# bolcom/serenade

Hardware: AMD Instinct MI355X
Metric: predict_next queries/sec (higher is better)
Workload: dtype u32 ids / i32 accumulators / f64 scores; 1 GPU; BASELINE configs[2]: synthetic 60000000 interactions / 1760000 items, k=1500 m=2500 idf_weighting=2 last_items=4 how_many=21; batch_per_gpu=1048576, query_pool_batches=2, parallelism=query-sharded replicas x1 (no data-path collective), index=csr (built by this library)

## Files before the change

### include/serenade_hip_internal.h

```cpp
#ifndef SERENADE_HIP_INTERNAL_H
#define SERENADE_HIP_INTERNAL_H

#include "serenade_hip.h"

#ifdef __cplusplus
extern "C" {
#endif

int srn_debug_phase_cycles(const srn_index_t* idx, int enable, uint64_t* out16);

int srn_debug_shard_group_times(const srn_shard_group_t* g, double* out_ms3);

int srn_debug_last_mid_count(const srn_index_t* idx, uint32_t* out_listed);
int srn_debug_last_dedup_count(const srn_index_t* idx, uint32_t* out_merged);
int srn_debug_serve_stamps(const srn_index_t* idx, uint32_t* out4);
uint32_t srn_debug_shard_nb_positions_stride(size_t k, size_t m);
int srn_debug_last_big_count(const srn_index_t* idx, uint32_t* out_listed);

int srn_debug_sback_launches(const srn_index_t* idx, uint64_t* out_launches);

int srn_debug_eval_terms(srn_eval_set_t* set, const srn_eval_trial_t* trial, double* out_terms, size_t cap, size_t* out_n, srn_eval_result_t* out);

int srn_debug_device_sessions_last_batch(srn_device_sessions_t* s, const void** d_items, const void** d_q_off, size_t* out_n, size_t* out_max_len,
                                         uint64_t* h_items, size_t cap, uint32_t* h_q_off);

int srn_debug_exclude_filter(const srn_index_t* idx, size_t nq, const uint64_t* d_wide_ids, const double* d_wide_scores, const uint32_t* d_wide_counts, size_t wide, const uint64_t* d_excl_flat,
                             const uint32_t* d_excl_off, size_t max_excl, const uint64_t* d_items_flat, const uint32_t* d_q_off, size_t how_many, uint64_t* d_out_ids, double* d_out_scores,
                             uint32_t* d_out_counts, void* stream);

int srn_debug_fill(const srn_index_t* idx, size_t nq, uint64_t* d_ids, double* d_scores, uint32_t* d_counts, size_t how_many, const uint64_t* d_excl_flat, const uint32_t* d_excl_off,
                   const uint64_t* d_items_flat, const uint32_t* d_q_off, unsigned flags, void* stream);

int srn_debug_class_counts(const uint64_t* acc, size_t n_waves, uint32_t* out16, int device);

#define SRN_DEBUG_MERGE_ROOM 12032
int srn_debug_merge_pair(uint32_t* room, const uint32_t* pairs, size_t n_pairs, int device);

void srn_debug_reload_knobs(void);

#ifdef __cplusplus
}
#endif
#endif
```

### serenade_amd/capi.py

```python
import ctypes as C
import os

import numpy as np

from . import build as _build

SRN_OK, SRN_EINVAL, SRN_ENOMEM, SRN_EHIP, SRN_ERANGE, SRN_EIO, SRN_ENODEV, SRN_ESTATE, SRN_ETIMEOUT = 0, -1, -2, -3, -4, -5, -6, -7, -8
ATTR_ADULT, ATTR_FOR_SALE, ATTR_NONE = 1, 2, 0xFF
FLAG_BUSINESS_LOGIC = 1
MAX_HOW_MANY, MAX_SESSION_LEN, MAX_K = 512, 255, 8192

_CODES = {SRN_EINVAL: "SRN_EINVAL", SRN_ENOMEM: "SRN_ENOMEM", SRN_EHIP: "SRN_EHIP", SRN_ERANGE: "SRN_ERANGE",
          SRN_EIO: "SRN_EIO", SRN_ENODEV: "SRN_ENODEV", SRN_ESTATE: "SRN_ESTATE", SRN_ETIMEOUT: "SRN_ETIMEOUT"}


class SerenadeError(RuntimeError):
    def __init__(self, code, msg):
        super().__init__("%s: %s" % (_CODES.get(code, code), msg))
        self.code = code


class SessionsView(C.Structure):
    _fields_ = [("sess_off", C.c_void_p), ("items", C.c_void_p), ("max_ts", C.c_void_p), ("n_sessions", C.c_size_t)]

# ... 143 lines not shown
    "srn_find_neighbors": (_i, [_vp, _vp, _sz, _sz, _sz, _vp, _vp, C.POINTER(_sz)]),
    "srn_index_free": (None, [_vp]),
    "srn_predict": (_i, [_vp, _vp, _sz, _sz, _sz, _sz, _i, _vp, _vp, C.POINTER(_sz)]),
    "srn_predict_stats": (_i, [_vp, C.POINTER(_u64), C.POINTER(_u64), C.POINTER(_u64)]),
    "srn_predict_batch": (_i, [_vp, _vp, _vp, _sz, _sz, _sz, _sz, C.c_uint, _vp, _vp, _vp]),
    "srn_batcher_create": (_i, [_vp, _sz, C.c_uint, _sz, _sz, _sz, _i, C.POINTER(_vp)]),
    "srn_batcher_predict": (_i, [_vp, _vp, _sz, _vp, _vp, C.POINTER(_sz)]),
    "srn_batcher_stats": (_i, [_vp, C.POINTER(_u64), C.POINTER(_u64), C.POINTER(_u64)]),
    "srn_batcher_free": (None, [_vp]),
    "srn_batcher_how_many": (_i, [_vp, C.POINTER(_sz)]),
    "srn_session_key": (_i, [C.c_char_p, _sz, C.POINTER(_u64), C.POINTER(_u64)]),
    "srn_session_store_create": (_i, [_u64, _u64, C.POINTER(_vp)]),
    "srn_session_store_free": (None, [_vp]),
    "srn_session_store_get": (_i, [_vp, _u64, _u64, _u64, _vp, _sz, C.POINTER(_sz)]),
    "srn_session_store_update": (_i, [_vp, _u64, _u64, _u64, _vp, _sz]),
    "srn_session_store_sweep": (_i, [_vp, _u64, C.POINTER(_u64)]),
    "srn_recommend": (_i, [_vp, _vp, C.c_char_p, _sz, _u64, _i, _sz, _u64, _vp, _vp, C.POINTER(_sz)]),
    "srn_predict_batch_device": (_i, [_vp, _vp, _vp, _sz, _sz, _sz, _sz, _sz, C.c_uint, _vp, _vp, _vp, _vp]),
    "srn_predict_batch_device_excl": (_i, [_vp, _vp, _vp, _sz, _sz, _vp, _vp, _sz, _sz, _sz, _sz, C.c_uint, _vp, _vp, _vp, _vp]),
    "srn_predict_batch_excl": (_i, [_vp, _vp, _vp, _sz, _vp, _vp, _sz, _sz, _sz, _sz, C.c_uint, _vp, _vp, _vp]),
    "srn_debug_exclude_filter": (_i, [_vp, _sz, _vp, _vp, _vp, _sz, _vp, _vp, _sz, _vp, _vp, _sz, _vp, _vp, _vp, _vp]),
    "srn_debug_fill": (_i, [_vp, _sz, _vp, _vp, _vp, _sz, _vp, _vp, _vp, _vp, C.c_uint, _vp]),
    "srn_debug_class_counts": (_i, [_vp, _sz, _vp, _i]),
    "srn_debug_merge_pair": (_i, [_vp, _vp, _sz, _i]),
    "srn_predict_batch_debug": (_i, [_vp, _vp, _vp, _sz, _sz, _sz, _sz, C.c_uint, _vp, _vp, _vp, _vp, _vp, _vp, _vp]),
    "srn_index_reserve": (_i, [_vp, _sz, _sz, _sz, _sz, _sz, C.c_uint, _vp]),
    "srn_last_kernel_ms": (_i, [_vp, C.POINTER(C.c_double), C.POINTER(C.c_double), C.POINTER(C.c_uint32)]),
    "srn_index_build_shard": (_i, [C.POINTER(SessionsView), _sz, _sz, C.c_double, C.c_uint32, C.c_uint32, _i, C.POINTER(_vp)]),
    "srn_index_shard": (_i, [_vp, C.c_uint32, C.c_uint32, _i, C.POINTER(_vp)]),
    "srn_index_build_shard_gpu": (_i, [C.POINTER(SessionsView), _sz, _sz, C.c_double, C.c_uint32, C.c_uint32, _i, C.POINTER(_vp)]),
    "srn_index_load_shard": (_i, [C.c_char_p, C.c_uint32, C.c_uint32, _i, C.POINTER(_vp)]),
    "srn_shard_group_unique_id": (_i, [_vp, _sz]),
    "srn_shard_group_create": (_i, [_vp, _vp, _i, _i, C.POINTER(_vp)]),
    "srn_shard_group_create_with_comm": (_i, [_vp, _i, _i, _vp, C.POINTER(_vp)]),
    "srn_shard_group_create_local": (_i, [C.POINTER(_vp), _i, C.POINTER(_vp)]),
    "srn_shard_group_predict_batch": (_i, [_vp, _vp, _vp, _sz, _sz, _sz, _sz, _sz, C.c_uint, _vp, _vp, _vp, _vp]),
    "srn_shard_group_stats": (_i, [_vp, _vp]),
    "srn_shard_group_set_overlap": (_i, [_vp, _i]),
    "srn_shard_group_wait": (_i, [_vp, _u64]),
    "srn_shard_group_set_postings": (_i, [_vp, _vp]),
    "srn_debug_shard_group_times": (_i, [_vp, _vp]),
    "srn_index_postings_view": (_i, [_vp, _i, C.POINTER(_vp)]),
    "srn_shard_group_free": (None, [_vp]),
    "srn_kernel_timing": (_i, [_vp, C.c_int]),
    "srn_kernel_times": (_i, [_vp, C.c_uint32, _vp, _vp, C.POINTER(C.c_uint32)]),
    "srn_kernel_times_detail": (_i, [_vp, C.c_uint32, _vp, _vp, _vp, _vp, C.POINTER(C.c_uint32)]),
    "srn_debug_phase_cycles": (_i, [_vp, _i, _vp]),
    "srn_debug_reload_knobs": (None, []),
    "srn_debug_last_mid_count": (_i, [_vp, C.POINTER(C.c_uint32)]),
    "srn_debug_last_dedup_count": (_i, [_vp, C.POINTER(C.c_uint32)]),
    "srn_debug_serve_stamps": (_i, [_vp, _vp]),
    "srn_debug_shard_nb_positions_stride": (C.c_uint32, [_sz, _sz]),
    "srn_debug_last_big_count": (_i, [_vp, C.POINTER(C.c_uint32)]),
    "srn_debug_sback_launches": (_i, [_vp, C.POINTER(_u64)]),
    "srn_last_path_counts": (_i, [_vp, C.POINTER(C.c_uint32), C.POINTER(C.c_uint32), C.POINTER(C.c_uint32)]),
    "srn_eval_set_create": (_i, [_vp, _vp, _vp, _sz, _vp, _vp, _sz, C.POINTER(_vp)]),
    "srn_eval_set_from_tsv": (_i, [_vp, C.c_char_p, C.c_char_p, C.POINTER(_vp)]),
    "srn_eval_set_from_events": (_i, [_vp, _vp, _vp, _vp, _sz, _vp, _sz, C.c_uint, _vp, C.POINTER(_vp)]),
    "srn_evaluate": (_i, [_vp, C.POINTER(EvalTrial), _sz, C.POINTER(EvalResult), _vp]),
    "srn_eval_set_free": (None, [_vp]),
    "srn_evaluate_bootstrap": (_i, [_vp, C.POINTER(EvalTrial), _sz, C.POINTER(Bootstrap), C.POINTER(EvalResult), _vp, _vp]),
    "srn_bootstrap_weights": (_i, [_u64, C.c_uint32, _u64, _sz, _vp]),
    "srn_debug_eval_terms": (_i, [_vp, C.POINTER(EvalTrial), _vp, _sz, C.POINTER(_sz), C.POINTER(EvalResult)]),
    "srn_device_sessions_create": (_i, [_i, _sz, _sz, _u64, _u64, C.POINTER(_vp)]),
    "srn_device_sessions_free": (None, [_vp]),
    "srn_device_sessions_get": (_i, [_vp, _u64, _u64, _u64, _vp, _sz, C.POINTER(_sz)]),
    "srn_device_sessions_update": (_i, [_vp, _u64, _u64, _u64, _vp, _sz]),
    "srn_device_sessions_sweep": (_i, [_vp, _u64, C.POINTER(_u64)]),
    "srn_device_sessions_stats": (_i, [_vp, C.POINTER(DeviceSessionsStats)]),
    "srn_device_sessions_timing": (_i, [_vp, _i]),
    "srn_device_sessions_last_ms": (_i, [_vp, C.POINTER(C.c_double), C.POINTER(C.c_double)]),
    "srn_device_sessions_count": (_i, [_vp, _u64, C.POINTER(_u64), C.POINTER(_u64)]),
    "srn_device_sessions_export_device": (_i, [_vp, _u64, _sz, _vp, _vp, _vp, _vp, _vp, _sz, _vp, _vp]),
    "srn_device_sessions_export": (_i, [_vp, _u64, _sz, _vp, _vp, _vp, _vp, _vp, _sz, C.POINTER(_sz)]),
    "srn_device_sessions_import_device": (_i, [_vp, _vp, _vp, _vp, _vp, _vp, _sz, _sz, _vp]),
    "srn_device_sessions_import": (_i, [_vp, _vp, _vp, _vp, _vp, _vp, _sz, _sz]),
    "srn_device_sessions_resize": (_i, [_vp, _sz, _sz, _u64]),
    "srn_device_sessions_set_max_capacity": (_i, [_vp, _sz]),
    "srn_device_sessions_growth": (_i, [_vp, C.POINTER(_u64), C.POINTER(_u64), C.POINTER(_u64)]),
    "srn_device_sessions_save": (_i, [_vp, C.c_char_p, _u64]),
    "srn_device_sessions_load": (_i, [C.c_char_p, _i, _sz, _sz, _u64, _u64, C.POINTER(_vp)]),
    "srn_device_sessions_file_info": (_i, [C.c_char_p, C.POINTER(DeviceSessionsFileInfo)]),
    "srn_device_sessions_top_items": (_i, [_vp, _u64, _u64, C.c_uint32, _sz, _vp, _vp, C.POINTER(_sz)]),
    "srn_index_set_fallback_trending": (_i, [_vp, _vp, _u64, _u64, C.c_uint32, _sz, C.c_uint, C.POINTER(_sz)]),
    "srn_session_keys": (_i, [_vp, _vp, _sz, _vp, _vp]),
    "srn_device_sessions_set_history": (_i, [_vp, _sz]),
    "srn_device_sessions_history": (_i, [_vp, C.POINTER(_sz)]),
    "srn_recommend_batch_device": (_i, [_vp, _vp, _vp, _vp, _vp, _vp, _sz, _u64, _sz, _sz, _sz, _sz, C.c_uint, _vp, _vp, _vp, _vp]),
    "srn_recommend_batch": (_i, [_vp, _vp, _vp, _vp, _vp, _vp, _sz, _u64, _sz, _sz, _sz, _sz, C.c_uint, _vp, _vp, _vp]),
    "srn_recommend_batch_device_at": (_i, [_vp, _vp, _vp, _vp, _vp, _vp, _vp, _sz, _u64, _sz, _sz, _sz, _sz, C.c_uint, _vp, _vp, _vp, _vp]),
    "srn_recommend_batch_at": (_i, [_vp, _vp, _vp, _vp, _vp, _vp, _vp, _sz, _u64, _sz, _sz, _sz, _sz, C.c_uint, _vp, _vp, _vp]),
    "srn_feedback_observe_device_at": (_i, [_vp, _vp, _vp, _vp, _vp, _vp, _sz, _u64, _vp, _vp, _vp, _sz, _vp, _vp]),
    "srn_feedback_observe_at": (_i, [_vp, _vp, _vp, _vp, _vp, _vp, _sz, _u64, _vp, _vp, _vp, _sz, _vp]),
    "srn_debug_device_sessions_last_batch": (_i, [_vp, C.POINTER(_vp), C.POINTER(_vp), C.POINTER(_sz), C.POINTER(_sz), _vp, _sz, _vp]),
    "srn_feedback_create": (_i, [_i, _sz, _sz, _u64, _u64, C.POINTER(_vp)]),
    "srn_feedback_free": (None, [_vp]),
    "srn_feedback_observe_device": (_i, [_vp, _vp, _vp, _vp, _vp, _sz, _u64, _vp, _vp, _vp, _sz, _vp, _vp]),
    "srn_feedback_observe": (_i, [_vp, _vp, _vp, _vp, _vp, _sz, _u64, _vp, _vp, _vp, _sz, _vp]),
    "srn_feedback_stats": (_i, [_vp, C.POINTER(FeedbackStats)]),
    "srn_feedback_histogram": (_i, [_vp, _vp, _vp, _sz]),
    "srn_feedback_reset_counters": (_i, [_vp]),
    "srn_feedback_sweep": (_i, [_vp, _u64, C.POINTER(_u64)]),
    "srn_feedback_get": (_i, [_vp, _u64, _u64, _u64, _vp, _sz, C.POINTER(C.c_uint32), C.POINTER(C.c_uint32), C.POINTER(_u64)]),
    "srn_feedback_bootstrap_enable": (_i, [_vp, C.c_uint32, _u64]),
    "srn_feedback_bootstrap_disable": (_i, [_vp]),
    "srn_feedback_bootstrap_info": (_i, [_vp, C.POINTER(C.c_uint32), C.POINTER(_u64)]),
# ... 82 lines not shown
```

### serenade_amd/csrc/srn_capi.cpp

```cpp
#include <algorithm>
#include <cstring>
#include <new>
#include <vector>

#include "srn_internal.h"

namespace srn { const char* last_error_cstr(); int device_count(); }
using namespace srn;

namespace {
template <typename F> int guarded(F f) {
    try { return f(); }
    catch (const std::bad_alloc&) { return fail(SRN_ENOMEM, "out of host memory"); }
    catch (const std::exception& e) { return fail(SRN_EINVAL, std::string("internal error: ") + e.what()); }
    catch (...) { return fail(SRN_EINVAL, "internal error"); }
}

int check_predict_args(const srn_index_t* idx, size_t k, size_t m, size_t how_many) {
    if (!idx) return fail(SRN_EINVAL, "null index");
    if (!idx->dev) return fail(SRN_ENODEV, "index has no device attached; there is no CPU fallback behind this ABI");
    if (idx->flat.postings_only) return fail(SRN_EINVAL, "a postings-only view holds no rows: it serves a shard group (srn_shard_group_set_postings), not predict calls");
    if (k == 0 || m == 0 || how_many == 0) return fail(SRN_EINVAL, "k, m and how_many must be > 0");
    if (how_many > SRN_MAX_HOW_MANY) return fail(SRN_ERANGE, "how_many above SRN_MAX_HOW_MANY");
    if (k > SRN_MAX_K) return fail(SRN_ERANGE, "k above SRN_MAX_K");
// ... 585 lines not shown
        if (rc) return rc;
        srn_index* ix = new srn_index();
        return finish_index(ix, shard_flat_index(full, shard, n_shards, ix->flat), device, out); });
}
int srn_index_load_shard(const char* path, uint32_t shard, uint32_t n_shards, int device, srn_index_t** out) {
    return guarded([&]() -> int {
        if (!path || !out) return fail(SRN_EINVAL, "null argument");
        *out = nullptr;
        FlatIndex full;
        int rc = load_flat_index(path, full);
        if (rc) return rc;
        srn_index* ix = new srn_index();
        rc = full.n_shards == 1 ? shard_flat_index(full, shard, n_shards, ix->flat)
                                : (full.shard == shard && full.n_shards == n_shards ? (ix->flat = std::move(full), SRN_OK) : fail(SRN_EINVAL, "the file holds another shard"));
        return finish_index(ix, rc, device, out); });
}
int srn_kernel_times(const srn_index_t* idx, uint32_t max_n, double* out_ms_main, double* out_ms_retry, uint32_t* out_n) {
    if (!idx || !idx->dev) return fail(SRN_ENODEV, "index has no device attached");
    if (!out_n) return fail(SRN_EINVAL, "null argument");
    return guarded([&]() -> int { return device_kernel_times(idx->dev, max_n, out_ms_main, out_ms_retry, out_n); });
}

int srn_kernel_times_detail(const srn_index_t* idx, uint32_t max_n, double* out_ms_prep, double* out_ms_fast, double* out_ms_predict,
                            double* out_ms_retry, uint32_t* out_n) {
    if (!idx || !idx->dev) return fail(SRN_ENODEV, "index has no device attached");
    if (!out_n) return fail(SRN_EINVAL, "null argument");
    return guarded([&]() -> int { return device_kernel_times(idx->dev, max_n, out_ms_predict, out_ms_retry, out_n, out_ms_prep, out_ms_fast); });
}

int srn_kernel_timing(srn_index_t* idx, int enable) {
    if (!idx || !idx->dev) return fail(SRN_ENODEV, "index has no device attached");
    return device_kernel_timing(idx->dev, enable);
}

int srn_debug_phase_cycles(const srn_index_t* idx, int enable, uint64_t* out16) {
    if (!idx || !idx->dev) return fail(SRN_ENODEV, "index has no device attached");
    return guarded([&]() -> int { return device_phase_cycles(idx->dev, enable, (unsigned long long*)out16); });
}

int srn_last_path_counts(const srn_index_t* idx, uint32_t* out_nq, uint32_t* out_general, uint32_t* out_global_pass) {
    if (!idx || !idx->dev) return fail(SRN_ENODEV, "index has no device attached");
    return guarded([&]() -> int { return device_last_path_counts(idx->dev, out_nq, out_general, out_global_pass); });
}
uint32_t srn_debug_shard_nb_positions_stride(size_t k, size_t m) {
    return device_shard_nb_positions_stride(launch_params(1, k, m, 21, 0, 4));
}
int srn_debug_serve_stamps(const srn_index_t* idx, uint32_t* out4) {
    if (!idx || !idx->dev || !out4) return fail(SRN_EINVAL, "null argument");
    return device_serve_last_stamps(idx->dev, out4);
}
int srn_debug_last_mid_count(const srn_index_t* idx, uint32_t* out_listed) {
    if (!idx || !idx->dev) return fail(SRN_ENODEV, "index has no device attached");
    return guarded([&]() -> int { return device_last_mid_count(idx->dev, out_listed); });
}
int srn_debug_last_dedup_count(const srn_index_t* idx, uint32_t* out_merged) {
    if (!idx || !idx->dev || !out_merged) return fail(SRN_EINVAL, "null argument");
    return guarded([&]() -> int { return device_last_dedup_count(idx->dev, out_merged); });
}
int srn_debug_last_big_count(const srn_index_t* idx, uint32_t* out_listed) {
    if (!idx || !idx->dev) return fail(SRN_ENODEV, "index has no device attached");
    return guarded([&]() -> int { return device_last_mid_count(idx->dev, nullptr, out_listed); });
}

int srn_debug_sback_launches(const srn_index_t* idx, uint64_t* out_launches) {
    if (!idx || !idx->dev || !out_launches) return fail(SRN_EINVAL, "null argument / no device");
    *out_launches = device_sback_launches(idx->dev); return SRN_OK;
}

void srn_debug_reload_knobs(void) { reload_knobs(); }

static int check_eval_index(const srn_index_t* idx) {
    if (!idx) return fail(SRN_EINVAL, "null index");
    if (!idx->dev) return fail(SRN_ENODEV, "index has no device attached; evaluation runs on the GPU only");
    if (idx->flat.postings_only) return fail(SRN_EINVAL, "a postings-only view holds no rows");
    return check_not_a_shard(idx);
}

static int check_trials(const srn_eval_set_t* set, const srn_eval_trial_t* trials, size_t n_trials, const srn_eval_result_t* out) {
    if (n_trials && (!trials || !out)) return fail(SRN_EINVAL, "null argument");
    for (size_t t = 0; t < n_trials; ++t) {
        const srn_eval_trial_t& tr = trials[t];
        if (tr.max_items_in_session == 0) return fail(SRN_EINVAL, "max_items_in_session must be > 0");
        if (tr.max_items_in_session > SRN_MAX_SESSION_LEN) return fail(SRN_ERANGE, "max_items_in_session above SRN_MAX_SESSION_LEN: a prefix could exceed the kernels' session limit");
        if (tr.length == 0) return fail(SRN_EINVAL, "length must be > 0");
        if (tr.length > SRN_MAX_HOW_MANY) return fail(SRN_ERANGE, "length above SRN_MAX_HOW_MANY");
        if (tr.k == 0 || tr.m == 0 || tr.how_many == 0) return fail(SRN_EINVAL, "k, m and how_many must be > 0");
        if (tr.how_many > SRN_MAX_HOW_MANY) return fail(SRN_ERANGE, "how_many above SRN_MAX_HOW_MANY");
        if (tr.k > SRN_MAX_K) return fail(SRN_ERANGE, "k above SRN_MAX_K");
        if (tr.m > 0x7FFFFFFFu) return fail(SRN_ERANGE, "m too large");
        if (tr.history != 0 && (tr.history < tr.max_items_in_session || tr.history > SRN_MAX_SESSION_LEN))
            return fail(SRN_ERANGE, "history must be 0 or in max_items_in_session..SRN_MAX_SESSION_LEN");
        if (tr.how_many + eval_excl_capacity(tr) > SRN_MAX_HOW_MANY)
            return fail(SRN_ERANGE, "how_many + the exclusion lists' capacity (history, or max_items_in_session) above SRN_MAX_HOW_MANY");
    }
    if (!set) return fail(SRN_EINVAL, "null evaluation set");
    for (size_t t = 0; t < n_trials; ++t) { int rc = check_predict_args(set->idx, trials[t].k, trials[t].m, trials[t].how_many); if (rc) return rc;
                                            if (trials[t].flags & SRN_FLAG_FILL) { rc = check_has_fallback(set->idx); if (rc) return rc; } }
    return SRN_OK;
}

int srn_eval_set_create(const srn_index_t* idx, const uint64_t* items_flat, const uint64_t* sess_off, size_t n_sessions,
                        const uint64_t* train_item_ids, const uint64_t* train_item_counts, size_t n_train_items, srn_eval_set_t** out) {
    return guarded([&]() -> int {
        if (!out) return fail(SRN_EINVAL, "null argument");
        *out = nullptr;
        int rc = check_eval_index(idx); if (rc) return rc;
// ... 280 lines not shown
```

### serenade_amd/csrc/srn_fast.hip

```cpp
#include <hip/hip_runtime.h>

#include <cstdio>
#include <cstdlib>

#include "srn_device.h"
#include "srn_prep.h"
#include "srn_kernels.h"

namespace srn {

#ifndef SRN_FAST_NT
#define SRN_FAST_NT 1
#endif
typedef uint32_t fin_v4u __attribute__((ext_vector_type(4)));
__device__ __forceinline__ void fin_store(uint4* p, const uint4& v) {
#if SRN_FAST_NT
    __builtin_nontemporal_store((fin_v4u{v.x, v.y, v.z, v.w}), reinterpret_cast<fin_v4u*>(p));
#else
    *p = v;
#endif
}
__device__ __forceinline__ uint4 fin_load(const uint4* p) {
#if SRN_FAST_NT
    const fin_v4u v = __builtin_nontemporal_load(reinterpret_cast<const fin_v4u*>(p)); return make_uint4(v.x, v.y, v.z, v.w);
// ... 232 lines not shown
            inm |= in ? 1u << x : 0u;
            nmp |= in ? (unsigned long long)nmv[x] << (4 * x) : 0ull;
            acc += in ? 1ull << (4u * nmv[x]) : 0ull;
        }
    }
    uint32_t* cls = misc + FS_CLS;
    {
        const uint32_t wc = wave_class_counts(acc, lane);
        const uint32_t mycnt = lane < 16u ? wc : 0u;
        if (mycnt) atomicAdd(&cls[lane], mycnt);
    }
    __syncthreads();
    uint32_t nstar, rstar;
    {
        const uint32_t cv = lane < 16u ? cls[lane] : 0u; const uint32_t pre = wave_incl_scan(cv);
        const uint32_t suf = (uint32_t)__builtin_amdgcn_readlane((int)pre, 63) - pre + cv;
        const unsigned long long reach = __ballot(suf >= k);
        nstar = 63u - (uint32_t)__clzll((long long)reach);
        rstar = k - ((uint32_t)__builtin_amdgcn_readlane((int)suf, (int)nstar) - (uint32_t)__builtin_amdgcn_readlane((int)cv, (int)nstar));
    }
    uint32_t mine = 0;
#pragma unroll
    for (int x = 0; x < G; ++x) mine += ((inm >> x) & 1u) && (uint32_t)((nmp >> (4 * x)) & 15ull) == nstar;
    uint32_t tot_star;
    uint32_t before = block_excl_scan<BLOCK>(mine, misc + FS_SCAN_B, tot_star);
    uint32_t sel = 0, tmask = 0;
#pragma unroll
    for (int x = 0; x < G; ++x) {
        const bool in = (inm >> x) & 1u; const uint32_t c = (uint32_t)((nmp >> (4 * x)) & 15ull);
        const bool eq = in && c == nstar, take = in && (c > nstar || (eq && before < rstar));
        tmask |= take ? 1u << x : 0u; sel += take; before += eq;
    }
    const uint32_t inc = wave_incl_scan(sel);
    uint32_t base = 0; if (lane == 63u && inc) base = atomicAdd(&misc[FS_NB], inc);
    uint32_t at = (uint32_t)__builtin_amdgcn_readlane((int)base, 63) + inc - sel;
#pragma unroll
    for (int x = 0; x < G; ++x) if ((tmask >> x) & 1u) nbl[at++] = fv[x];
    return 0xFFFFFFFFu;
}

enum { FM_FUSED = 0, FM_FRONT = 1, FM_BACK = 2 };
template <int WG_PER_CU, bool FRAG, bool WIDE, int MODE = FM_FUSED, bool MID = false, bool BIG = false, bool LONG = false, bool TINY = false>
#ifndef SRN_FAST_WAVES
#define SRN_FAST_WAVES (WG_PER_CU * 2)
#endif
#ifndef SRN_TINY_WAVES
#define SRN_TINY_WAVES 2
#endif
__global__ __launch_bounds__(512, TINY ? SRN_TINY_WAVES : BIG ? 4 : SRN_FAST_WAVES) void vmis_fast_kernel(DeviceIndex ix_arg, LaunchParams p_arg, FastParams f_arg) {
#if SRN_FAST_SMALL
    static_assert(!BIG || MID, "BIG is a form of MID"); static_assert(!LONG || BIG, "LONG is a form of BIG");
    constexpr uint32_t SIDF = BIG ? F_BIG_TOTAL - (F_TOTAL - F_SIDF) : F_SIDF, SATTR = SIDF + 512 * 8;
    constexpr uint32_t MW = (SIDF - F_WORK) / 4;
    __shared__ __attribute__((aligned(16))) char smem[BIG ? F_BIG_TOTAL : F_TOTAL];
#else
    extern __shared__ __attribute__((aligned(16))) char smem[];
#endif
    typedef const __attribute__((address_space(4))) char* KArg;
    const KArg ka = (KArg)__builtin_amdgcn_kernarg_segment_ptr();
    constexpr size_t OFF_P = (sizeof(DeviceIndex) + alignof(LaunchParams) - 1) / alignof(LaunchParams) * alignof(LaunchParams);
    constexpr size_t OFF_F = (OFF_P + sizeof(LaunchParams) + alignof(FastParams) - 1) / alignof(FastParams) * alignof(FastParams);
    const __attribute__((address_space(4))) DeviceIndex& ix = *(const __attribute__((address_space(4))) DeviceIndex*)ka;
    const __attribute__((address_space(4))) LaunchParams& p = *(const __attribute__((address_space(4))) LaunchParams*)(ka + OFF_P);
    const __attribute__((address_space(4))) FastParams& f = *(const __attribute__((address_space(4))) FastParams*)(ka + OFF_F);
    constexpr int BLOCK = 512, NW = 8;
    constexpr int NL = LONG ? (int)F_LONG_LISTS : MID ? (int)F_MID_LISTS : 4;
    constexpr uint32_t SINV = F_SINV;
    static_assert(!MID || MODE == FM_FUSED, "MID: fused form only");
    const uint32_t tid = threadIdx.x, lane = tid & 63u, wave = tid >> 6;
    const unsigned long long lt = (1ull << lane) - 1ull;
    static_assert(!TINY || (MODE == FM_FUSED && !BIG && !FRAG), "TINY: the lean or the MID fused form over an unsharded index");
    if constexpr (TINY) {
        unsigned long long* const a_items = reinterpret_cast<unsigned long long*>(smem + F_W10 + 64); uint32_t* const a_off = reinterpret_cast<uint32_t*>(smem + F_W10 + 64 + 64);
        const uint32_t alen = f.tiny_len;
        if (f.serve == nullptr) {
        if (alen) { if (tid < 8u) a_items[tid] = f.tiny_items[tid]; if (tid == 0u) { a_off[0] = 0u; a_off[1] = alen; } __syncthreads(); }
        if (tid < PREP_LANES) prep_group(ix_arg, alen ? (const uint64_t*)a_items : p.items_flat, alen ? (const uint32_t*)a_off : p.q_off, alen ? 0u : blockIdx.x, tid, p.m, p.max_len,
                                         const_cast<char*>(p.prep) + (size_t)blockIdx.x * p.prep_stride, nullptr, 0u, nullptr);
        __syncthreads();
        }
    }

    uint32_t* misc = (uint32_t*)(smem + F_MISC);
    uint8_t* wlut = (uint8_t*)(smem + F_WLUT);
    uint16_t* w10t = (uint16_t*)(smem + F_W10);
    uint32_t* nbl = (uint32_t*)(smem + F_NBL);
    unsigned long long* ckey = (unsigned long long*)(smem + F_CAND);
    uint32_t* cidx = (uint32_t*)(smem + F_CAND + F_CAND_CAP * 8);
    char* const acc_base = smem + F_HOT;
    uint32_t* hot = (uint32_t*)(smem + F_HOT);
    uint32_t* ikeys = (uint32_t*)(smem + F_TABLE);
    int* iacc = (int*)(smem + F_TABLE + F_TABLE_WORDS * 4);
    uint2* hits = (uint2*)(smem + F_HITS);
    uint32_t* surv = (uint32_t*)(smem + F_SURV);
    constexpr uint32_t SURV_CAP = F_SURV_WORDS - 256u;
    uint32_t* const cls_area = BIG ? (uint32_t*)(smem + SIDF) - 256 : surv + SURV_CAP;
    uint32_t* const dn_area = cls_area - F_M_MAX / 4u;
    uint2* const nb2 = reinterpret_cast<uint2*>(dn_area - F_K_MAX * 2u);
    uint32_t* thist = surv + SURV_CAP;
    auto num_of = [&](uint32_t set) -> uint32_t {
        if constexpr (MID) return (uint32_t)wlut[set & 31u] + (uint32_t)wlut[32u + (set >> 5)];
        else return (uint32_t)wlut[set]; };
    auto w10_of = [&](uint32_t set) -> uint32_t {
        if constexpr (MID) { const uint32_t lo = set & 31u, hi = set >> 5; const uint32_t mp = lo ? (uint32_t)wlut[64u + lo] : (uint32_t)wlut[96u + hi]; return (9u - mp) * ((uint32_t)wlut[lo] + (uint32_t)wlut[32u + hi]); }
        else return (uint32_t)w10t[set]; };

    unsigned long long* tacc = (unsigned long long*)(smem + F_MISC + FS_TACC * 4);
    if (tid < 16u) tacc[tid] = 0ull;
    const bool ticking = p.phase_cycles != nullptr;
    const bool business = (p.flags & SRN_FLAG_BUSINESS_LOGIC) != 0u;
    const uint32_t n_kept = ix.n_kept;
    auto qpos = [&](uint32_t pq) -> uint32_t { return ((wave + NW * (pq >> 6)) << 6) + (pq & 63u); };

    uint32_t* const pre = (uint32_t*)(smem + F_W10 + 64);
    bool have_pre = false;
    { const ItemMeta m0 = f.meta_sample[tid];
      ((double*)(smem + SIDF))[tid] = m0.idf > 0.0 ? m0.idf : 1.0; ((uint8_t*)(smem + SATTR))[tid] = (uint8_t)m0.attr;
      if (tid < 16u) ((double*)(smem + SINV))[tid] = tid < 8u ? f.inv_idf_hot[tid] : f.inv_idf_hi; }
    const bool listed = !MID && MODE == FM_BACK && f.mid_list != nullptr;
    const uint32_t q_end = TINY ? p.nq : LONG ? *f.long_cnt : BIG ? *f.bigq_cnt : MID || listed ? *f.mid_cnt : p.nq;
    const bool ordered = !MID && MODE != FM_FRONT && f.order != nullptr && !listed;
    const uint32_t ox = blockIdx.x & 7u;
    const bool serving = TINY && f.serve != nullptr;
    const uint32_t qi_step = serving ? 0u : ordered ? gridDim.x >> 3 : gridDim.x;
    uint32_t serve_seq = 0u; bool serve_have = false; unsigned long long serve_t0 = 0ull, serve_c0 = 0ull;
    if constexpr (TINY) { if (serving) serve_seq = __atomic_load_n(&(f.serve + blockIdx.x)->done_seq, __ATOMIC_RELAXED); }
    const uint32_t qi_end = ordered ? ord_count(f.order_dups != nullptr ? p.nq - *f.order_dups : p.nq, ox) : q_end;
    for (uint32_t qi = ordered ? blockIdx.x >> 3 : (MODE == FM_FRONT ? f.q_base : 0u) + blockIdx.x; qi < qi_end; qi += qi_step) {
        if constexpr (TINY) {
            if (serving) {
                uint32_t* const sv_flag = reinterpret_cast<uint32_t*>(smem + F_W10 + 64 + 192);
                unsigned long long* const sv_items = reinterpret_cast<unsigned long long*>(smem + F_W10 + 64); uint32_t* const sv_off = reinterpret_cast<uint32_t*>(smem + F_W10 + 64 + 128);
                ServeCtl* const c = f.serve + blockIdx.x;
                __syncthreads();
                if (wave == 0u) {
                    __threadfence_system();
                    uint32_t leave = 0u;
                    if (serve_have && lane == 0u) {
                        const uint32_t cnt = __atomic_load_n(&p.out_counts[blockIdx.x], __ATOMIC_RELAXED);
                        if (cnt & 0x80000000u) { (void)atomicExch(&f.slow_cnt[SC_GENERAL], 0u); (void)atomicExch(&f.slow_cnt[SC_MID], 0u); (void)atomicExch(&f.slow_cnt[SC_BIG_TICKET_LO], 0u); (void)atomicExch(&f.slow_cnt[SC_BIG_TICKET_HI], 0u); }
                        const unsigned long long t_end = wall_clock64();
                        c->stamp[2] = (uint32_t)(t_end - serve_t0); c->stamp[3] = (uint32_t)((unsigned long long)clock64() - serve_c0);
                        __atomic_store_n(&c->count, cnt, __ATOMIC_RELAXED);
                        __atomic_store_n(&c->status, (cnt & 0x80000000u) ? 1u : 0u, __ATOMIC_RELAXED);
                        __threadfence_system();
                        __atomic_store_n(&c->done_seq, serve_seq, __ATOMIC_RELAXED);
                    }
                    const unsigned long long t0 = wall_clock64(), idle = __builtin_nontemporal_load(&c->idle_ticks);
                    uint32_t w = 0u, s_new = 0u, n = 0u;
                    for (;;) {
                        if (lane < 16u) w = __atomic_load_n(reinterpret_cast<const uint32_t*>(c) + lane, __ATOMIC_RELAXED);
                        s_new = (uint32_t)__builtin_amdgcn_readlane((int)w, 0); n = min((uint32_t)__builtin_amdgcn_readlane((int)w, 1), 16u);
                        if (s_new != serve_seq) {
                            uint32_t x = lane >= 4u && lane < 4u + 2u * min(n, 5u) ? w : 0u;
#pragma unroll
                            for (int d = 1; d < 16; d <<= 1) x ^= __shfl_xor(x, d, 16);
                            if ((uint32_t)__builtin_amdgcn_readlane((int)x, 0) == ((uint32_t)__builtin_amdgcn_readlane((int)w, 2) ^ s_new ^ n)) break;
                        }
                        if ((uint32_t)__builtin_amdgcn_readlane((int)w, 3) != 0u || wall_clock64() - t0 > idle) { leave = 1u; break; }
                    }
                    if (!leave) {
                        serve_seq = s_new; serve_have = true; serve_t0 = wall_clock64(); serve_c0 = (unsigned long long)clock64();
                        if (lane >= 4u && lane < 14u) reinterpret_cast<uint32_t*>(sv_items)[lane - 4u] = w;
                        if (n > 5u && lane < 2u * (n - 5u)) reinterpret_cast<uint32_t*>(sv_items)[10u + lane] = __atomic_load_n(reinterpret_cast<const uint32_t*>(c->more) + lane, __ATOMIC_RELAXED);
                        if (lane == 0u) { sv_off[0] = 0u; sv_off[1] = n; p.out_counts[blockIdx.x] = 0x80000002u; c->stamp[0] = (uint32_t)(serve_t0 - t0); }
                    }
                    if (lane == 0u) sv_flag[0] = leave;
                }
                __syncthreads();
                if (sv_flag[0] != 0u) break;
                if (tid < PREP_LANES) prep_group(ix_arg, (const uint64_t*)sv_items, (const uint32_t*)sv_off, 0u, tid, p.m, p.max_len, const_cast<char*>(p.prep) + (size_t)blockIdx.x * p.prep_stride, nullptr, 0u, nullptr);
                __syncthreads();
                if (tid == 0u) c->stamp[1] = (uint32_t)(wall_clock64() - serve_t0);
            }
        }
        const uint32_t q = TINY ? qi : LONG ? f.long_list[qi] : BIG ? f.bigq_list[qi] : MID || listed ? f.mid_list[qi] : ordered ? (uint32_t)f.order[ord_pos(ox, qi)] : qi;
        const uint32_t q_ord_next = ordered && qi + qi_step < qi_end ? (uint32_t)f.order[ord_pos(ox, qi + qi_step)]
                                  : listed && qi + qi_step < qi_end ? f.mid_list[qi + qi_step] : 0xFFFFFFFFu;
#ifndef SRN_MID_PREFETCH
#define SRN_MID_PREFETCH 0
#endif
        const uint32_t q_after = !(MID && SRN_MID_PREFETCH) ? 0xFFFFFFFFu : qi + gridDim.x < q_end ? (BIG ? f.bigq_list : f.mid_list)[qi + gridDim.x] : 0xFFFFFFFFu;
        long long t_prev = ticking ? clock64() : 0;
        FAST_PRIO(FP_REC);
        const char* const rec = p.prep + (size_t)q * p.prep_stride;
        struct { uint32_t U, rmax, xlo, sumw, L, n_staged, cur_attr, unsafe; } hd;
        constexpr uint32_t HW = (uint32_t)sizeof(PrepHead) / 4u;
        struct { uint32_t idx, kept; unsigned long long base; } x0{kNone, 0u, 0ull};
        if (have_pre) {
            auto uni = [&](uint32_t w) -> uint32_t { return (uint32_t)__builtin_amdgcn_readfirstlane((int)pre[w]); };
            hd.U = uni(0); hd.rmax = uni(1); hd.xlo = uni(2); hd.sumw = uni(3); hd.L = uni(6); hd.n_staged = uni(7); hd.cur_attr = uni(16); hd.unsafe = uni(17);
            if (lane < (LONG ? 32u : MID ? 16u : 8u) && lane < hd.L) { const uint32_t* it = pre + HW + 6u * lane; x0.idx = it[0]; x0.kept = it[3]; x0.base = ((unsigned long long)it[5] << 32) | it[4]; }
        } else {
            const PrepHead h0 = *(const PrepHead*)rec;
            hd.U = h0.U; hd.rmax = h0.rmax; hd.xlo = h0.xlo; hd.sumw = h0.sumw; hd.L = h0.L; hd.n_staged = h0.n_staged; hd.cur_attr = h0.cur_attr; hd.unsafe = h0.unsafe;
            if ((MID ? lane < (LONG ? 32u : 16u) && lane < p.max_len : lane < 8u) && lane < hd.L) { const PrepItem pi = ((const PrepItem*)(rec + sizeof(PrepHead)))[lane]; x0.idx = pi.idx; x0.kept = pi.kept; x0.base = pi.base; }
        }
        have_pre = false;
        const uint32_t L = hd.L, n = hd.n_staged, U = hd.U;
        unsigned long long rm = __ballot(x0.kept > 0u);
#ifdef SRN_FAST_EXP_ONELIST
        rm &= 0ull - rm;
#endif
        const uint32_t nr = (uint32_t)__popcll(rm);
        const bool rel = MID || (WIDE && nr > 3u);
        const uint32_t NB = LONG ? F_LONG_NB : MID ? max(nr, 4u) : WIDE && !rel ? 3u : 4u, NBM = (1u << NB) - 1u, base = rel ? hd.xlo : 0u;
        const bool fits = hd.unsafe != 0u ? false : LONG ? L >= 1u && L <= F_LONG_LMAX && L <= p.max_len && hd.sumw <= F_LONG_CLASSES && nr <= F_LONG_LISTS && 2u * n + 8u + F_LONG_RES_WORDS <= MW && hd.rmax - hd.xlo < (1u << (32u - F_LONG_NB))
                        : MID ? L >= 1u && L <= F_MID_LMAX && L <= p.max_len && hd.sumw <= F_MID_CLASSES && nr <= F_MID_LISTS && 2u * n + 8u + 256u <= MW && hd.rmax - hd.xlo < (1u << (32u - NB))
                              : L >= 1u && L <= 8u && L <= p.max_len && hd.sumw <= 15u && nr <= 4u && 2u * n + 8u <= MW && (!rel || hd.rmax - hd.xlo < (1u << 28));
        uint32_t* const xq = MODE == FM_FUSED ? nullptr : f.xchg + (size_t)q * f.xchg_stride;
        if (!fits) {
            if constexpr (MODE == FM_FRONT) { if (tid == 0) xq[0] = 0xFFFFFFFFu; }
            else if (tid == 0) {
                if (hd.unsafe != 0u) f.slow_list[atomicAdd(&f.slow_cnt[SC_GENERAL], 1u)] = q;
                else if (!MID && MODE == FM_FUSED && f.bigq_list != nullptr && L >= 1u && L <= 8u && L <= p.max_len && hd.sumw <= 15u && nr <= 4u && hd.rmax - hd.xlo < (1u << 28) &&
                    2u * n + 8u + 256u <= (F_BIG_TOTAL - (F_TOTAL - F_SIDF) - F_WORK) / 4u) f.bigq_list[atomicAdd(f.bigq_cnt, 1u)] = q;
                else if (!MID && MODE == FM_FUSED && f.mid_list != nullptr && L >= 1u && L <= F_MID_LMAX && L <= p.max_len) f.mid_list[atomicAdd(f.mid_cnt, 1u)] = q;
                else if (!MID && MODE == FM_FUSED && f.long_list != nullptr && L > F_MID_LMAX && L <= F_LONG_LMAX && L <= p.max_len) f.long_list[atomicAdd(f.long_cnt, 1u)] = q;
                else if (MID && !BIG && f.bigq_list != nullptr && L >= 1u && L <= F_MID_LMAX && L <= p.max_len && hd.sumw <= F_MID_CLASSES && nr <= F_MID_LISTS && hd.rmax - hd.xlo < (1u << (32u - NB)) &&
                         2u * n + 8u + 256u <= (F_BIG_TOTAL - (F_TOTAL - F_SIDF) - F_WORK) / 4u) f.bigq_list[atomicAdd(f.bigq_cnt, 1u)] = q;
                else f.slow_list[atomicAdd(&f.slow_cnt[SC_GENERAL], 1u)] = q;
            }
            continue;
        }
        if (n == 0u) { if (tid == 0) { if constexpr (MODE == FM_FRONT) xq[0] = 0u; else p.out_counts[q] = 0u; } continue; }
        uint32_t kp[NL], ps[NL]; const uint32_t* src[NL];
#pragma unroll
        for (int r = 0; r < NL; ++r) {
            const int l = rm ? __ffsll((long long)rm) - 1 : 0;
            kp[r] = rm ? (uint32_t)__builtin_amdgcn_readlane((int)x0.kept, l) : 0u;
            const uint32_t blo = (uint32_t)__builtin_amdgcn_readlane((int)(uint32_t)x0.base, l), bhi = (uint32_t)__builtin_amdgcn_readlane((int)(uint32_t)(x0.base >> 32), l);
            src[r] = ix.post_rank + (((unsigned long long)bhi << 32) | blo);
            ps[r] = (uint32_t)l;
            rm &= rm - 1ull;
        }
        const uint32_t cur_idx = (uint32_t)__builtin_amdgcn_readlane((int)x0.idx, 0);
        const uint32_t cur_attr = hd.cur_attr;
        const uint32_t s1 = kp[0], s2 = s1 + kp[1], s3 = s2 + kp[2];

        uint32_t v[4][5];
        uint32_t K = 0;
        uint32_t pfv[4] = {0u, 0u, 0u, 0u};
        uint32_t xsv[3] = {0u, 0u, 0u};
        if constexpr (MODE == FM_BACK) {
            const uint32_t kv = xq[0];
#pragma unroll
            for (int t = 0; t < 3; ++t) xsv[t] = xq[1u + min(wave * 64u + lane + (uint32_t)t * BLOCK, f.xchg_stride - 2u)];
            K = (uint32_t)__builtin_amdgcn_readfirstlane((int)kv);
        } else {
#pragma unroll
        for (int r = 0; r < 4; ++r)
#pragma unroll
            for (int j = 0; j < 5; ++j) { v[r][j] = 0u; if ((uint32_t)j * BLOCK < kp[r]) v[r][j] = src[r][min(tid + j * BLOCK, kp[r] - 1u)]; }
        }
        __syncthreads();
        FAST_PRIO(FP_FRONT);
        if constexpr (MODE != FM_BACK) {
#pragma unroll
        for (int r = 0; r < 4; ++r)
#pragma unroll
            for (int j = 0; j < 5; ++j) asm volatile("" : "+v"(v[r][j]));
        }
        FAST_TICK(0);
        if (tid < (uint32_t)FS_TACC) misc[tid] = 0;
#ifndef SRN_FAST_EARLY_CLEAR
#define SRN_FAST_EARLY_CLEAR 0
#endif
        const uint32_t clr_lo = (!SRN_FAST_EARLY_CLEAR || MODE == FM_FRONT) ? F_TABLE : (MODE == FM_BACK || nr <= 1u) ? F_HOT : min(F_TABLE, max(F_HOT, (F_WORK + (2u * n + 16u) * 4u + 15u) & ~15u));
        if (SRN_FAST_EARLY_CLEAR && MODE != FM_FRONT) {
            uint4* z = reinterpret_cast<uint4*>(smem);
            for (uint32_t i = clr_lo / 16u + tid; i < F_TABLE / 16u; i += BLOCK) z[i] = make_uint4(0u, 0u, 0u, 0u);
        }
        if constexpr (LONG) {
            if (tid < 32u) {
                uint32_t pr = 0u;
#pragma unroll
                for (int r = 0; r < NL; ++r) pr = tid == (uint32_t)(31 - r) ? ps[r] : pr;
                wlut[tid] = (uint8_t)(L - pr); wlut[32u + tid] = (uint8_t)pr;
            }
        } else
        if constexpr (MID) {
            if (tid < 64u) {
                const uint32_t half = tid >> 5, hs = tid & 31u;
                uint32_t num = 0u, mp = 0u;
                const uint32_t lo = hs ? (uint32_t)__ffs((int)hs) - 1u : 0u;
#pragma unroll
                for (int r = 0; r < 5; ++r) { const uint32_t pr = half ? ps[5 + r] : ps[r]; num += ((hs >> r) & 1u) ? L - pr : 0u; mp = lo == (uint32_t)r ? pr : mp; }
                wlut[tid] = (uint8_t)num; wlut[64u + tid] = (uint8_t)mp;
            }
        } else
        if (tid < (1u << nr)) {
            const uint32_t num = ((tid & 1u) ? L - ps[0] : 0u) + ((tid & 2u) ? L - ps[1] : 0u) + ((tid & 4u) ? L - ps[2] : 0u) + ((tid & 8u) ? L - ps[3] : 0u);
            const uint32_t lo = tid ? (uint32_t)__ffs((int)tid) - 1u : 0u;
            const uint32_t mp = lo == 0u ? ps[0] : lo == 1u ? ps[1] : lo == 2u ? ps[2] : ps[3];
            wlut[tid] = (uint8_t)num; w10t[tid] = (uint16_t)((9u - mp) * num);
        }
        if constexpr (MODE == FM_BACK) {
            if (K == 0xFFFFFFFFu) { if (tid == 0) f.slow_list[atomicAdd(&f.slow_cnt[SC_GENERAL], 1u)] = q; continue; }
            if (K == 0u) { if (tid == 0) p.out_counts[q] = 0u; continue; }
        } else
        if (nr == 1u) {
            K = min(kp[0], p.k);
#pragma unroll
            for (int j = 0; j < 3; ++j) { const uint32_t e = tid + j * BLOCK; if ((uint32_t)j * BLOCK < K && e < K) {
                if constexpr (LONG) nb2[e] = make_uint2(((v[0][j] - base) << NB) | 31u, (uint32_t)((9 - (int)ps[0]) * (int)(L - ps[0])));
                else nbl[e] = ((v[0][j] - base) << NB) | 1u; } }
            __syncthreads();
// ... 241 lines not shown
        __syncthreads();
        FAST_PRIO(FP_WALK);
        FAST_TICK(8);
        auto add2 = [&](uint32_t wd, uint32_t w) {
            if constexpr (LONG) {
                const bool neg = (int)w < 0; const uint32_t a = wd & 0xFFFFu, b = wd >> 16;
                if (!neg || a < F_SKETCH - F_HOT) atomicAdd((uint32_t*)(acc_base + a), w);
                if (!neg || b < F_SKETCH - F_HOT) atomicAdd((uint32_t*)(acc_base + b), w);
            } else {
            atomicAdd((uint32_t*)(acc_base + (wd & 0xFFFFu)), w); atomicAdd((uint32_t*)(acc_base + (wd >> 16)), w); } };
        constexpr uint32_t INL1 = FRAG ? 6u : 14u, INL2 = FRAG ? 20u : 28u;
        uint32_t cnt3 = 0;
#pragma unroll
        for (int t = 0; t < 3; ++t) {
            const bool m3 = wave * 64u + lane + (uint32_t)t * BLOCK < K && (rq[t].x & 0xFFFFu) > INL1;
            const unsigned long long b3 = __ballot(m3);
            if (m3) nbl[qpos(cnt3 + (uint32_t)__popcll(b3 & lt))] = LONG ? wave * 64u + lane + (uint32_t)t * BLOCK : svr[t];
            cnt3 += (uint32_t)__popcll(b3);
        }
#ifdef SRN_FAST_SUBTICKS
        FAST_TICK(5);
#endif
        uint32_t wr[3];
#pragma unroll
        for (int t = 0; t < 3; ++t) wr[t] = LONG ? wvr[t] : w10_of(svr[t] & NBM);
        if constexpr (!FRAG) {
#pragma unroll
            for (int t = 0; t < 3; ++t) {
                const bool more6 = wave * 64u + lane + (uint32_t)t * BLOCK < K && (rq[t].x & 0xFFFFu) > 6u;
                const size_t r1 = more6 ? (size_t)(base + (svr[t] >> NB)) : (size_t)n_kept;
                rq1[t] = *reinterpret_cast<const uint4*>(&f.row_packed[r1 * 4 + 1]);
            }
        }
        auto tok_slot = [&](uint32_t tok) -> uint32_t { if constexpr (LONG) return nb2[tok].x; else return tok; };
        auto tok_w = [&](uint32_t tok, uint32_t slot) -> uint32_t { if constexpr (LONG) return nb2[tok].y; else return w10_of(slot & NBM); };
        auto q3_load = [&](uint32_t p0, uint32_t& tok, uint32_t& sv, uint32_t& hdr, uint4& c4, uint4& d4, uint32_t& blk) {
            tok = nbl[qpos(min(p0 + lane, cnt3 - 1u))];
            sv = tok_slot(tok);
            if constexpr (FRAG) {
                const uint4 s4 = *reinterpret_cast<const uint4*>(f.row_packed + (size_t)(base + (sv >> NB)));
                hdr = s4.x;
                const uint4* eb = reinterpret_cast<const uint4*>(f.row_ext16) + ((hdr & 0xFFFFu) > 6u ? (size_t)s4.w : (size_t)0);
                c4 = eb[0]; d4 = eb[1]; blk = s4.w + 2u;
            } else {
                const RowQuad* rowp = f.row_packed + (size_t)(base + (sv >> NB)) * 4;
                hdr = *reinterpret_cast<const uint32_t*>(rowp); c4 = *reinterpret_cast<const uint4*>(rowp + 2); d4 = *reinterpret_cast<const uint4*>(rowp + 3); blk = 0u;
            } };
        uint32_t tk3 = 0, sv3 = 0, hdr3 = 0, blk3 = 0; uint4 c43 = make_uint4(0u, 0u, 0u, 0u), d43 = c43;
        if (cnt3) q3_load(0u, tk3, sv3, hdr3, c43, d43, blk3);
        const uint32_t w3 = cnt3 ? tok_w(tk3, sv3) : 0u;
        const uint32_t qn = MID ? q_after : ordered || listed ? q_ord_next : q + gridDim.x;
        const bool park = MID ? q_after != 0xFFFFFFFFu : ordered || listed ? q_ord_next != 0xFFFFFFFFu : qn < p.nq;
        if (wave == 1u && park) {
            const char* const rn = p.prep + (size_t)qn * p.prep_stride + lane * 4u;
            const uint32_t dst = (uint32_t)__builtin_amdgcn_readfirstlane((int)lds_addr(pre));
            if (lane * 4u < p.prep_stride) glds_dword_uncounted(rn, dst);
            if (256u + lane * 4u < min(p.prep_stride, 320u)) glds_dword_uncounted(rn + 256, dst + 256u);
        }
#pragma unroll
        for (int t = 0; t < 3; ++t) {
            if (wave * 64u + (uint32_t)t * BLOCK < K) {
                const bool act = wave * 64u + lane + (uint32_t)t * BLOCK < K;
                const uint32_t w = wr[t], len = rq[t].x & 0xFFFFu;
                if constexpr (FRAG) { if (act) { add2(rq[t].y, w); add2(rq[t].z, w); if (len <= 6u) add2(rq[t].w, w); } }
                else if (act) { add2(rq[t].y, w); add2(rq[t].z, w); add2(rq[t].w, w); }
            }
        }
        if constexpr (!FRAG) {
#pragma unroll
        for (int t = 0; t < 3; ++t) {
            if (wave * 64u + (uint32_t)t * BLOCK < K) {
                const bool act = wave * 64u + lane + (uint32_t)t * BLOCK < K;
                const uint32_t w = wr[t], len = rq[t].x & 0xFFFFu;
                if (act && len > 6u) { add2(rq1[t].x, w); add2(rq1[t].y, w); add2(rq1[t].z, w); add2(rq1[t].w, w); }
            }
        }
        }
        auto add_tail = [&](uint32_t p0, uint32_t w, uint32_t hdr, const uint4& c4, const uint4& d4, uint32_t blk) {
            const bool act = p0 + lane < cnt3;
            const uint32_t len = hdr & 0xFFFFu;
            const bool more = FRAG ? true : len > 30u;
            if constexpr (FRAG) {
                if (act) { add2(c4.x, w); add2(c4.y, w); add2(c4.z, w); add2(c4.w, w); }
                if (act && len > 12u) { add2(d4.x, w); add2(d4.y, w); add2(d4.z, w); add2(d4.w, w); }
            } else if (act) {
                add2(c4.x, w); add2(c4.y, w); add2(c4.z, w); add2(c4.w, w);
                add2(d4.x, w); add2(d4.y, w); add2(d4.z, w);
                if (len <= 30u) add2(d4.w, w);
            }
            for (uint32_t t8 = INL2; __ballot(act && more && t8 < len) != 0ull; t8 += 8u) {
                if (act && more && t8 < len) {
                    const uint4 e4 = reinterpret_cast<const uint4*>(f.row_ext16)[(size_t)blk + ((t8 - INL2) >> 3)];
                    add2(e4.x, w); add2(e4.y, w); add2(e4.z, w); add2(e4.w, w);
                }
            } };
#ifdef SRN_FAST_SUBTICKS
        FAST_TICK(6);
#endif
        FAST_PRIO_X(1);
        { fin_v4u dv = {d43.x, d43.y, d43.z, d43.w};
          asm volatile("" : "+v"(hdr3), "+v"(dv));
          d43 = make_uint4(dv.x, dv.y, dv.z, dv.w); }
        if constexpr (!FRAG) blk3 = d43.w;
        if (cnt3) add_tail(0u, w3, hdr3, c43, d43, blk3);
        for (uint32_t p0 = 64u; p0 < cnt3; p0 += 64u) { uint32_t tk, sv, hdr, blk; uint4 c4, d4; q3_load(p0, tk, sv, hdr, c4, d4, blk); if constexpr (!FRAG) blk = d4.w; add_tail(p0, tok_w(tk, sv), hdr, c4, d4, blk); }
#ifdef SRN_FAST_SUBTICKS
        FAST_TICK(7);
#endif
        __syncthreads();
        FAST_PRIO(FP_HARV);
// ... 605 lines not shown
```

### serenade_amd/csrc/srn_internal.h

```cpp
#pragma once
#include <cstddef>
#include <cstdint>
#include <mutex>
#include <string>
#include <vector>

#include "../../include/serenade_hip.h"

namespace srn {

void set_error(const std::string& msg);
int fail(int code, const std::string& msg);
std::string last_error_string();

struct IdSlot {
    uint64_t key;
    uint32_t idx;
    uint32_t pad;
};
static constexpr uint32_t kNone = 0xFFFFFFFFu;

static inline uint64_t mix64(uint64_t x) {
    x ^= x >> 33; x *= 0xff51afd7ed558ccdULL;
    x ^= x >> 33; x *= 0xc4ceb9fe1a85ec53ULL;
// ... 118 lines not shown
    for (size_t q = 0; q < nq; ++q) if (counts[q] == 0xFFFFFFFFu) return fail(SRN_ERANGE, "a query exceeded the kernel's table limits");
    return SRN_OK;
}
int device_exclude_filter(DeviceState* d, uint32_t nq, const uint64_t* w_ids, const double* w_scores, const uint32_t* w_counts, uint32_t wide, const uint64_t* x_flat, const uint32_t* x_off,
                          uint32_t max_excl, const uint64_t* items_flat, const uint32_t* q_off, uint64_t* out_ids, double* out_scores, uint32_t* out_counts, uint32_t how_many, void* stream);
bool device_has_fallback(const DeviceState* d);
int device_set_fallback(DeviceState* d, const FlatIndex& ix, const uint64_t* item_ids, uint32_t n);
void device_clear_fallback(DeviceState* d);
int device_fill(DeviceState* d, uint32_t nq, uint64_t* ids, double* scores, uint32_t* counts, uint32_t how_many, const uint64_t* x_flat, const uint32_t* x_off,
                const uint64_t* items_flat, const uint32_t* q_off, bool whole_session, bool business, void* stream);
int device_debug_class_counts(const uint64_t* acc, size_t n_waves, uint32_t* out16, int device);
int device_debug_merge_pair(uint32_t* room, const uint32_t* pairs, size_t n_pairs, int device);
struct ShardIO {
    void* cand; uint32_t* cand_cnt;
    const void* gathered; const uint32_t* gathered_cnt; uint32_t n_shards;
    uint32_t gathered_stride;
    void* nb; uint32_t* nb_cnt; int* minpos;
};

bool device_shard_lists_supported(DeviceState* d, const FlatIndex& ix, const LaunchParams& p);
bool device_fast_eligible(DeviceState* d, const FlatIndex& ix, const LaunchParams& p, uint64_t max_row_len_all = 0);
bool device_has_packed_rows(const DeviceState* d);
int device_sback_attach_postings(DeviceState* d, DeviceState* post, uint64_t n_postings);
bool device_sback_streams(const DeviceState* d);
bool device_sback_wanted(const DeviceState* d);
uint64_t device_sback_launches(const DeviceState* d);
int device_shard_nb_prep(DeviceState* d, DeviceState* post, const LaunchParams& p, char* records, void* stream, char** order_buf = nullptr, size_t* order_bytes = nullptr,
                         const unsigned long long** order_out = nullptr);
int device_shard_nb_front(DeviceState* d, const FlatIndex& ix, DeviceState* post, const LaunchParams& p, const char* records, uint32_t* xchg, uint32_t xchg_stride, uint32_t q_lo, uint32_t q_hi, void* stream);
int device_shard_nb_back(DeviceState* d, const FlatIndex& ix, DeviceState* post, const LaunchParams& p, const char* records, uint32_t* xchg, uint32_t xchg_stride, void* stream,
                         const unsigned long long* order = nullptr, bool positions = false);
int device_shard_nb_positions(DeviceState* d, const FlatIndex& ix, DeviceState* post, const LaunchParams& p, const char* records, const uint32_t* xin, uint32_t in_stride, uint32_t* xout, uint32_t out_stride,
                              uint32_t q_lo, uint32_t q_hi, void* stream);
uint32_t device_shard_nb_positions_stride(const LaunchParams& p);
uint32_t device_prep_stride(uint32_t max_len);
int device_shard_lists_head(DeviceState* d, const LaunchParams& p, void* pos, int* head, void* stream);
int device_shard_lists_count(DeviceState* d, const LaunchParams& p, const void* pos, const int* head, uint32_t* kept, int* tot, void* stream);
int device_shard_lists_copy(DeviceState* d, const LaunchParams& p, const void* pos, const uint32_t* kept, const long long* off, uint32_t* out, void* stream);
int device_shard_lists_predict(DeviceState* d, const FlatIndex& ix, const LaunchParams& p, uint32_t n_shards, const uint32_t* kept_g, const long long* off_g,
                               unsigned long long shard_stride, const uint32_t* lists_g, const int* head, const void* pos_local, char* records, void* stream,
                               const unsigned long long* shard_base = nullptr, bool direct = false);
int device_shard_stage(DeviceState* d, const FlatIndex& ix, int stage, const LaunchParams& p, const ShardIO& sh, void* stream);
int device_slot_bytes(DeviceState* d, const FlatIndex& ix, uint32_t max_len, uint32_t* num_bits = nullptr);
int device_serve_start(DeviceState* d, const FlatIndex& ix, uint32_t k, uint32_t m, uint32_t how_many, uint32_t flags, uint32_t lanes, uint32_t max_items, uint32_t idle_ms);
int device_serve_stop(DeviceState* d);
int device_serve_predict(DeviceState* d, const uint64_t* items, uint32_t len, uint32_t k, uint32_t m, uint32_t how_many, uint32_t flags, uint64_t* out_ids, double* out_scores, size_t* out_n);
int device_serve_last_stamps(DeviceState* d, uint32_t* out4);
int device_serve_stats(DeviceState* d, uint64_t* served, uint64_t* not_served, uint64_t* launches, uint32_t* lanes);
int device_last_kernel_ms(DeviceState* d, double* ms_main, double* ms_retry, uint32_t* retried);
int device_phase_cycles(DeviceState* d, int enable, unsigned long long* out16);
int device_kernel_timing(DeviceState* d, int enable);
int device_reserve(DeviceState* d, const FlatIndex& ix, const LaunchParams& p, void* stream);
int device_last_path_counts(DeviceState* d, uint32_t* nq, uint32_t* general, uint32_t* global_pass);
int device_last_mid_count(DeviceState* d, uint32_t* listed, uint32_t* big_listed = nullptr);
int device_last_dedup_count(DeviceState* d, uint32_t* merged);
static constexpr unsigned kFlagNoResultCache = 0x80000000u;
int device_result_cache_enable(DeviceState* d, uint64_t rows, uint32_t max_len, uint32_t k, uint32_t m, uint32_t how_many, uint32_t flags);
int device_result_cache_disable(DeviceState* d);
int device_result_cache_clear(DeviceState* d);
int device_result_cache_clear_if_enabled(DeviceState* d);
int device_result_cache_stats(DeviceState* d, srn_result_cache_stats_t* out);
void device_result_cache_bypassed(DeviceState* d);
int device_kernel_times(DeviceState* d, uint32_t max_n, double* ms_main, double* ms_retry, uint32_t* out_n, double* ms_prep = nullptr, double* ms_fast = nullptr);

}

namespace srn {
struct Combiner;
Combiner* combiner_create();
void combiner_free(Combiner* c);
void combiner_stats(const Combiner* c, uint64_t* rounds, uint64_t* requests, uint64_t* max_round);
int combiner_predict(Combiner* c, const srn_index* idx, const uint64_t* evolving, size_t len, size_t k, size_t m, size_t how_many, unsigned flags,
                     uint64_t* out_ids, double* out_scores, size_t* out_n, int lanes, size_t round_cap);
int knob_predict_lanes();
size_t knob_tiny_max();
}

struct srn_index {
    srn::FlatIndex flat;
    srn::DeviceState* dev = nullptr;
    int device = -1;
    srn::Combiner* comb = nullptr;
    std::vector<uint64_t> fallback;
    mutable std::vector<uint32_t> session_to_rank; mutable std::once_flag s2r_once;
};
struct srn_sessions {
    srn::Sessions s;
    srn_load_info_t info{};
};
struct srn_events {
    uint64_t* s = nullptr; uint64_t* i = nullptr; uint64_t* t = nullptr;
    size_t n = 0;
    int device = -1;
};

namespace srn { struct EvalDevice; }
struct srn_eval_set {
    const srn_index* idx = nullptr;
    std::vector<uint64_t> sess_off;
    uint64_t max_session_len = 0;
    double max_freq = 1.0;
    uint64_t unique_training_items = 0;
    srn::EvalDevice* dev = nullptr;
};
namespace srn {
int eval_set_create(const srn_index* idx, const uint64_t* items_flat, const uint64_t* sess_off, size_t n_sessions,
// ... 80 lines not shown
```

### serenade_amd/csrc/srn_kernels.h

```cpp
#pragma once
#include <hip/hip_runtime.h>

#include "srn_internal.h"

namespace srn {

static constexpr uint32_t EMPTY32 = 0xFFFFFFFFu;
static constexpr int CAND_CAP = 1024;
static constexpr int MISC_WORDS = 64;
static constexpr int kBlock = 512;
static constexpr int SEL_BITS = 11, SEL_BINS = 1 << SEL_BITS;
static constexpr int SEL_WORDS = SEL_BINS + SEL_BINS / 32;

struct KernelCfg {
    uint32_t sess_slots, item_slots;
    uint32_t item_buckets;
    uint32_t hot_slots;
    uint32_t sketch_slots, sketch_shift;
    uint32_t sum_bits;
    uint32_t num_bits;
    uint32_t q_cap;
    uint32_t off_q, off_wave, off_b, off_a;
    uint32_t region_a_bytes;
    uint32_t no_merge;
};

struct LaunchAux { const uint32_t* qlist; const uint32_t* qlist_n; uint32_t* retry_list; uint32_t* retry_cnt; char* gscratch; unsigned long long gscratch_stride; char* nb_spill; };

struct PrepHead { uint32_t U, rmax, xlo, sumw, P, nruns, L, n_staged, run_start[8], cur_attr, unsafe; };
struct PrepItem { uint32_t idx, len, pre, kept; unsigned long long base; };

struct ShardPos { uint32_t idx, len; unsigned long long base; };

#ifndef SRN_FAST_SMALL
#define SRN_FAST_SMALL 1
#endif
#if defined(SRN_FAST_EXP_LDS40)
static constexpr uint32_t F_HOT_WORDS = 3840, F_SK_WORDS = 1024, F_DUMP_WORDS = 256, F_TABLE_BUCKETS = 127, F_TABLE_WORDS = 512, F_SURV_WORDS = 512, F_WG_PER_CU = 4;
#elif SRN_FAST_SMALL
static constexpr uint32_t F_HOT_WORDS = 4096, F_SK_WORDS = 4096, F_DUMP_WORDS = 256, F_TABLE_BUCKETS = 127, F_TABLE_WORDS = 512, F_SURV_WORDS = 512, F_WG_PER_CU = 3;
#else
static constexpr uint32_t F_HOT_WORDS = 4096, F_SK_WORDS = 8192, F_DUMP_WORDS = 1024, F_TABLE_BUCKETS = 127, F_TABLE_WORDS = 512, F_SURV_WORDS = 768, F_WG_PER_CU = 2;
#endif
static constexpr uint32_t F_MISC = 0, F_WLUT = 256, F_W10 = 512, F_NBL = 1024, F_K_MAX = 1536, F_CAND = F_NBL + F_K_MAX * 4, F_CAND_CAP = 160;
static constexpr uint32_t F_HOT = 9216, F_SKETCH = F_HOT + F_HOT_WORDS * 4, F_DUMP = F_SKETCH + F_SK_WORDS * 4, F_TABLE = F_DUMP + F_DUMP_WORDS * 4;
static constexpr uint32_t F_HITS = F_HOT, F_HIT_CAP = F_HOT_WORDS / 2 - 1, F_ZERO_OFF = (F_HOT_WORDS - 1) * 4;
#ifndef SRN_FAST_REPLICAS
#define SRN_FAST_REPLICAS 1
#endif
#ifndef SRN_FAST_REP_ITEMS
#define SRN_FAST_REP_ITEMS 16
#endif
static constexpr uint32_t F_REP_ITEMS = SRN_FAST_REPLICAS ? SRN_FAST_REP_ITEMS : 0, F_REP = 8, F_DIRECT = F_HOT_WORDS - F_REP_ITEMS * F_REP;
static constexpr uint32_t F_SURV = F_TABLE + F_TABLE_WORDS * 8;
static constexpr uint32_t F_LDS_BYTES = F_SURV + F_SURV_WORDS * 4;
static constexpr uint32_t F_WORK = F_NBL, F_WORK_WORDS = (F_LDS_BYTES - F_WORK) / 4;
static constexpr uint32_t F_M_MAX = 2560;
static constexpr uint32_t F_FIN_BYTES = 1024, F_FIN_ENTRIES = F_FIN_BYTES / 16 - 1;
static_assert(F_CAND + F_CAND_CAP * 12 <= F_HOT, "candidate buffer overlaps the accumulators");
static constexpr uint32_t F_BIG_TOTAL = 80 * 1024;
static constexpr uint32_t F_MID_LISTS = 10, F_MID_LMAX = 10, F_MID_CLASSES = 63;
static constexpr uint32_t F_LONG_LISTS = 20, F_LONG_LMAX = 20, F_LONG_CLASSES = 255, F_LONG_NB = 5;
static constexpr uint32_t F_LONG_RES_WORDS = F_K_MAX * 2 + F_M_MAX / 4 + 256;
static_assert(F_LDS_BYTES * F_WG_PER_CU <= 160 * 1024, "LDS budget");
static_assert(F_DUMP + F_DUMP_WORDS * 4 - F_HOT <= 65536, "16-bit row offsets");
struct ServeCtl {
    uint32_t seq, len, check, stop;
    unsigned long long items[5]; unsigned long long pad1;
    unsigned long long more[8];
    uint32_t pad2[2]; unsigned long long idle_ticks; uint32_t pad3[12];
    uint32_t done_seq, status, count, alive; uint32_t stamp[4]; uint32_t pad4[8];
};
static_assert(sizeof(ServeCtl) == 256, "ServeCtl layout");
enum SlowCnt : uint32_t { SC_GENERAL = 0, SC_MID = 1, SC_BIG_TICKET_LO = 2, SC_BIG_TICKET_HI = 3, SC_BIGQ = 4, SC_LONG = 5, SC_TINY_TICKET = 6, SC_SPARE = 7, SC_WORDS = 8 };
using SlowCntBlock = uint32_t[SC_WORDS];
enum HostWord : uint32_t { HW_GLOBAL = 0, HW_GENERAL = 1, HW_MID = 2, HW_BIGQ = 3, HW_OVER63 = 4, HW_SEQ = 5, HW_MERGED = 6, HW_WORDS = 8 };
using HostWordBlock = uint32_t[HW_WORDS];
enum SlowPart : uint32_t { SL_GENERAL = 0, SL_MID = 1, SL_BIGQ = 2, SL_LONG = 3 };
inline uint32_t* slow_part(uint32_t* slow_list, size_t slow_cap, SlowPart part) { return slow_list + (size_t)part * (slow_cap + 16); }
struct FastParams {
    const RowQuad* row_packed; const uint32_t* row_ext16;
    const ItemMeta* meta_sample;
    double inv_idf_hot[8];
    double inv_idf_hi;
    uint32_t* slow_list; uint32_t* slow_cnt;
    uint32_t* bigq_list; uint32_t* bigq_cnt;
    uint32_t* long_list; uint32_t* long_cnt;
    uint32_t* mid_list; uint32_t* mid_cnt;
    char* fin;
    char* big_arena; uint32_t* big_list; unsigned long long* big_ticket; uint32_t big_cap_entries;
    uint32_t nb;
    uint32_t max_runs;
    uint32_t* xchg; uint32_t xchg_stride; uint32_t q_base;
    const unsigned long long* order;
    uint64_t tiny_items[8]; uint32_t tiny_len, host_seq;
    ServeCtl* serve;
    uint32_t* host_words;
    const uint32_t* order_dups;
};
hipError_t sort_order_keys(hipStream_t st, const unsigned long long* in, unsigned long long* out, size_t n, void* temp, size_t* temp_bytes);
uint32_t dedup_slots(uint32_t nq);
hipError_t launch_dedup_group(hipStream_t st, const uint64_t* items_flat, const uint32_t* q_off, uint32_t nq, uint32_t* slots, uint32_t* slot_min, uint32_t n_slots, uint32_t hash_bits,
                              uint32_t* rep, unsigned long long* okeys, uint32_t* out_counts, uint32_t* n_dup);
hipError_t launch_dedup_mark(hipStream_t st, uint32_t nq, const uint32_t* rep, uint32_t* out_counts);
hipError_t launch_dedup_fill(hipStream_t st, uint32_t nq, const uint32_t* rep, uint64_t* out_ids, double* out_scores, uint32_t* out_counts, uint32_t how_many, const uint32_t* n_dup, uint32_t* host_word);

static constexpr uint32_t RC_WAYS = 8, RC_MAX_LEN = 8;
enum ResultCacheCounter : uint32_t { RC_LOOKUPS = 0, RC_HITS = 1, RC_INSERTS = 2, RC_EVICTIONS = 3, RC_COUNTERS = 4 };
struct ResultCacheView {
    uint32_t* stamp; uint32_t* len; uint32_t* count;
    uint64_t* keys; uint64_t* ids; double* scores;
    unsigned long long* counters;
    uint32_t n_buckets, max_len, how_many, hash_mask;
};

static constexpr uint32_t SB_H = 1024, SB_S = 1024, SB_DUMP = 64, SB_REP_ITEMS = 16, SB_REP = 8, SB_DIRECT = SB_H - SB_REP_ITEMS * SB_REP;
struct SBackParams {
    const uint2* frag8;
    const uint4* ext8;
    const ItemMeta* sample;
    double inv_idf_chunk[SB_H / 256];
    double inv_idf_all;
    const uint2* frag_post;
    const uint32_t* post_rank;
    uint32_t finish_here;
    uint32_t* scr;
};
hipError_t launch_rows_to_frag8(hipStream_t st, const uint64_t* row_off, const uint32_t* row_items, uint64_t n_rows, const uint32_t* block_base, uint2* frag8, uint4* ext8);
hipError_t launch_frag_post(hipStream_t st, const uint32_t* post_rank, const uint2* frag8, uint2* out, uint64_t n);
uint32_t shard_back_scratch_words();
hipError_t launch_shard_nb_positions(dim3 grid, hipStream_t st, const char* prep, uint32_t prep_stride, uint32_t max_len, const uint32_t* xin, uint32_t in_stride, uint32_t* xout, uint32_t out_stride,
                                     const uint32_t* post_rank, uint32_t q_lo, uint32_t q_hi, uint32_t m, bool wide);
uint32_t shard_nb_positions_stride(uint32_t k, uint32_t m);
hipError_t launch_shard_back(dim3 grid, hipStream_t st, const DeviceIndex& di, const LaunchParams& p, const FastParams& f, const SBackParams& sb, bool debug = false);

struct PredictLaunch {
    bool masks = false, slot64 = false, global_tables = false; int stage = 0;
    const uint32_t* qlist = nullptr; const uint32_t* qn = nullptr;
    uint32_t* retry_list = nullptr; uint32_t* retry_cnt = nullptr;
    char* gscratch = nullptr; unsigned long long gstride = 0; char* spill = nullptr; ShardIO sh{};
};
hipError_t launch_predict(const PredictLaunch& a, dim3 grid, size_t lds, hipStream_t st, const DeviceIndex& di, const LaunchParams& p, const KernelCfg& c);
hipError_t launch_prep(hipStream_t st, const DeviceIndex& di, const uint64_t* items_flat, const uint32_t* q_off, uint32_t nq, uint32_t m,
                       uint32_t max_len, char* out, uint32_t stride, uint32_t* zero_a = nullptr, uint32_t* zero_b = nullptr,
                       const IdSlot* loc_table = nullptr, uint32_t loc_mask = 0, unsigned long long* okeys = nullptr);
hipError_t launch_finish_big(hipStream_t st, const DeviceIndex& di, const FastParams& f, uint64_t* out_ids, double* out_scores, uint32_t* out_counts, uint32_t how_many, uint32_t grid, const uint32_t* cnt_retry = nullptr, const uint32_t* cnt_slow = nullptr, uint32_t* host_words = nullptr);
hipError_t launch_finish(hipStream_t st, const DeviceIndex& di, const FastParams& f, uint64_t* out_ids, double* out_scores, uint32_t* out_counts, uint32_t nq, uint32_t how_many);
hipError_t launch_shard_lists_head(hipStream_t st, const DeviceIndex& di, const uint64_t* items_flat, const uint32_t* q_off, uint32_t nq, uint32_t m, uint32_t max_len,
                                   ShardPos* pos_out, int* head);
hipError_t launch_shard_lists_count(hipStream_t st, const DeviceIndex& di, const uint32_t* q_off, uint32_t nq, uint32_t max_len, const ShardPos* pos_in, const int* head,
                                    uint32_t* kept, int* tot);
hipError_t launch_shard_lists_copy(hipStream_t st, const DeviceIndex& di, uint32_t nq, uint32_t max_len, const ShardPos* pos_in, const uint32_t* kept, const long long* off,
                                   uint32_t* out);
hipError_t launch_shard_prep(hipStream_t st, const uint64_t* items_flat, const uint32_t* q_off, uint32_t nq, uint32_t max_len, uint32_t n_shards, const uint32_t* kept_g,
                             const long long* off_g, unsigned long long shard_stride, const int* head, const ShardPos* pos_local, char* out, uint32_t stride,
                             const unsigned long long* shard_base = nullptr, bool direct = false);
hipError_t launch_shard_max(hipStream_t st, int* dst, const int* src, size_t n);
hipError_t launch_shard_offsets(hipStream_t st, const uint32_t* kept_g, uint32_t nq, uint32_t max_len, uint32_t n_shards, long long* off_g, unsigned long long* tot_dev,
                                unsigned long long* tot_host, unsigned long long* chunk_scratch);
hipError_t launch_shard_min(hipStream_t st, int* dst, const int* src, size_t n);
hipError_t launch_shard_scrub_counts(hipStream_t st, uint32_t* cnt_g, uint32_t n_shards, uint32_t nq, uint32_t* flag);
hipError_t launch_shard_mark(hipStream_t st, const uint32_t* flag, uint32_t nq, uint32_t* out_counts);
hipError_t launch_shard_fill_i32(hipStream_t st, int* dst, int v, size_t n);
hipError_t launch_shard_merge_topn(hipStream_t st, const char* part, size_t block_bytes, uint32_t n_shards, uint32_t nq, uint32_t how_many, uint64_t* out_ids, double* out_scores,
                                   uint32_t* out_counts);
enum class FastForm { Lean, Mid, Big, Long, Tiny, TinyMid, Front, Back };
hipError_t launch_fast(FastForm form, dim3 grid, hipStream_t st, const DeviceIndex& di, const LaunchParams& p, const FastParams& f, bool debug = false);
hipError_t launch_rows_to_packed(hipStream_t st, const uint64_t* row_off, const uint32_t* row_items, uint64_t n_rows, const uint32_t* block_base,
                                 uint32_t* packed, uint32_t* ext16, bool frag = false);
hipError_t launch_rows_to_frags(hipStream_t st, const uint64_t* row_off, const uint32_t* row_items, uint64_t n_rows, const uint32_t* block_base,
                                uint32_t* slots, uint32_t* ext);
hipError_t launch_rows_to_slots(hipStream_t st, const uint64_t* row_off, const uint32_t* row_items, uint64_t n_rows, const uint32_t* block_base,
                                uint32_t* slots, uint32_t* ext);

}
```

### serenade_amd/csrc/srn_kernels.hip

```cpp
#include <hip/hip_runtime.h>

#include <algorithm>
#include <cstdio>
#include <cstdlib>
#include <mutex>
#include <string>
#include <vector>

#include "srn_kernels.h"
#include "srn_device.h"
#include "srn_prep.h"

namespace srn {

#define HIP_TRY(expr)                                                                                   \
    do {                                                                                                \
        hipError_t e_ = (expr);                                                                         \
        if (e_ != hipSuccess) return fail(SRN_EHIP, std::string(#expr) + ": " + hipGetErrorString(e_)); \
    } while (0)


static constexpr int MAX_ITEM_PASSES = 64;


// ... 206 lines not shown
                                                             const uint32_t* __restrict__ block_base, uint32_t* __restrict__ slots, uint32_t* __restrict__ ext) {
    __shared__ uint32_t wave_tot[16];
    const uint64_t r = (uint64_t)blockIdx.x * 1024 + threadIdx.x;
    const int lane = threadIdx.x & 63, wave = threadIdx.x >> 6;
    uint64_t o = 0, len = 0;
    if (r < n) { o = row_off[r]; len = row_off[r + 1] - o; }
    const uint32_t e = len > 15 ? (uint32_t)(len - 14) : 0u;
    uint32_t inc = e;
#pragma unroll
    for (int d = 1; d < 64; d <<= 1) { const uint32_t t = __shfl_up(inc, d, 64); if (lane >= d) inc += t; }
    if (lane == 63) wave_tot[wave] = inc;
    __syncthreads();
    uint32_t base = block_base[blockIdx.x];
    for (int w = 0; w < wave; ++w) base += wave_tot[w];
    const uint32_t eoff = base + inc - e;
    if (r > n) return;
    uint32_t sl[16];
#pragma unroll
    for (int i = 0; i < 16; ++i) sl[i] = EMPTY32;
    sl[0] = (uint32_t)len;
    if (len <= 15) { for (uint32_t i = 0; i < (uint32_t)len; ++i) sl[1 + i] = row_items[o + i]; }
    else { sl[1] = eoff;
#pragma unroll
           for (int i = 0; i < 14; ++i) sl[2 + i] = row_items[o + i];
           for (uint64_t i = 14; i < len; ++i) ext[eoff + (i - 14)] = row_items[o + i]; }
    uint4* dst = reinterpret_cast<uint4*>(slots + r * 16);
#pragma unroll
    for (int qd = 0; qd < 4; ++qd) dst[qd] = make_uint4(sl[4 * qd], sl[4 * qd + 1], sl[4 * qd + 2], sl[4 * qd + 3]);
}

__global__ __launch_bounds__(1024) void rows_to_frags_kernel(const uint64_t* __restrict__ row_off, const uint32_t* __restrict__ row_items, uint64_t n,
                                                             const uint32_t* __restrict__ block_base, uint32_t* __restrict__ slots, uint32_t* __restrict__ ext) {
    __shared__ uint32_t wave_tot[16];
    const uint64_t r = (uint64_t)blockIdx.x * 1024 + threadIdx.x;
    const int lane = threadIdx.x & 63, wave = threadIdx.x >> 6;
    uint64_t o = 0, len = 0;
    if (r < n) { o = row_off[r]; len = row_off[r + 1] - o; }
    const uint32_t e = len > 3 ? (uint32_t)(len - 2) : 0u;
    const uint32_t inc = wave_incl_scan(e);
    if (lane == 63) wave_tot[wave] = inc;
    __syncthreads();
    uint32_t base = block_base[blockIdx.x];
    for (int w = 0; w < wave; ++w) base += wave_tot[w];
    const uint32_t eoff = base + inc - e;
    if (r > n) return;
    uint32_t sl[4] = {(uint32_t)len, EMPTY32, EMPTY32, EMPTY32};
    if (len <= 3) { for (uint32_t i = 0; i < (uint32_t)len; ++i) sl[1 + i] = row_items[o + i]; }
    else { sl[1] = eoff; sl[2] = row_items[o]; sl[3] = row_items[o + 1];
           for (uint64_t i = 2; i < len; ++i) ext[eoff + (i - 2)] = row_items[o + i]; }
    reinterpret_cast<uint4*>(slots)[r] = make_uint4(sl[0], sl[1], sl[2], sl[3]);
}

__global__ __launch_bounds__(256) void vmis_prep_kernel(DeviceIndex ix, const uint64_t* __restrict__ items_flat, const uint32_t* __restrict__ q_off,
                                                        uint32_t nq, uint32_t m, uint32_t max_len, char* out, uint32_t stride, uint32_t* zero_a, uint32_t* zero_b,
                                                        const IdSlot* __restrict__ loc_table, uint32_t loc_mask, unsigned long long* __restrict__ okeys) {
    const uint32_t t = blockIdx.x * blockDim.x + threadIdx.x;
    if (t < 8 && zero_a) zero_a[t] = 0u;
    if (t == 8 && zero_b) *zero_b = 0u;
    const uint32_t q = t / PREP_LANES, sub = t % PREP_LANES;
    if (q >= nq) return;
    prep_group(ix, items_flat, q_off, q, sub, m, max_len, out + (size_t)q * stride, loc_table, loc_mask, okeys);
}

#ifndef SRN_GEN_PRIO_LEVELS
#define SRN_GEN_PRIO_LEVELS 2013
#endif
#define GEN_PRIO(ph) do { if (SRN_GEN_PRIO_LEVELS) __builtin_amdgcn_s_setprio((short)(((SRN_GEN_PRIO_LEVELS) / (ph)) % 10)); } while (0)
#ifndef SRN_STOP_AT
#define SRN_STOP_AT (-1)
#endif
#define SRN_TICK(ph)                                                                                         \
    do { if (ticking && tid == 0) { const long long t_ = clock64(); atomicAdd(&p.phase_cycles[ph], (unsigned long long)(t_ - t_prev)); t_prev = t_; } } while (0); \
    if (SRN_STOP_AT == (ph)) continue

template <int BLOCK, typename SlotT, bool GLOBAL_TABLES, int STAGE = 0, bool MASKS = false>
__global__ __launch_bounds__(BLOCK, 2 * BLOCK / 256) void vmis_predict_kernel(DeviceIndex ix_arg, LaunchParams p_arg, KernelCfg c_arg, LaunchAux aux_arg, ShardIO sh_arg) {
    extern __shared__ __attribute__((aligned(16))) char smem[];
    typedef const __attribute__((address_space(4))) char* KArg;
    const KArg ka = (KArg)__builtin_amdgcn_kernarg_segment_ptr();
    constexpr size_t OFF_P = (sizeof(DeviceIndex) + alignof(LaunchParams) - 1) / alignof(LaunchParams) * alignof(LaunchParams);
    constexpr size_t OFF_C = (OFF_P + sizeof(LaunchParams) + alignof(KernelCfg) - 1) / alignof(KernelCfg) * alignof(KernelCfg);
    const __attribute__((address_space(4))) DeviceIndex& ix = *(const __attribute__((address_space(4))) DeviceIndex*)ka;
    const __attribute__((address_space(4))) LaunchParams& p = *(const __attribute__((address_space(4))) LaunchParams*)(ka + OFF_P);
    const __attribute__((address_space(4))) KernelCfg& c = *(const __attribute__((address_space(4))) KernelCfg*)(ka + OFF_C);
    constexpr size_t OFF_X = (OFF_C + sizeof(KernelCfg) + alignof(LaunchAux) - 1) / alignof(LaunchAux) * alignof(LaunchAux);
    constexpr size_t OFF_S = (OFF_X + sizeof(LaunchAux) + alignof(ShardIO) - 1) / alignof(ShardIO) * alignof(ShardIO);
    const __attribute__((address_space(4))) LaunchAux& aux = *(const __attribute__((address_space(4))) LaunchAux*)(ka + OFF_X);
    const __attribute__((address_space(4))) ShardIO& sh = *(const __attribute__((address_space(4))) ShardIO*)(ka + OFF_S);
    const int tid = threadIdx.x, lane = tid & 63, wave = tid >> 6;
    constexpr int NWAVES = BLOCK / 64;
    constexpr SlotT SEMPTY = SlotTraits<SlotT>::EMPTY;

    uint32_t* misc = (uint32_t*)smem;
    uint64_t* q_raw = (uint64_t*)(smem + c.off_q);
    unsigned long long* l_base = (unsigned long long*)(q_raw + c.q_cap);
    uint32_t* q_idx = (uint32_t*)(l_base + c.q_cap);
    uint32_t* l_len = q_idx + c.q_cap;
    uint32_t* l_pre = l_len + c.q_cap;
    char* region_b = smem + c.off_b;
    uint32_t* hist = (uint32_t*)region_b;
    char* region_a = GLOBAL_TABLES ? (aux.gscratch + (size_t)blockIdx.x * aux.gscratch_stride) : (smem + c.off_a);

    SlotT* stab = (SlotT*)region_a;
    uint32_t* hot = (uint32_t*)region_a;
    uint32_t* sketch = hot + c.hot_slots;
    uint32_t* ikeys = sketch + c.sketch_slots;
    int* iacc = (int*)(ikeys + c.item_slots);
    SlotT* nbl = (SlotT*)region_b;
    SlotT* nb_spill = aux.nb_spill ? (SlotT*)aux.nb_spill + (size_t)blockIdx.x * p.k : nullptr;
    uint64_t* ckey = (uint64_t*)region_b;
    uint32_t* cidx = (uint32_t*)(region_b + CAND_CAP * 8);

    const uint32_t NB = c.num_bits;
    const SlotT num_mask = ((SlotT)1 << NB) - 1;
// ... 914 lines not shown
            if (GLOBAL_TABLES || (STAGE == 3 && aux.retry_list == nullptr)) { if (tid == 0) { p.out_counts[q] = 0xFFFFFFFFu; if (p.stats) p.stats[(size_t)q * 8 + 7] = 3; } }
            else if (tid == 0) aux.retry_list[atomicAdd(aux.retry_cnt, 1u)] = q;
            continue;
        }
        const uint32_t n_res = min(misc[S_CCNT], n_out);
        if (tid < n_res) {
            p.out_ids[(size_t)q * n_out + tid] = ix.id_sorted[cidx[tid]];
            p.out_scores[(size_t)q * n_out + tid] = key_score(ckey[tid]);
        }
        if (tid == 0) {
            p.out_counts[q] = n_res;
            if (p.nb_cnt) p.nb_cnt[q] = K;
            if (p.stats) { uint32_t* st = p.stats + (size_t)q * 8;
                st[0] = P; st[1] = Cm; st[2] = K; st[3] = misc[S_I]; st[4] = d_total; st[5] = n_res; st[6] = L;
                st[7] = misc[S_ERR] ? 4u : (GLOBAL_TABLES ? 1u : (parts > 1 ? 0x100u * parts : 0u)); }
        }
    }
}


template <int BLOCK, bool GLOBAL_TABLES, int STAGE = 0, bool MASKS = false>
static hipError_t launch_variant(const PredictLaunch& a, dim3 grid, size_t lds, hipStream_t st, const DeviceIndex& di, const LaunchParams& p, const KernelCfg& c) {
#define SRN_LAUNCH(SLOT)                                                                                             \
    do {                                                                                                                  \
        auto kern = vmis_predict_kernel<BLOCK, SLOT, GLOBAL_TABLES, STAGE, MASKS>;                                           \
        hipError_t e = hipFuncSetAttribute((const void*)kern, hipFuncAttributeMaxDynamicSharedMemorySize, (int)lds);     \
        if (e != hipSuccess) return e;                                                                                    \
        hipLaunchKernelGGL(kern, grid, dim3(BLOCK), lds, st, di, p, c, LaunchAux{a.qlist, a.qn, a.retry_list, a.retry_cnt, a.gscratch, a.gstride, a.spill}, a.sh); \
        return hipGetLastError();                                                                                         \
    } while (0)
    if (!a.slot64) SRN_LAUNCH(uint32_t);
    SRN_LAUNCH(unsigned long long);
#undef SRN_LAUNCH
}

hipError_t launch_predict(const PredictLaunch& a, dim3 grid, size_t lds, hipStream_t st, const DeviceIndex& di, const LaunchParams& p, const KernelCfg& c) {
    const bool masks = a.masks; const int stage = a.stage;
#define SRN_V(G, S, M) launch_variant<kBlock, G, S, M>(a, grid, lds, st, di, p, c)
    if (a.global_tables) {
        if (stage != 0) return masks ? hipErrorInvalidValue : stage == 1 ? SRN_V(true, 1, false) : stage == 2 ? SRN_V(true, 2, false) : stage == 3 ? SRN_V(true, 3, false) : hipErrorInvalidValue;
        return masks ? SRN_V(true, 0, true) : SRN_V(true, 0, false);
    }
    switch (stage) {
        case 0: return masks ? SRN_V(false, 0, true) : SRN_V(false, 0, false);
        case 1: return masks ? SRN_V(false, 1, true) : SRN_V(false, 1, false);
        case 2: return masks ? SRN_V(false, 2, true) : SRN_V(false, 2, false);
        case 3: return masks ? SRN_V(false, 3, true) : SRN_V(false, 3, false);
        default: return hipErrorInvalidValue;
    }
#undef SRN_V
}

hipError_t launch_prep(hipStream_t st, const DeviceIndex& di, const uint64_t* items_flat, const uint32_t* q_off, uint32_t nq, uint32_t m,
                       uint32_t max_len, char* out, uint32_t stride, uint32_t* zero_a, uint32_t* zero_b, const IdSlot* loc_table, uint32_t loc_mask, unsigned long long* okeys) {
    static_assert(sizeof(PrepHead) == 72 && sizeof(PrepItem) == 24, "vmis_prep_kernel writes the record word by word");
    const uint32_t per_block = 256 / PREP_LANES;
    hipLaunchKernelGGL(vmis_prep_kernel, dim3((nq + per_block - 1) / per_block), dim3(256), 0, st, di, items_flat, q_off, nq, m, max_len, out, stride, zero_a, zero_b, loc_table, loc_mask, okeys);
    return hipGetLastError();
}

hipError_t launch_rows_to_frags(hipStream_t st, const uint64_t* row_off, const uint32_t* row_items, uint64_t n_rows, const uint32_t* block_base,
                                uint32_t* slots, uint32_t* ext) {
    hipLaunchKernelGGL(rows_to_frags_kernel, dim3((unsigned)((n_rows + 1 + 1023) / 1024)), dim3(1024), 0, st, row_off, row_items, n_rows, block_base, slots, ext);
    return hipGetLastError();
}

hipError_t launch_rows_to_slots(hipStream_t st, const uint64_t* row_off, const uint32_t* row_items, uint64_t n_rows, const uint32_t* block_base,
                                uint32_t* slots, uint32_t* ext) {
    hipLaunchKernelGGL(rows_to_slots_kernel, dim3((unsigned)((n_rows + 1 + 1023) / 1024)), dim3(1024), 0, st, row_off, row_items, n_rows, block_base, slots, ext);
    return hipGetLastError();
}

__global__ __launch_bounds__(512) void class_counts_debug_kernel(const unsigned long long* __restrict__ acc, uint32_t n_waves, uint32_t* __restrict__ out16) {
    const uint32_t gt = blockIdx.x * 512u + threadIdx.x, w = gt >> 6, lane = threadIdx.x & 63u;
    const unsigned long long a = w < n_waves ? acc[gt] : 0ull;
    const uint32_t c = wave_class_counts(a, lane);
    if (w < n_waves && lane < 16u) out16[(size_t)w * 16u + lane] = c;
}

int device_debug_class_counts(const uint64_t* acc, size_t n_waves, uint32_t* out16, int device) {
    if (!acc || !out16) return fail(SRN_EINVAL, "null buffer");
    if (n_waves == 0) return SRN_OK;
    if (n_waves > (1u << 20)) return fail(SRN_ERANGE, "srn_debug_class_counts: at most 2^20 waves");
    int prev_device = 0;
    HIP_TRY(hipGetDevice(&prev_device));
    HIP_TRY(hipSetDevice(device));
    struct Restore { int d; ~Restore() { (void)hipSetDevice(d); } } restore{prev_device};
    void* mem = nullptr;
    const size_t in_bytes = n_waves * 64 * 8, out_bytes = n_waves * 16 * 4;
    if (hipMalloc(&mem, in_bytes + out_bytes) != hipSuccess) { (void)hipGetLastError(); return fail(SRN_ENOMEM, "srn_debug_class_counts: hipMalloc failed"); }
    unsigned long long* d_acc = (unsigned long long*)mem; uint32_t* d_out = (uint32_t*)((char*)mem + in_bytes);
    hipError_t e = hipMemcpy(d_acc, acc, in_bytes, hipMemcpyHostToDevice);
    if (e == hipSuccess) {
        hipLaunchKernelGGL(class_counts_debug_kernel, dim3((unsigned)((n_waves + 7) / 8)), dim3(512), 0, 0, d_acc, (uint32_t)n_waves, d_out);
        e = hipGetLastError();
    }
    if (e == hipSuccess) e = hipMemcpy(out16, d_out, out_bytes, hipMemcpyDeviceToHost);
    (void)hipFree(mem);
    if (e != hipSuccess) return fail(SRN_EHIP, std::string("srn_debug_class_counts: ") + hipGetErrorString(e));
    return SRN_OK;
}

}
```

### serenade_amd/csrc/srn_latency.hip

```cpp
#include <hip/hip_runtime.h>

#include <algorithm>
#include <atomic>
#include <chrono>
#include <cstdio>
#include <cstring>
#include <memory>
#include <mutex>
#include <string>
#include <vector>

#include "srn_runtime.h"
#include "srn_hipsync.h"

namespace srn {


struct TinyPin { Bump::Region<uint64_t> items{}, ids{}; Bump::Region<double> sc{}; Bump::Region<uint32_t> qoff{}, cnt{}, rc{}, rl{}; char* dp = nullptr; };
static int tiny_stage(Workspace* w, LaunchParams& p, const uint64_t* h_items, const uint32_t* h_qoff, TinyPin& t) {
    const size_t nitems = h_qoff[p.nq], n_out = (size_t)p.nq * p.how_many;
    Bump b(64);
    t.items = b.take<uint64_t>(nitems * 8); t.qoff = b.take<uint32_t>(((size_t)p.nq + 1) * 4); t.ids = b.take<uint64_t>(n_out * 8); t.sc = b.take<double>(n_out * 8); t.cnt = b.take<uint32_t>((size_t)p.nq * 4);
    t.rc = b.take<uint32_t>(4); t.rl = b.take<uint32_t>((size_t)p.nq * 4 + 4);
    const size_t off = b.bytes;
// ... 64 lines not shown
                               (unsigned long long)c, (unsigned long long)second.load(), (unsigned long long)why[0].load(), (unsigned long long)why[1].load(), (unsigned long long)why[2].load());
}
static int tiny_fused(TinyCall& c, const uint64_t* h_items, const uint32_t* h_qoff) {
    Workspace* w = c.w; const LaunchParams& p = c.p; FastParams& fp = c.fp;
    uint32_t L1 = 0; for (uint32_t q = 0; q < p.nq; ++q) L1 = std::max(L1, h_qoff[q + 1] - h_qoff[q]);
    if (w->cnt_dirty) HIP_TRY(hipMemsetAsync(w->slow_cnt, 0, sizeof(SlowCntBlock), c.st));
    w->cnt_dirty = true;
    fp.tiny_len = p.nq == 1 && L1 >= 1u && L1 <= 8u ? L1 : 0u;
    for (uint32_t i = 0; i < fp.tiny_len; ++i) fp.tiny_items[i] = h_items[h_qoff[0] + i];
    uint32_t seq = ++w->tiny_seq; if (seq == 0u) seq = ++w->tiny_seq;
    fp.host_seq = seq; fp.host_words = w->h_retry_dev;
    HIP_TRY(launch_fast(c.plan.mid_tier && L1 > 4u ? FastForm::TinyMid : FastForm::Tiny, dim3(p.nq), c.st, c.d->di, p, fp, c.kn.debug));
    fp.host_words = nullptr; fp.tiny_len = 0;
    const volatile uint32_t* hw = w->h_retry;
    bool seen = false;
    if (!c.blocking_wait && !c.kn.no_tiny_spin) {
        const auto t0 = std::chrono::steady_clock::now();
        for (uint32_t spin = 0; !seen; ++spin) {
            seen = hw[HW_SEQ] == seq;
            if (!seen) {
                __builtin_ia32_pause();
                if ((spin & 1023u) == 1023u && std::chrono::steady_clock::now() - t0 > std::chrono::milliseconds(5)) break;
            }
        }
        std::atomic_thread_fence(std::memory_order_acquire);
    }
    if (!seen) { int rc = latency_wait(w, c.st, c.blocking_wait); if (rc) return rc; }
    if (hw[HW_SEQ] != seq) { int rc = tiny_rest(c); return rc ? rc : latency_wait(w, c.st, c.blocking_wait); }
    const uint32_t n_slow = hw[HW_GENERAL], n_mid = hw[HW_MID], n_big = hw[HW_OVER63];
    if (c.kn.debug) tiny_fused_stats(n_slow, n_mid, n_big);
    if ((n_slow | n_mid | n_big) == 0u) { w->cnt_dirty = false; return SRN_OK; }
    int rc = SRN_OK;
    if (n_mid == 0u) {
        if (n_slow) rc = tiny_general(c, true, std::min<uint32_t>(p.nq, n_slow));
        if (!rc && n_big) rc = tiny_finish_big(c);
    }
    else rc = tiny_rest(c);
    return rc ? rc : latency_wait(w, c.st, c.blocking_wait);
}

int device_predict_tiny(DeviceState* d, const FlatIndex& ix, Workspace* w, const Geometry& geo, LaunchParams p, const uint64_t* h_items, const uint32_t* h_qoff,
                        uint64_t* h_ids, double* h_scores, uint32_t* h_counts, bool blocking_wait) {
    TinyPin pin; { int rc = tiny_stage(w, p, h_items, h_qoff, pin); if (rc) return rc; }
    hipStream_t st = w->stream;
    const size_t cap_q = std::max<size_t>(p.nq, (size_t)std::max(1, knobs().tiny_max));
    { int rc = ensure(&w->spill, &w->spill_bytes, cap_q * p.k * geo.slot_bytes); if (rc) return rc; }
    const uint32_t prep_stride = prep_stride_of(p.max_len);
    { int rc = ensure(&w->prep, &w->prep_bytes, cap_q * prep_stride); if (rc) return rc; }
    const Knobs kn = knobs();
    const FastPlan plan = fast_plan(d, ix, p, geo, kn, false);
    const bool tiny_fast = plan.fast && (kn.tiny_fast == 3 || (kn.tiny_fast >= 1 && p.max_len > 8) || (kn.tiny_fast == 2 && p.nq <= (kn.no_tiny_fused ? 32u : (uint32_t)kn.tiny_fused_max)));
    if (tiny_fast) { int rc = reserve_fast(w, cap_q); if (rc) return rc; }
    const bool fused = tiny_fast && p.nq <= (uint32_t)kn.tiny_fused_max && !kn.no_tiny_fused;
    if (!fused) { w->cnt_dirty = true; HIP_TRY(launch_prep(st, d->di, p.items_flat, p.q_off, p.nq, p.m, p.max_len, w->prep, prep_stride, tiny_fast ? w->slow_cnt : nullptr)); }
    p.prep = w->prep; p.prep_stride = prep_stride;
    TinyCall c{d, w, geo, p, plan, kn, pin, st, blocking_wait};
    int rc = SRN_OK;
    if (fused) { c.fp = fast_params(d, w, plan, cap_q, plan.mid_tier ? TIER_MID : 0u); rc = tiny_fused(c, h_items, h_qoff); }
    else if (tiny_fast) {
        c.fp = fast_params(d, w, plan, cap_q, plan.mid_tier ? TIER_MID : 0u);
        HIP_TRY(launch_fast(FastForm::Lean, dim3(p.nq), st, d->di, p, c.fp, kn.debug));
        rc = tiny_rest(c);
        if (!rc) rc = latency_wait(w, st, blocking_wait);
    } else {
        rc = tiny_general(c, false, p.nq);
        if (!rc) rc = latency_wait(w, st, blocking_wait);
    }
    if (rc) return rc;
    if (*(volatile uint32_t*)pin.rc.at(w->pin) != 0) return 1;
    ++w->untimed_calls; w->last_nq = p.nq; w->last_retry = 0; w->last_fast = tiny_fast; w->last_mid = tiny_fast && plan.mid_tier; w->last_dedup = false; w->last_untimed = true;
    tiny_unstage(w, p, pin, h_ids, h_scores, h_counts);
    return SRN_OK;
}


struct ServeForm {
    DeviceState* d = nullptr; bool mid = false; std::atomic<bool> dead{false}; uint32_t n = 0;
    hipStream_t st = nullptr;
    ServeCtl* ctl = nullptr; ServeCtl* ctl_dev = nullptr;
    char* rows = nullptr; char* rows_dev = nullptr; size_t row_bytes = 0;
    char *prep = nullptr, *fin = nullptr, *big = nullptr; uint32_t *slow_list = nullptr, *slow_cnt = nullptr, *counts = nullptr;
    LaunchParams p{}; FastParams fp{};
    std::unique_ptr<std::atomic<int>[]> busy; std::vector<uint32_t> seq;
    std::mutex mu; bool running = false;
};
struct ServeState {
    std::vector<ServeForm*> forms; uint32_t k = 0, m = 0, how_many = 0, flags = 0, max_items = 0; unsigned long long idle_ticks = 0;
    std::atomic<uint64_t> served{0}, not_served{0}, launches{0};
};
static std::mutex g_serve_mu; static std::vector<ServeForm*> g_serve_forms; static std::atomic<int> g_serve_running{0};

static void lane_lock(ServeForm* f, uint32_t i) { int e = 0; while (!f->busy[i].compare_exchange_weak(e, 1, std::memory_order_acquire)) { e = 0; __builtin_ia32_pause(); } }
static void lane_unlock(ServeForm* f, uint32_t i) { f->busy[i].store(0, std::memory_order_release); }
static void form_park(ServeForm* f) {
    if (!f->running) return;
    for (uint32_t i = 0; i < f->n; ++i) lane_lock(f, i);
    int cur = 0; (void)hipGetDevice(&cur);
    if (cur != f->d->device) (void)hipSetDevice(f->d->device);
    for (uint32_t i = 0; i < f->n; ++i) __atomic_store_n(&f->ctl[i].stop, 1u, __ATOMIC_RELEASE);
    (void)hipStreamSynchronize(f->st);
    if (cur != f->d->device) (void)hipSetDevice(cur);
    f->running = false; g_serve_running.fetch_sub(1);
    for (uint32_t i = 0; i < f->n; ++i) lane_unlock(f, i);
}
static std::atomic<int> g_serve_hold{0};
void serve_hold_begin() { g_serve_hold.fetch_add(1, std::memory_order_acq_rel); serve_quiesce_all(); }
void serve_hold_end() { g_serve_hold.fetch_sub(1, std::memory_order_acq_rel); }
// ... 150 lines not shown
```

### serenade_amd/csrc/srn_prep.h

```cpp
#pragma once
#include <hip/hip_runtime.h>

#include "srn_device.h"
#include "srn_kernels.h"

namespace srn {

static constexpr uint32_t PREP_LANES = 8;
__device__ __forceinline__ void prep_group(const DeviceIndex& ix, const uint64_t* __restrict__ items_flat, const uint32_t* __restrict__ q_off, uint32_t q, uint32_t sub, uint32_t m, uint32_t max_len,
                                           char* rec, const IdSlot* __restrict__ loc_table, uint32_t loc_mask, unsigned long long* __restrict__ okeys) {
    const uint32_t qb = q_off[q], L = q_off[q + 1] - qb;
    PrepItem* items = (PrepItem*)(rec + sizeof(PrepHead));
    uint32_t U = 0, rmax = 0, xlo = 0, sumw = 0, P = 0, nruns = 0, n_staged = 0, cur_attr = SRN_ATTR_NONE, my_run_start = 0;
    const bool ok = L != 0 && L <= max_len;
    const uint32_t rounds = ok ? (L + PREP_LANES - 1) / PREP_LANES : 0;
    uint32_t vmax = 0;
    uint32_t hot_key2 = kNone;
    uint32_t hot_key = kNone;
    uint32_t idx = kNone, len = 0, pre = 0; unsigned long long base = 0;
    for (uint32_t r = 0; r < rounds; ++r) {
        const uint32_t pos = r * PREP_LANES + sub;
        const bool have = pos < L;
        idx = kNone; len = 0; base = 0;
        uint32_t first_i = 0, head_rank = 0, mth_rank = 0;
        if (have) {
            const uint64_t raw = items_flat[qb + (L - 1 - pos)];
            bool first = true;
            for (uint32_t j = 0; j < pos; ++j) first = first && (items_flat[qb + (L - 1 - j)] != raw);
            { uint32_t hh = (uint32_t)dev_mix64(raw) & ix.id_mask;
              for (;;) { const IdSlot s = ix.id_table[hh]; if (s.idx == kNone) break; if (s.key == raw) { idx = s.idx; break; } hh = (hh + 1) & ix.id_mask; } }
            if (idx < hot_key) { hot_key2 = hot_key; hot_key = idx; } else if (idx != hot_key) hot_key2 = min(hot_key2, idx);
            if (ix.viol != nullptr && idx != kNone) vmax = max(vmax, ix.viol[idx]);
            first_i = first ? 1u : 0u;
            if (first && idx != kNone) {
                const unsigned long long o0 = ix.post_off[idx], o1 = ix.post_off[idx + 1];
                len = (uint32_t)min((unsigned long long)m, o1 - o0); base = o0;
                if (len) { head_rank = ix.post_rank[o0]; if (len >= m) mth_rank = ix.post_rank[o0 + m - 1]; }
            }
            if (pos == 0 && idx != kNone) cur_attr = ix.meta[idx].attr;
            if (loc_table) {
                idx = kNone;
                uint32_t hh = (uint32_t)dev_mix64(raw) & loc_mask;
                for (;;) { const IdSlot s2 = loc_table[hh]; if (s2.idx == kNone) break; if (s2.key == raw) { idx = s2.idx; break; } hh = (hh + 1) & loc_mask; }
            }
        }
        uint32_t sc_len = len, sc_run = len ? 1u : 0u;
        #pragma unroll
        for (uint32_t d = 1; d < PREP_LANES; d <<= 1) {
            const uint32_t a = __shfl_up(sc_len, d, PREP_LANES), b2 = __shfl_up(sc_run, d, PREP_LANES);
            if (sub >= d) { sc_len += a; sc_run += b2; }
        }
        uint32_t u = first_i, rm = head_rank, xl = mth_rank, sw = len ? L - pos : 0u;
        #pragma unroll
        for (uint32_t d = 1; d < PREP_LANES; d <<= 1) {
            u += __shfl_xor(u, d, PREP_LANES); sw += __shfl_xor(sw, d, PREP_LANES);
            rm = max(rm, __shfl_xor(rm, d, PREP_LANES)); xl = max(xl, __shfl_xor(xl, d, PREP_LANES));
        }
        pre = P + sc_len - len;
        const uint32_t run_idx = nruns + sc_run - (len ? 1u : 0u);
        #pragma unroll
        for (uint32_t s = 0; s < PREP_LANES; ++s) {
            const uint32_t rp = __shfl(pre, s, PREP_LANES), ri = __shfl(run_idx, s, PREP_LANES), rl = __shfl(len, s, PREP_LANES);
            if (rl != 0u && ri == sub) my_run_start = rp;
        }
        U += u; sumw += sw; rmax = max(rmax, rm); xlo = max(xlo, xl);
        P += __shfl(sc_len, PREP_LANES - 1, PREP_LANES); nruns += __shfl(sc_run, PREP_LANES - 1, PREP_LANES);
        if (have && rounds > 1) items[pos] = PrepItem{idx, len, pre, 0u, base};
    }
    for (uint32_t r = 0; r < rounds; ++r) {
        const uint32_t pos = r * PREP_LANES + sub;
        const bool have = pos < L;
        uint32_t kept = 0;
        if (have) {
            if (rounds > 1) { len = items[pos].len; base = items[pos].base; }
            if (len != 0) {
                const uint32_t* __restrict__ lst = ix.post_rank + base;
                uint32_t lo = 0, hi = len;
                if (xlo == 0u || lst[len - 1] >= xlo) lo = len;
                while (hi - lo > 8u) {
                    const uint32_t w = hi - lo;
                    uint32_t b[7], v[7];
#pragma unroll
                    for (uint32_t j = 0; j < 7u; ++j) { b[j] = lo + (uint32_t)(((unsigned long long)w * (j + 1u)) >> 3); v[j] = lst[b[j]]; }
                    uint32_t c = 0;
#pragma unroll
                    for (uint32_t j = 0; j < 7u; ++j) c += v[j] >= xlo ? 1u : 0u;
                    uint32_t nlo = lo, nhi = hi;
#pragma unroll
                    for (uint32_t j = 0; j < 7u; ++j) { if (c == j + 1u) nlo = b[j] + 1u; if (c == j) nhi = b[j]; }
                    lo = nlo; hi = nhi;
                }
                {
                    uint32_t v[8], c = 0;
#pragma unroll
                    for (uint32_t j = 0; j < 8u; ++j) v[j] = lst[min(lo + j, len - 1u)];
#pragma unroll
                    for (uint32_t j = 0; j < 8u; ++j) c += lo + j < hi && v[j] >= xlo ? 1u : 0u;
                    lo += c; hi = lo;
                }
                kept = lo;
            }
            if (rounds > 1) items[pos].kept = kept; else items[pos] = PrepItem{idx, len, pre, kept, base};
        }
        uint32_t ks = kept;
        #pragma unroll
        for (uint32_t d = 1; d < PREP_LANES; d <<= 1) ks += __shfl_xor(ks, d, PREP_LANES);
        n_staged += ks;
    }
    cur_attr = __shfl(cur_attr, 0, PREP_LANES);
    #pragma unroll
    for (uint32_t d = 1; d < PREP_LANES; d <<= 1) {
        const uint32_t o1 = (uint32_t)__shfl_xor((int)hot_key, d, PREP_LANES), o2 = (uint32_t)__shfl_xor((int)hot_key2, d, PREP_LANES);
        hot_key2 = o1 == hot_key ? min(hot_key2, o2) : min(max(hot_key, o1), min(hot_key2, o2));
        hot_key = min(hot_key, o1);
        vmax = max(vmax, (uint32_t)__shfl_xor((int)vmax, d, PREP_LANES));
    }
    const uint32_t unsafe = vmax > xlo ? 1u : 0u;
#ifndef SRN_ORDER_KEY2
#define SRN_ORDER_KEY2 0
#endif
    if (okeys && sub == 0) okeys[q] = SRN_ORDER_KEY2 ? ((unsigned long long)min(hot_key, 0xFFFFu) << 40) | ((unsigned long long)min(hot_key2 >> 4, 0xFFu) << 32) | q :
                                      ((unsigned long long)min(hot_key, 0xFFFFu) << 32) | q;
    uint32_t* hw = (uint32_t*)rec;
    if (sub == 0) {
        *(uint2*)hw = make_uint2(U, rmax); *(uint2*)(hw + 2) = make_uint2(xlo, sumw); *(uint2*)(hw + 4) = make_uint2(P, nruns); *(uint2*)(hw + 6) = make_uint2(L, n_staged);
        *(uint2*)(hw + 16) = make_uint2(cur_attr, unsafe);
    }
    hw[8 + sub] = sub < nruns ? my_run_start : 0u;
}

}
```

### serenade_amd/csrc/srn_runtime.hip

```cpp
#include <hip/hip_runtime.h>

#include <chrono>

#include <algorithm>
#include <climits>
#include <cstdio>
#include <cstdlib>
#include <cstring>
#include <memory>
#include <mutex>
#include <string>
#include <vector>

#include "srn_runtime.h"
#include "srn_hipsync.h"

namespace srn {

static Knobs g_knobs; static std::once_flag g_knobs_once; static std::mutex g_knobs_mu;
static bool env_flag(const char* name) { return getenv(name) != nullptr; }
static int env_int(const char* name, int unset, int lo = INT_MIN, int hi = INT_MAX) { const char* e = getenv(name); return e ? std::min(hi, std::max(lo, atoi(e))) : unset; }
static void knobs_read() {
    Knobs k;
    k.fast_how_many_max = env_int("SRN_FAST_HOW_MANY_MAX", k.fast_how_many_max, 1, 64);
// ... 303 lines not shown
    g.slot_bytes = g.slot64 ? 8 : 4;
    const uint32_t slot_bytes = g.slot_bytes;
    const uint64_t m_eff = std::min<uint64_t>(p.m, ix.m_index);
    g.need_sess = std::max<uint64_t>(1, std::min<uint64_t>(Lmax * m_eff, ix.n_kept));
    g.need_item = std::max<uint64_t>(1, std::min<uint64_t>((uint64_t)p.k * std::max<uint64_t>(1, ix.max_row_len), ix.n_items));
    KernelCfg& c = g.c;
    c.num_bits = (uint32_t)num_bits;
    c.q_cap = round_up((uint32_t)Lmax + 1, 4);
    c.off_q = MISC_WORDS * 4 + 1024;
    c.off_wave = round_up(c.off_q + c.q_cap * 24 + (c.q_cap + 4) * 4, 16);
    c.off_b = c.off_wave;
    const uint32_t region_b = round_up(std::max<uint32_t>(std::max<uint32_t>(p.k * slot_bytes, CAND_CAP * 12), min_region_b), 16);
    c.off_a = c.off_b + region_b;
    const uint32_t lds_max = (uint32_t)std::min(d->lds_per_block_max, 160 * 1024);
    uint32_t budget = 80 * 1024;
    if (kn.lds_budget_kb) budget = (uint32_t)kn.lds_budget_kb * 1024;
    if (c.off_a + 32 * 1024 > budget) budget = lds_max;
    if (c.off_a + 8 * 1024 > budget) return fail(SRN_ERANGE, "k / session length too large for the LDS layout");
    const uint32_t a_max = budget - c.off_a;
    c.sess_slots = std::min<uint32_t>(floor_pow2(a_max / slot_bytes), (uint32_t)std::min<uint64_t>(1u << 30, ceil_pow2(g.need_sess * 2)));
    c.sess_slots = std::max<uint32_t>(c.sess_slots, 256);
    const uint64_t w_abs = g.masks ? 9 : std::max<uint64_t>(9, std::min<uint64_t>(Lmax, 99) > 10 ? std::min<uint64_t>(Lmax, 99) - 10 : 0);
    const uint64_t w_max = (uint64_t)p.k * w_abs * (Lmax * (Lmax + 1) / 2) + 1;
    {
        uint64_t wn_max = 0;
        for (uint64_t q = 1; q <= std::min<uint64_t>(Lmax, 99); ++q) {
            const uint64_t wq = q <= 10 ? 10 - q : q - 10, nq_ = (Lmax - q + 1) * (Lmax - q + 2) / 2;
            wn_max = std::max(wn_max, wq * nq_);
        }
        if ((uint64_t)p.k * wn_max >= (1ull << 31))
            return fail(SRN_ERANGE, "k * |10 * linear_score| * similarity numerator can exceed the 32-bit item accumulators at this k and session length: lower k or max_items_in_session");
        g.sketch_may_wrap = sketch_wraps(p.k, ix.max_row_len, Lmax);
    }
    const int sbits = std::max(2, bits_host(w_max) + 1), cbits = bits_host(p.k);
    uint32_t hot = sbits + cbits <= 32 ? (p.k >= 1024 ? 4096u : 2048u) : 0u;
    if (kn.hot_slots >= 0) hot = sbits + cbits <= 32 ? (uint32_t)kn.hot_slots : 0u;
    hot = std::min<uint32_t>(std::min<uint32_t>(hot, a_max / 8), round_up((uint32_t)std::min<uint64_t>(ix.n_items, 1u << 20), 4)) / 4 * 4;
    c.hot_slots = hot; c.sum_bits = (uint32_t)sbits;
    uint32_t sk = hot && !g.sketch_may_wrap ? 8192u : 0u;
    if (kn.sketch_slots >= 0) sk = hot && !g.sketch_may_wrap && kn.sketch_slots > 0 ? floor_pow2((uint64_t)kn.sketch_slots) : 0u;
    while (sk && (uint64_t)sk * 4 * 8 > (uint64_t)(a_max - hot * 4) * 5) sk >>= 1;
    c.sketch_slots = sk; c.sketch_shift = sk ? 32u - (uint32_t)(bits_host(sk) - 1) : 31u;
    const uint64_t want_buckets = std::max<uint64_t>(61, g.need_item / 2 + 8);
    c.item_buckets = prime_at_most((uint32_t)std::min<uint64_t>((a_max - hot * 4 - sk * 4) / 32, want_buckets));
    c.item_slots = c.item_buckets * 4;
    const uint32_t region_a = std::max<uint32_t>(hot * 4 + sk * 4 + c.item_slots * 8, c.sess_slots * slot_bytes);
    c.region_a_bytes = region_a;
    c.no_merge = kn.no_merge ? 1u : 0u;
    g.lds = (size_t)c.off_a + region_a;
    g.sess_may_overflow = (uint64_t)c.sess_slots < g.need_sess * 2; g.item_may_overflow = (uint64_t)c.item_slots < g.need_item * 2;
    return SRN_OK;
}

static uint32_t fast_nb(const FlatIndex& ix, const Knobs& kn) {
    const int rank_bits_f = std::max(1, bits_host(ix.n_kept ? ix.n_kept - 1 : 0));
    return kn.fast_runs == 3 && rank_bits_f <= 29 ? 3u : rank_bits_f <= 28 ? 4u : rank_bits_f <= 29 ? 3u : 0u;
}
FastPlan fast_plan(const DeviceState* d, const FlatIndex& ix, const LaunchParams& p, const Geometry& geo, const Knobs& kn, bool has_ext) {
    FastPlan f;
    f.nb_fast = fast_nb(ix, kn);
    const bool sets_exact = p.m <= ix.m_index && (ix.lists_complete || (d->di.viol != nullptr && !kn.no_viol)) && !kn.no_masks;
    const bool fast_sketch_ok = (uint64_t)p.k * std::max<uint64_t>(1, ix.max_row_len) * 9ull * (p.max_len > 10 ? 210ull : 55ull) < (1ull << 32);
    f.mid_tier = !kn.no_mid && !has_ext && d->di.row_frag == 0u && p.max_len >= 5;
    f.long_tier = f.mid_tier && !kn.no_long && !kn.no_big && p.max_len > 10;
    f.fast = d->fast.row_packed != nullptr && sets_exact && (p.max_len <= 8 ? (geo.masks || !ix.lists_complete) && !geo.sketch_may_wrap : f.mid_tier && fast_sketch_ok) && f.nb_fast != 0 && kn.geometry_default() &&
             !kn.no_fast && p.k <= F_K_MAX && p.m <= F_M_MAX && p.how_many <= (uint32_t)kn.fast_how_many_max && (p.flags & ~(unsigned)SRN_FLAG_BUSINESS_LOGIC) == 0 && p.stats == nullptr && p.nb_rank == nullptr;
    return f;
}

struct DedupRoom { uint32_t* n_dup = nullptr; uint32_t* rep = nullptr; uint32_t* slots = nullptr; uint32_t* slot_min = nullptr; uint32_t n_slots = 0; };
struct OrderBufs { unsigned long long* keys_in = nullptr; unsigned long long* keys_out = nullptr; void* temp = nullptr; size_t temp_bytes = 0; DedupRoom dd;
                   uint32_t* n_skip = nullptr; };
static int order_room(char** buf, size_t* have, uint32_t nq, OrderBufs* o, bool dedup = false, bool cache = false) {
    DedupRoom* dd = dedup ? &o->dd : nullptr;
    size_t tb = 0;
    if (sort_order_keys(nullptr, nullptr, nullptr, nq, nullptr, &tb) != hipSuccess) return fail(SRN_EHIP, "rocprim::radix_sort_keys (size query) failed");
    const size_t kb = ((size_t)nq * 8 + 255) / 256 * 256, tbr = (tb + 255) / 256 * 256;
    const size_t rb = ((size_t)nq * 4 + 255) / 256 * 256, n_slots = dd ? dedup_slots(nq) : 0;
    const size_t dd_bytes = dd ? 256 + rb + 2 * n_slots * 4 : 0;
    int rc = ensure(buf, have, 2 * kb + tbr + 256 + dd_bytes + (cache ? 256 + 256 : 0)); if (rc) return rc;
    o->keys_in = (unsigned long long*)*buf; o->keys_out = (unsigned long long*)(*buf + kb); o->temp = *buf + 2 * kb; o->temp_bytes = tb;
    if (dd) { char* b = *buf + 2 * kb + tbr + 256; dd->n_dup = (uint32_t*)b; dd->rep = (uint32_t*)(b + 256); dd->slots = (uint32_t*)(b + 256 + rb); dd->slot_min = dd->slots + n_slots; dd->n_slots = (uint32_t)n_slots; }
    if (cache) o->n_skip = (uint32_t*)(*buf + (2 * kb + tbr + 256 + dd_bytes + 255) / 256 * 256);
    return SRN_OK;
}

static int ensure_side(Workspace* w) {
    if (w->side) return SRN_OK;
    int lo = 0, hi = 0; (void)hipDeviceGetStreamPriorityRange(&lo, &hi);
    HIP_TRY(hipStreamCreateWithPriority(&w->side, hipStreamNonBlocking, hi));
    for (int i = 0; i < 2; ++i) { HIP_TRY(hipEventCreateWithFlags(&w->ev_prep[i], hipEventDisableTiming)); HIP_TRY(hipEventCreateWithFlags(&w->ev_done[i], hipEventDisableTiming)); }
    HIP_TRY(hipEventCreateWithFlags(&w->ev_fork, hipEventDisableTiming)); HIP_TRY(hipEventCreateWithFlags(&w->ev_join, hipEventDisableTiming));
    return SRN_OK;
}

static uint64_t fast_big_entries(size_t cap_q) { return std::min<uint64_t>(0x7FFFFFF0ull, (uint64_t)cap_q * 16 + 4096); }
int reserve_fast(Workspace* w, size_t cap_q) {
    { int rc = ensure_list(&w->slow_list, &w->slow_cap, cap_q, (cap_q * 4 + 64) * 4); if (rc) return rc; }
    { int rc = ensure(&w->fin, &w->fin_bytes, cap_q * F_FIN_BYTES + 1024); if (rc) return rc; }
    return ensure(&w->big, &w->big_bytes, fast_big_entries(cap_q) * 16 + cap_q * 4 + 64);
}
FastBuffers fast_buffers(const Workspace* w, size_t cap_q) { return FastBuffers{w->slow_list, w->slow_cap, w->slow_cnt, w->fin, w->big, fast_big_entries(cap_q)}; }
FastParams fast_params(const DeviceState* d, const FastBuffers& b, const FastPlan& plan, unsigned tiers) {
    FastParams fp = d->fast; fp.slow_list = b.slow_list; fp.slow_cnt = b.slow_cnt; fp.nb = plan.nb_fast; fp.max_runs = plan.nb_fast; fp.fin = b.fin;
    fp.big_arena = b.big; fp.big_list = b.big ? (uint32_t*)(b.big + b.big_entries * 16) : nullptr; fp.big_cap_entries = (uint32_t)b.big_entries;
    fp.big_ticket = b.slow_cnt ? (unsigned long long*)(b.slow_cnt + SC_BIG_TICKET_LO) : nullptr;
    fp.xchg = nullptr; fp.xchg_stride = 0; fp.q_base = 0; fp.order = nullptr;
    fp.mid_list = (tiers & TIER_MID) ? slow_part(b.slow_list, b.slow_cap, SL_MID) : nullptr; fp.mid_cnt = fp.mid_list ? b.slow_cnt + SC_MID : nullptr;
    fp.bigq_list = (tiers & TIER_BIGQ) ? slow_part(b.slow_list, b.slow_cap, SL_BIGQ) : nullptr; fp.bigq_cnt = fp.bigq_list ? b.slow_cnt + SC_BIGQ : nullptr;
    fp.long_list = (tiers & TIER_LONG) ? slow_part(b.slow_list, b.slow_cap, SL_LONG) : nullptr; fp.long_cnt = fp.long_list ? b.slow_cnt + SC_LONG : nullptr;
// ... 52 lines not shown
        rc = ensure_side(w); if (rc) return rc;
    }
    if (pl.fast.fast) { int rc = reserve_fast(w, p.nq); if (rc) return rc; }
    if (pl.ordered) return order_room(pl.order_set2 ? &w->order2 : &w->order, pl.order_set2 ? &w->order2_bytes : &w->order_bytes, p.nq, &ob, pl.dedup, pl.cache);
    return SRN_OK;
}

struct BatchCall {
    DeviceState* d; Workspace* w; const LaunchPlan& pl; const ExtLists* ext; hipStream_t st; DeviceIndex di; LaunchParams p; OrderBufs ob;
    hipEvent_t* ev = nullptr; bool timed = false, fork_retry = false;
    bool sback_second = false;
    FastParams fp{};
    ResultCache* rcache = nullptr; uint32_t cache_now = 0;
};

static int stage_host_inputs(Workspace* w, hipStream_t st, LaunchParams& p, const HostRows& h) {
    const bool stats = h.stats != nullptr, nb = h.nb_rank != nullptr;
    const size_t n_out = (size_t)p.nq * p.how_many, nitems = h.q_off[p.nq];
    Bump b;
    const auto r_items = b.take<const uint64_t>(nitems * 8); const auto r_qoff = b.take<const uint32_t>(((size_t)p.nq + 1) * 4);
    const auto r_ids = b.take<uint64_t>(n_out * 8); const auto r_sc = b.take<double>(n_out * 8); const auto r_cnt = b.take<uint32_t>((size_t)p.nq * 4);
    const auto r_st = b.take<uint32_t>(stats ? (size_t)p.nq * 32 : 0);
    const auto r_nr = b.take<uint32_t>(nb ? (size_t)p.nq * p.k * 4 : 0), r_nn = b.take<uint32_t>(nb ? (size_t)p.nq * p.k * 4 : 0), r_nc = b.take<uint32_t>(nb ? (size_t)p.nq * 4 : 0);
    int rc = ensure(&w->stage, &w->stage_bytes, b.bytes); if (rc) return rc;
    char* s = w->stage;
    p.items_flat = r_items.at(s); p.q_off = r_qoff.at(s);
    p.out_ids = r_ids.at(s); p.out_scores = r_sc.at(s); p.out_counts = r_cnt.at(s);
    p.stats = stats ? r_st.at(s) : nullptr;
    p.nb_rank = nb ? r_nr.at(s) : nullptr; p.nb_num = nb ? r_nn.at(s) : nullptr;
    p.nb_cnt = nb ? r_nc.at(s) : nullptr;
    HIP_TRY(hipMemsetAsync(p.out_ids, 0, n_out * 8, st));
    HIP_TRY(hipMemsetAsync(p.out_scores, 0, n_out * 8, st));
    HIP_TRY(hipMemcpyAsync((void*)p.items_flat, h.items, nitems * 8, hipMemcpyHostToDevice, st));
    HIP_TRY(hipMemcpyAsync((void*)p.q_off, h.q_off, ((size_t)p.nq + 1) * 4, hipMemcpyHostToDevice, st));
    return SRN_OK;
}
static int fetch_host_outputs(const BatchCall& c, const HostRows& h) {
    const LaunchParams& p = c.p; hipStream_t st = c.st; const size_t n_out = (size_t)p.nq * p.how_many;
    HIP_TRY(hipMemcpyAsync(h.ids, p.out_ids, n_out * 8, hipMemcpyDeviceToHost, st));
    HIP_TRY(hipMemcpyAsync(h.scores, p.out_scores, n_out * 8, hipMemcpyDeviceToHost, st));
    HIP_TRY(hipMemcpyAsync(h.counts, p.out_counts, (size_t)p.nq * 4, hipMemcpyDeviceToHost, st));
    if (h.stats) HIP_TRY(hipMemcpyAsync(h.stats, p.stats, (size_t)p.nq * 32, hipMemcpyDeviceToHost, st));
    if (h.nb_rank) {
        HIP_TRY(hipMemcpyAsync(h.nb_rank, p.nb_rank, (size_t)p.nq * p.k * 4, hipMemcpyDeviceToHost, st));
        HIP_TRY(hipMemcpyAsync(h.nb_num, p.nb_num, (size_t)p.nq * p.k * 4, hipMemcpyDeviceToHost, st));
        HIP_TRY(hipMemcpyAsync(h.nb_cnt, p.nb_cnt, (size_t)p.nq * 4, hipMemcpyDeviceToHost, st));
    }
    HIP_TRY(hipStreamSynchronize(st));
    return SRN_OK;
}

static int enqueue_front(BatchCall& c, hipStream_t s, char* rec) {
    const LaunchParams& p = c.p; const LaunchPlan& pl = c.pl; OrderBufs& ob = c.ob; Workspace* w = c.w;
    HIP_TRY(launch_prep(s, c.di, p.items_flat, p.q_off, p.nq, p.m, p.max_len, rec, pl.prep_stride, pl.prep_clears && pl.fast.fast ? w->slow_cnt : nullptr,
                        pl.prep_clears && pl.retry ? w->retry_cnt : nullptr, nullptr, 0, ob.keys_in));
    if (pl.dedup) {
        HIP_TRY(hipMemsetAsync(ob.dd.slots, 0xFF, (size_t)ob.dd.n_slots * 8, s));
        HIP_TRY(launch_dedup_group(s, p.items_flat, p.q_off, p.nq, ob.dd.slots, ob.dd.slot_min, ob.dd.n_slots, (uint32_t)pl.kn.dedup_hash_bits, ob.dd.rep, ob.keys_in, pl.prep_clears ? p.out_counts : nullptr, ob.dd.n_dup));
    }
    if (pl.cache) { int rc = rcache_enqueue_lookup(c.rcache, s, p, pl.dedup ? ob.dd.rep : nullptr, ob.keys_in, pl.dedup ? ob.dd.n_dup : nullptr, ob.n_skip, pl.kn.cache_hash_bits, &c.cache_now); if (rc) return rc; }
    if (pl.ordered) HIP_TRY(sort_order_keys(s, ob.keys_in, ob.keys_out, p.nq, ob.temp, &ob.temp_bytes));
    c.p.prep = rec; c.p.prep_stride = pl.prep_stride;
    return SRN_OK;
}
static int enqueue_front_resident(BatchCall& c) {
    Workspace* w = c.w; hipStream_t st = c.st;
    const int par = (int)(w->resident_calls & 1u);
    if (!w->rec_used[par] && w->calls > 0) { HIP_TRY(hipEventRecord(w->ev_done[par], st)); w->rec_used[par] = true; }
    if (w->rec_used[par]) HIP_TRY(hipStreamWaitEvent(w->side, w->ev_done[par], 0));
    { int rc = enqueue_front(c, w->side, par ? w->prep2 : w->prep); if (rc) return rc; }
    HIP_TRY(hipEventRecord(w->ev_prep[par], w->side));
    HIP_TRY(hipStreamWaitEvent(st, w->ev_prep[par], 0));
    if (c.pl.dedup) HIP_TRY(launch_dedup_mark(st, c.p.nq, c.ob.dd.rep, c.p.out_counts));
    return SRN_OK;
}
static int enqueue_shard_front(BatchCall& c) {
    const ExtLists* ext = c.ext; LaunchParams& p = c.p;
    if (ext->q_lo >= p.nq) return SRN_OK;
    p.prep = ext->prep; p.prep_stride = c.pl.prep_stride;
    FastParams fp = fast_params(c.d, FastBuffers{}, c.pl.fast);
    fp.xchg = ext->xchg; fp.xchg_stride = ext->xchg_stride; fp.q_base = ext->q_lo;
    const uint64_t cnt = p.nq - ext->q_lo, res_wg = (uint64_t)c.d->n_cu * F_WG_PER_CU;
    const uint32_t grid_front = (uint32_t)std::min<uint64_t>(cnt, std::min<uint64_t>(res_wg * 64, std::max<uint64_t>(res_wg * 16, cnt / 12)));
    HIP_TRY(launch_fast(FastForm::Front, dim3(grid_front), c.st, c.di, p, fp, c.pl.kn.debug));
    return SRN_OK;
}
static int enqueue_shard_back(BatchCall& c) {
    DeviceState* d = c.d; Workspace* w = c.w; const ExtLists* ext = c.ext; const LaunchParams& p = c.p; const Knobs& kn = c.pl.kn; FastParams& fp = c.fp;
    SBackParams sbp = d->sback;
    const bool stream = ext->positions;
    if (stream && !(d->sb_frag_post && d->sb_post_for == ext->post_rank)) return fail(SRN_ESTATE, "the batch's neighbours came as posting positions, but this shard does not hold its fragments in posting order");
    const uint64_t slots = (uint64_t)d->n_cu * (stream ? 9 : 12);
    uint32_t grid_b = (uint32_t)std::min<uint64_t>(p.nq, slots * (kn.grid_mult_set ? (uint32_t)kn.grid_mult : stream ? 4 : 16));
    if (fp.order) grid_b = std::max<uint32_t>(8u, grid_b / 8u * 8u);
    if (stream) {
        int rc = ensure(&w->sb_scr, &w->sb_scr_bytes, (size_t)grid_b * shard_back_scratch_words() * 4); if (rc) return rc;
        sbp.frag_post = (const uint2*)d->sb_frag_post; sbp.post_rank = ext->post_rank; sbp.scr = (uint32_t*)w->sb_scr;
    }
    const bool second = !kn.no_sback_second && !stream; c.sback_second = second;
    if (second) { fp.mid_list = slow_part(w->slow_list, w->slow_cap, SL_MID); fp.mid_cnt = w->slow_cnt + SC_MID; }
    HIP_TRY(launch_shard_back(dim3(grid_b), c.st, c.di, p, fp, sbp, kn.debug));
    d->sback_launches.fetch_add(1, std::memory_order_relaxed);
    if (second) {
        FastParams fl = fp; fl.order = nullptr;
        HIP_TRY(launch_fast(FastForm::Back, dim3((uint32_t)std::min<uint64_t>(p.nq, (uint64_t)d->n_cu * F_WG_PER_CU * 4)), c.st, c.di, p, fl, kn.debug));
        fp.mid_list = nullptr; fp.mid_cnt = nullptr;
    }
// ... 187 lines not shown
        HIP_TRY(hipMemsetAsync(w->retry_cnt, 0, 4, st));
    }
    PredictLaunch a; a.masks = geo.masks; a.slot64 = geo.slot64; a.stage = stage; a.sh = sh;
    if (w) { a.retry_list = w->retry_list; a.retry_cnt = w->retry_cnt; }
    e = launch_predict(a, dim3(grid), geo.lds, st, d->di, p, geo.c);
    if (e != hipSuccess) return fail(SRN_EHIP, std::string("shard stage launch: ") + hipGetErrorString(e));
    if (retry) {
        PredictLaunch g; g.slot64 = geo.slot64; g.global_tables = true; g.stage = stage; g.sh = sh; g.qlist = w->retry_list; g.qn = w->retry_cnt; g.gscratch = w->gscratch; g.gstride = g_stride;
        e = launch_predict(g, dim3(retry_blocks), geo.c.off_a, st, d->di, p, cg);
        if (e != hipSuccess) return fail(SRN_EHIP, std::string("shard stage launch (global tables): ") + hipGetErrorString(e));
    }
    return SRN_OK;
}
bool device_shard_lists_supported(DeviceState* d, const FlatIndex& ix, const LaunchParams& p) {
    Geometry g;
    return make_geometry(d, ix, p, 0, g) == SRN_OK && g.masks && (p.flags & ~(unsigned)SRN_FLAG_BUSINESS_LOGIC) == 0 && p.stats == nullptr && p.nb_rank == nullptr;
}
bool device_fast_eligible(DeviceState* d, const FlatIndex& ix, const LaunchParams& p, uint64_t max_row_len_all) {
    Geometry geo;
    if (make_geometry(d, ix, p, 0, geo) != SRN_OK) return false;
    const Knobs kn = knobs();
    const int rank_bits_f = std::max(1, bits_host(ix.n_kept ? ix.n_kept - 1 : 0));
    const bool wraps = max_row_len_all ? sketch_wraps(p.k, std::max<uint64_t>(max_row_len_all, ix.max_row_len), p.max_len) : geo.sketch_may_wrap;
    return (max_row_len_all != 0 || d->fast.row_packed != nullptr) && geo.masks && !wraps && rank_bits_f <= 29 && kn.geometry_default() && !kn.no_fast && p.k <= F_K_MAX && p.m <= F_M_MAX &&
           p.how_many <= 24 && (p.flags & ~(unsigned)SRN_FLAG_BUSINESS_LOGIC) == 0 && p.stats == nullptr && p.nb_rank == nullptr && p.max_len <= 8;
}
uint32_t device_prep_stride(uint32_t max_len) { return prep_stride_of(max_len); }
int device_shard_lists_head(DeviceState* d, const LaunchParams& p, void* pos, int* head, void* stream) {
    HIP_TRY(hipSetDevice(d->device));
    if (p.nq == 0) return SRN_OK;
    HIP_TRY(launch_shard_lists_head((hipStream_t)stream, d->di, p.items_flat, p.q_off, p.nq, p.m, p.max_len, (ShardPos*)pos, head));
    return SRN_OK;
}
int device_shard_lists_count(DeviceState* d, const LaunchParams& p, const void* pos, const int* head, uint32_t* kept, int* tot, void* stream) {
    HIP_TRY(hipSetDevice(d->device));
    if (p.nq == 0) return SRN_OK;
    HIP_TRY(launch_shard_lists_count((hipStream_t)stream, d->di, p.q_off, p.nq, p.max_len, (const ShardPos*)pos, head, kept, tot));
    return SRN_OK;
}
int device_shard_lists_copy(DeviceState* d, const LaunchParams& p, const void* pos, const uint32_t* kept, const long long* off, uint32_t* out, void* stream) {
    HIP_TRY(hipSetDevice(d->device));
    if (p.nq == 0) return SRN_OK;
    HIP_TRY(launch_shard_lists_copy((hipStream_t)stream, d->di, p.nq, p.max_len, (const ShardPos*)pos, kept, off, out));
    return SRN_OK;
}
int device_shard_lists_predict(DeviceState* d, const FlatIndex& ix, const LaunchParams& p, uint32_t n_shards, const uint32_t* kept_g, const long long* off_g,
                               unsigned long long shard_stride, const uint32_t* lists_g, const int* head, const void* pos_local, char* records, void* stream,
                               const unsigned long long* shard_base, bool direct) {
    HIP_TRY(hipSetDevice(d->device));
    if (p.nq == 0) return SRN_OK;
    if (n_shards != ix.n_shards) return fail(SRN_EINVAL, "n_shards differs from the number of shards this index was cut into");
    if (!device_shard_lists_supported(d, ix, p)) return fail(SRN_EINVAL, "lists mode needs position-set slots (sessions of <= 8 items, m <= m_index, complete lists): use the three-stage pipeline");
    const uint32_t stride = device_prep_stride(p.max_len);
    HIP_TRY(launch_shard_prep((hipStream_t)stream, p.items_flat, p.q_off, p.nq, p.max_len, n_shards, kept_g, off_g, shard_stride, head, (const ShardPos*)pos_local, records, stride, shard_base, direct));
    ExtLists ext{records, stride, direct ? d->di.post_rank : lists_g};
    return predict_ext(d, ix, p, stream, ext);
}

int device_shard_nb_prep(DeviceState* d, DeviceState* post, const LaunchParams& p, char* records, void* stream, char** order_buf, size_t* order_bytes, const unsigned long long** order_out) {
    HIP_TRY(hipSetDevice(d->device));
    if (order_out) *order_out = nullptr;
    if (p.nq == 0) return SRN_OK;
    const Knobs kn = knobs();
    const bool ordered = order_buf && kn.order_min > 0 && p.nq >= (uint32_t)kn.order_min;
    OrderBufs ob;
    if (ordered) { int rc = order_room(order_buf, order_bytes, p.nq, &ob); if (rc) return rc; }
    HIP_TRY(launch_prep((hipStream_t)stream, post->di, p.items_flat, p.q_off, p.nq, p.m, p.max_len, records, device_prep_stride(p.max_len), nullptr, nullptr, d->di.id_table, d->di.id_mask, ob.keys_in));
    if (ordered) { HIP_TRY(sort_order_keys((hipStream_t)stream, ob.keys_in, ob.keys_out, p.nq, ob.temp, &ob.temp_bytes)); *order_out = ob.keys_out; }
    return SRN_OK;
}
int device_shard_nb_front(DeviceState* d, const FlatIndex& ix, DeviceState* post, const LaunchParams& p_in, const char* records, uint32_t* xchg, uint32_t xchg_stride, uint32_t q_lo, uint32_t q_hi, void* stream) {
    if (q_lo >= q_hi) return SRN_OK;
    LaunchParams p = p_in; p.nq = q_hi;
    ExtLists ext{records, device_prep_stride(p.max_len), post->di.post_rank, 1, xchg, xchg_stride, q_lo};
    return predict_ext(d, ix, p, stream, ext);
}
int device_shard_nb_positions(DeviceState* d, const FlatIndex& ix, DeviceState* post, const LaunchParams& p, const char* records, const uint32_t* xin, uint32_t in_stride, uint32_t* xout, uint32_t out_stride,
                              uint32_t q_lo, uint32_t q_hi, void* stream) {
    if (q_lo >= q_hi) return SRN_OK;
    HIP_TRY(hipSetDevice(d->device));
    const uint32_t grid = (uint32_t)std::min<uint64_t>(q_hi - q_lo, (uint64_t)d->n_cu * 16 * 4);
    HIP_TRY(launch_shard_nb_positions(dim3(grid), (hipStream_t)stream, records, device_prep_stride(p.max_len), p.max_len, xin, in_stride, xout, out_stride, post->di.post_rank, q_lo, q_hi, p.m,
                                      fast_nb(ix, knobs()) == 3u));
    return SRN_OK;
}
uint32_t device_shard_nb_positions_stride(const LaunchParams& p) {
    const Knobs kn = knobs();
    if (kn.no_sback_stream || kn.no_sback || p.max_len > 8) return 0u;
    return shard_nb_positions_stride(p.k, p.m);
}
int device_shard_nb_back(DeviceState* d, const FlatIndex& ix, DeviceState* post, const LaunchParams& p, const char* records, uint32_t* xchg, uint32_t xchg_stride, void* stream, const unsigned long long* order, bool positions) {
    if (p.nq == 0) return SRN_OK;
    ExtLists ext{records, device_prep_stride(p.max_len), post->di.post_rank, 2, xchg, xchg_stride, 0u, order, positions};
    return predict_ext(d, ix, p, stream, ext);
}

int device_slot_bytes(DeviceState* d, const FlatIndex& ix, uint32_t max_len, uint32_t* num_bits) {
    const LaunchParams p = launch_params(0, 1, 1, 0, 0, max_len); Geometry g;
    if (make_geometry(d, ix, p, 0, g) != SRN_OK) return -1;
    if (num_bits) *num_bits = g.c.num_bits;
    return (int)g.slot_bytes;
}

int device_last_kernel_ms(DeviceState* d, double* ms_main, double* ms_retry, uint32_t* retried) {
    HIP_TRY(hipSetDevice(d->device));
    Workspace* w;
    { std::lock_guard<std::mutex> lk(d->mu); w = d->last_ws; }
    if (!w || !(w->calls + w->untimed_calls)) return fail(SRN_EINVAL, "no timed predict call yet");
    if (w->last_untimed) return fail(SRN_EINVAL, "the last call took the latency path (<= 256 sessions on host pointers): it records no events");
    if (!w->ring_timed[(w->calls - 1) % Workspace::RING]) return fail(SRN_EINVAL, "kernel timing is off: srn_kernel_timing(idx, 1) before the calls to be timed");
    hipEvent_t* ev = w->ev[(w->calls - 1) % Workspace::RING];
    HIP_TRY(hipEventSynchronize(ev[2]));
    float a = 0, b = 0;
    HIP_TRY(hipEventElapsedTime(&a, ev[3], ev[1]));
    HIP_TRY(hipEventElapsedTime(&b, ev[1], ev[2]));
    if (ms_main) *ms_main = a;
    if (ms_retry) *ms_retry = b;
    if (retried) *retried = w->last_retry ? w->h_retry[HW_GLOBAL] : 0;
    return SRN_OK;
}

int device_reserve(DeviceState* d, const FlatIndex& ix, const LaunchParams& p, void* stream) {
    CallKind kind; kind.stream = stream; kind.reserve_only = true;
    return predict_core(d, ix, p, kind);
}

int device_last_path_counts(DeviceState* d, uint32_t* nq, uint32_t* general, uint32_t* global_pass) {
    HIP_TRY(hipSetDevice(d->device));
    Workspace* w;
    { std::lock_guard<std::mutex> lk(d->mu); w = d->last_ws; }
    if (!w || !(w->calls + w->untimed_calls)) return fail(SRN_EINVAL, "no predict call yet");
    if (!w->last_untimed) HIP_TRY(hipEventSynchronize(w->ev[(w->calls - 1) % Workspace::RING][2]));
    if (nq) *nq = w->last_nq;
    if (general) *general = w->last_fast ? w->h_retry[HW_GENERAL] : w->last_nq;
    if (global_pass) *global_pass = w->last_retry ? w->h_retry[HW_GLOBAL] : 0;
    return SRN_OK;
}
int device_last_mid_count(DeviceState* d, uint32_t* listed, uint32_t* big_listed) {
    uint32_t nq = 0;
    const int rc = device_last_path_counts(d, &nq, nullptr, nullptr);
    if (rc != SRN_OK) return rc;
    Workspace* w;
    { std::lock_guard<std::mutex> lk(d->mu); w = d->last_ws; }
    if (listed) *listed = w->last_fast && w->last_mid ? w->h_retry[HW_MID] : 0u;
    if (big_listed) *big_listed = w->last_fast ? w->h_retry[HW_BIGQ] : 0u;
    return SRN_OK;
}

int device_last_dedup_count(DeviceState* d, uint32_t* merged) {
    const int rc = device_last_path_counts(d, nullptr, nullptr, nullptr);
    if (rc != SRN_OK) return rc;
    Workspace* w;
    { std::lock_guard<std::mutex> lk(d->mu); w = d->last_ws; }
    if (merged) *merged = w->last_dedup ? w->h_retry[HW_MERGED] : 0u;
    return SRN_OK;
}

int device_kernel_timing(DeviceState* d, int enable) { d->timing.store(enable != 0, std::memory_order_relaxed); return SRN_OK; }

int device_phase_cycles(DeviceState* d, int enable, unsigned long long* out16) {
    HIP_TRY(hipSetDevice(d->device));
    HIP_TRY(hipDeviceSynchronize());
    if (!d->d_phase) { HIP_TRY(hipMalloc((void**)&d->d_phase, 16 * 8)); d->allocs.push_back(d->d_phase); HIP_TRY(hipMemset(d->d_phase, 0, 16 * 8)); }
    if (out16) HIP_TRY(hipMemcpy(out16, d->d_phase, 16 * 8, hipMemcpyDeviceToHost));
    HIP_TRY(hipMemset(d->d_phase, 0, 16 * 8));
    d->phase_on = enable != 0;
    return SRN_OK;
}

int device_kernel_times(DeviceState* d, uint32_t max_n, double* ms_main, double* ms_retry, uint32_t* out_n, double* ms_prep, double* ms_fast) {
    HIP_TRY(hipSetDevice(d->device));
    Workspace* w;
    { std::lock_guard<std::mutex> lk(d->mu); w = d->last_ws; }
    *out_n = 0;
    if (!w || !w->calls) return SRN_OK;
    uint64_t n = std::min<uint64_t>(std::min<uint64_t>(max_n, w->calls), Workspace::RING);
    { uint64_t timed = 0; while (timed < n && w->ring_timed[(w->calls - 1 - timed) % Workspace::RING]) ++timed; n = timed; }
    if (!n) return SRN_OK;
    HIP_TRY(hipEventSynchronize(w->ev[(w->calls - 1) % Workspace::RING][2]));
    for (uint64_t i = 0; i < n; ++i) {
        hipEvent_t* ev = w->ev[(w->calls - n + i) % Workspace::RING];
        float a = 0, b = 0;
        HIP_TRY(hipEventElapsedTime(&a, ev[3], ev[1]));
        HIP_TRY(hipEventElapsedTime(&b, ev[1], ev[2]));
        if (ms_main) ms_main[i] = a;
        if (ms_retry) ms_retry[i] = b;
        if (ms_prep) { float c2 = 0; HIP_TRY(hipEventElapsedTime(&c2, ev[0], ev[3])); ms_prep[i] = c2; }
        if (ms_fast) { float c2 = 0; HIP_TRY(hipEventElapsedTime(&c2, ev[3], ev[4])); ms_fast[i] = c2; }
// ... 7 lines not shown
```

### serenade_amd/csrc/srn_shard.hip

```cpp
#include <hip/hip_runtime.h>

#include <cstdlib>

#include "srn_device.h"
#include "srn_kernels.h"

namespace srn {

__global__ __launch_bounds__(256) void shard_lists_head_kernel(DeviceIndex ix, const uint64_t* __restrict__ items_flat, const uint32_t* __restrict__ q_off,
                                                               uint32_t nq, uint32_t m, uint32_t max_len, ShardPos* __restrict__ pos_out, int* __restrict__ head) {
    const uint32_t q = blockIdx.x * blockDim.x + threadIdx.x;
    if (q >= nq) return;
    const uint32_t qb = q_off[q], L = q_off[q + 1] - qb;
    uint32_t xlo = 0, rmax = 0; int attr = -1;
    ShardPos* const out = pos_out + (size_t)q * max_len;
    if (L != 0 && L <= max_len) {
        for (uint32_t pos = 0; pos < L; ++pos) {
            const uint64_t raw = items_flat[qb + (L - 1 - pos)];
            bool first = true;
            for (uint32_t j = 0; j < pos; ++j) first = first && (items_flat[qb + (L - 1 - j)] != raw);
            uint32_t idx = kNone;
            { uint32_t hh = (uint32_t)dev_mix64(raw) & ix.id_mask;
              for (;;) { const IdSlot s = ix.id_table[hh]; if (s.idx == kNone) break; if (s.key == raw) { idx = s.idx; break; } hh = (hh + 1) & ix.id_mask; } }
            uint32_t len = 0; unsigned long long base = 0;
            if (first && idx != kNone) {
                const unsigned long long o0 = ix.post_off[idx], o1 = ix.post_off[idx + 1];
                len = (uint32_t)min((unsigned long long)m, o1 - o0); base = o0;
                if (len) { rmax = max(rmax, ix.post_rank[o0]); if (len >= m) xlo = max(xlo, ix.post_rank[o0 + m - 1]); }
            }
            if (pos == 0 && idx != kNone) attr = (int)ix.meta[idx].attr;
            out[pos] = ShardPos{idx, len, base};
        }
    }
    head[3 * (size_t)q] = (int)xlo; head[3 * (size_t)q + 1] = (int)rmax; head[3 * (size_t)q + 2] = attr;
}

__global__ __launch_bounds__(256) void shard_lists_count_kernel(DeviceIndex ix, const uint32_t* __restrict__ q_off, uint32_t nq, uint32_t max_len,
                                                                const ShardPos* __restrict__ pos_in, const int* __restrict__ head,
                                                                uint32_t* __restrict__ kept, int* __restrict__ tot) {
    const uint32_t q = blockIdx.x * blockDim.x + threadIdx.x;
    if (q >= nq) return;
    const uint32_t L = q_off[q + 1] - q_off[q], xlo = (uint32_t)head[3 * (size_t)q];
    uint32_t total = 0;
    for (uint32_t pos = 0; pos < max_len; ++pos) {
        uint32_t lo = 0;
        if (L != 0 && L <= max_len && pos < L) {
            const ShardPos sp = pos_in[(size_t)q * max_len + pos];
            if (sp.len) {
                const uint32_t* __restrict__ lst = ix.post_rank + sp.base;
                uint32_t hi = sp.len;
                while (lo < hi) { const uint32_t mid = (lo + hi) >> 1; if (lst[mid] >= xlo) lo = mid + 1; else hi = mid; }
            }
        }
        kept[(size_t)q * max_len + pos] = lo; total += lo;
    }
    tot[q] = (int)total;
}

__global__ __launch_bounds__(256) void shard_lists_copy_kernel(DeviceIndex ix, uint32_t nq, uint32_t max_len, const ShardPos* __restrict__ pos_in,
                                                               const uint32_t* __restrict__ kept, const long long* __restrict__ off, uint32_t* __restrict__ out) {
    const uint32_t q = blockIdx.x * (blockDim.x >> 6) + (threadIdx.x >> 6), lane = threadIdx.x & 63u;
    if (q >= nq) return;
    uint32_t* dst = out + off[q];
    for (uint32_t pos = 0; pos < max_len; ++pos) {
        const uint32_t n = kept[(size_t)q * max_len + pos];
        if (n == 0) continue;
        const uint32_t* __restrict__ src = ix.post_rank + pos_in[(size_t)q * max_len + pos].base;
        for (uint32_t e = lane; e < n; e += 64u) dst[e] = src[e];
        dst += n;
    }
}

__global__ __launch_bounds__(256) void shard_prep_kernel(const uint64_t* __restrict__ items_flat, const uint32_t* __restrict__ q_off, uint32_t nq, uint32_t max_len,
                                                         uint32_t n_shards, const uint32_t* __restrict__ kept_g, const long long* __restrict__ off_g,
                                                         unsigned long long shard_stride, const unsigned long long* __restrict__ shard_base, const int* __restrict__ head,
                                                         const ShardPos* __restrict__ pos_local, char* __restrict__ out, uint32_t stride, bool direct) {
    const uint32_t q = blockIdx.x * blockDim.x + threadIdx.x;
    if (q >= nq) return;
    const uint32_t qb = q_off[q], L = q_off[q + 1] - qb;
    PrepHead h{0u, 0u, 0u, 0u, 0u, 0u, L, 0u, {0u, 0u, 0u, 0u, 0u, 0u, 0u, 0u}, SRN_ATTR_NONE, 0u};
    PrepItem* items = (PrepItem*)(out + (size_t)q * stride + sizeof(PrepHead));
    if (L != 0 && L <= max_len) {
        h.xlo = (uint32_t)head[3 * (size_t)q]; h.rmax = (uint32_t)head[3 * (size_t)q + 1];
        if (head[3 * (size_t)q + 2] >= 0) h.cur_attr = (uint32_t)head[3 * (size_t)q + 2];
        for (uint32_t pos = 0; pos < L; ++pos) {
            const uint64_t raw = items_flat[qb + (L - 1 - pos)];
            bool first = true;
            for (uint32_t j = 0; j < pos; ++j) first = first && (items_flat[qb + (L - 1 - j)] != raw);
            if (first) ++h.U;
            uint32_t kp = 0; unsigned long long base = 0;
            for (uint32_t g = 0; g < n_shards; ++g) {
                const uint32_t* kq = kept_g + ((size_t)g * nq + q) * max_len;
                if (kq[pos] == 0) continue;
                unsigned long long before = 0;
                for (uint32_t j = 0; j < pos; ++j) before += kq[j];
                kp = kq[pos];
                if (direct) base = pos_local[(size_t)q * max_len + pos].base;
                else base = (shard_base ? shard_base[g] : (unsigned long long)g * shard_stride) + (unsigned long long)off_g[(size_t)g * nq + q] + before;
                break;
            }
            if (kp) { h.sumw += L - pos; if (h.nruns < 8) h.run_start[h.nruns] = h.P; ++h.nruns; }
            items[pos] = PrepItem{pos_local[(size_t)q * max_len + pos].idx, kp, h.P, kp, base};
            h.P += kp;
        }
        h.n_staged = h.P;
    }
    *(PrepHead*)(out + (size_t)q * stride) = h;
}

hipError_t launch_shard_lists_head(hipStream_t st, const DeviceIndex& di, const uint64_t* items_flat, const uint32_t* q_off, uint32_t nq, uint32_t m, uint32_t max_len,
                                   ShardPos* pos_out, int* head) {
    hipLaunchKernelGGL(shard_lists_head_kernel, dim3((nq + 255) / 256), dim3(256), 0, st, di, items_flat, q_off, nq, m, max_len, pos_out, head);
    return hipGetLastError();
}
hipError_t launch_shard_lists_count(hipStream_t st, const DeviceIndex& di, const uint32_t* q_off, uint32_t nq, uint32_t max_len, const ShardPos* pos_in, const int* head,
                                    uint32_t* kept, int* tot) {
    hipLaunchKernelGGL(shard_lists_count_kernel, dim3((nq + 255) / 256), dim3(256), 0, st, di, q_off, nq, max_len, pos_in, head, kept, tot);
    return hipGetLastError();
}
hipError_t launch_shard_lists_copy(hipStream_t st, const DeviceIndex& di, uint32_t nq, uint32_t max_len, const ShardPos* pos_in, const uint32_t* kept, const long long* off,
                                   uint32_t* out) {
    hipLaunchKernelGGL(shard_lists_copy_kernel, dim3((nq + 3) / 4), dim3(256), 0, st, di, nq, max_len, pos_in, kept, off, out);
    return hipGetLastError();
}
hipError_t launch_shard_prep(hipStream_t st, const uint64_t* items_flat, const uint32_t* q_off, uint32_t nq, uint32_t max_len, uint32_t n_shards, const uint32_t* kept_g,
                             const long long* off_g, unsigned long long shard_stride, const int* head, const ShardPos* pos_local, char* out, uint32_t stride,
                             const unsigned long long* shard_base, bool direct) {
    hipLaunchKernelGGL(shard_prep_kernel, dim3((nq + 255) / 256), dim3(256), 0, st, items_flat, q_off, nq, max_len, n_shards, kept_g, off_g, shard_stride, shard_base, head, pos_local,
                       out, stride, direct);
    return hipGetLastError();
}


__global__ __launch_bounds__(256) void shard_max_kernel(int* __restrict__ dst, const int* __restrict__ src, size_t n) {
    const size_t i = (size_t)blockIdx.x * blockDim.x + threadIdx.x;
    if (i < n) dst[i] = max(dst[i], src[i]);
}
hipError_t launch_shard_max(hipStream_t st, int* dst, const int* src, size_t n) {
    if (n) hipLaunchKernelGGL(shard_max_kernel, dim3((unsigned)((n + 255) / 256)), dim3(256), 0, st, dst, src, n);
    return hipGetLastError();
}

constexpr uint32_t OFFS_CHUNK = 1024;
__device__ __forceinline__ unsigned long long row_sum(const uint32_t* __restrict__ kq, uint32_t max_len) {
    unsigned long long v = 0; for (uint32_t j = 0; j < max_len; ++j) v += kq[j]; return v;
}
__global__ __launch_bounds__(1024) void shard_offsets_sum_kernel(const uint32_t* __restrict__ kept_g, uint32_t nq, uint32_t max_len, uint32_t nchunks,
                                                                 unsigned long long* __restrict__ chunk_tot) {
    __shared__ unsigned long long wsum[16];
    const uint32_t g = blockIdx.y, c = blockIdx.x, q = c * OFFS_CHUNK + threadIdx.x, lane = threadIdx.x & 63u, wave = threadIdx.x >> 6;
    unsigned long long v = q < nq ? row_sum(kept_g + ((size_t)g * nq + q) * max_len, max_len) : 0ull;
    for (int d = 32; d >= 1; d >>= 1) v += __shfl_xor(v, d);
    if (lane == 0u) wsum[wave] = v;
    __syncthreads();
    if (threadIdx.x == 0) { unsigned long long t = 0; for (int w = 0; w < 16; ++w) t += wsum[w]; chunk_tot[(size_t)g * nchunks + c] = t; }
}
__global__ __launch_bounds__(1024) void shard_offsets_scan_kernel(unsigned long long* __restrict__ chunk_tot, uint32_t nchunks, unsigned long long* __restrict__ tot_dev,
                                                                  unsigned long long* __restrict__ tot_host) {
    __shared__ unsigned long long part[1024];
    const uint32_t g = blockIdx.x, t = threadIdx.x;
    unsigned long long* ct = chunk_tot + (size_t)g * nchunks;
    const uint32_t per = (nchunks + 1023u) / 1024u, c0 = min(t * per, nchunks), c1 = min(c0 + per, nchunks);
    unsigned long long sum = 0; for (uint32_t c = c0; c < c1; ++c) sum += ct[c];
    part[t] = sum;
    __syncthreads();
    for (uint32_t d = 1; d < 1024u; d <<= 1) { const unsigned long long v = t >= d ? part[t - d] : 0ull; __syncthreads(); part[t] += v; __syncthreads(); }
    unsigned long long run = part[t] - sum;
    for (uint32_t c = c0; c < c1; ++c) { const unsigned long long v = ct[c]; ct[c] = run; run += v; }
    if (t == 1023u) { tot_dev[g] = part[1023]; if (tot_host) tot_host[g] = part[1023]; }
}
__global__ __launch_bounds__(1024) void shard_offsets_write_kernel(const uint32_t* __restrict__ kept_g, uint32_t nq, uint32_t max_len, uint32_t nchunks,
                                                                   const unsigned long long* __restrict__ chunk_base, long long* __restrict__ off_g) {
    __shared__ unsigned long long wsum[16];
    const uint32_t g = blockIdx.y, c = blockIdx.x, q = c * OFFS_CHUNK + threadIdx.x, lane = threadIdx.x & 63u, wave = threadIdx.x >> 6;
    const unsigned long long v = q < nq ? row_sum(kept_g + ((size_t)g * nq + q) * max_len, max_len) : 0ull;
    unsigned long long inc = v;
    for (int d = 1; d < 64; d <<= 1) { const unsigned long long o = __shfl_up(inc, d); if ((int)lane >= d) inc += o; }
    if (lane == 63u) wsum[wave] = inc;
    __syncthreads();
    unsigned long long before = chunk_base[(size_t)g * nchunks + c];
    for (uint32_t w = 0; w < wave; ++w) before += wsum[w];
    if (q < nq) off_g[(size_t)g * nq + q] = (long long)(before + inc - v);
// ... 194 lines not shown
```

Baseline: 56.19 million queries/s.

## Precompute per-query ready words in prep records to skip in-kernel list decode

The prep stage now writes a 16-word 'ready' block into each PrepHead. It holds a fits/flags word, a per-run load mask, the current item index, list positions, kept counts and 64-bit bases. In the common non-MID path the fast predict kernel reads these words with one lane-indexed load plus readlane instead of ballot, ffs and the fits checks. The goal is less per-query setup latency in the front phase. The parked prefetch size is tightened to the record length, and a debug entry point dumps prep records. The cost is a larger prep record and more prep-kernel work, and kernel correctness now depends on prep and kernel agreeing on the record layout and the wide/NB flag.

```diff
diff --git a/include/serenade_hip_internal.h b/include/serenade_hip_internal.h
--- a/include/serenade_hip_internal.h
+++ b/include/serenade_hip_internal.h
@@ -36,6 +36,9 @@
 #define SRN_DEBUG_MERGE_ROOM 12032
 int srn_debug_merge_pair(uint32_t* room, const uint32_t* pairs, size_t n_pairs, int device);
 
+int srn_debug_prep_records(const srn_index_t* idx, const uint64_t* items_flat, const uint32_t* q_off, size_t nq, size_t m, size_t max_len, void* out_records, size_t cap_bytes,
+                           size_t* out_stride);
+
 void srn_debug_reload_knobs(void);
 
 #ifdef __cplusplus
diff --git a/serenade_amd/capi.py b/serenade_amd/capi.py
--- a/serenade_amd/capi.py
+++ b/serenade_amd/capi.py
@@ -219,6 +219,7 @@
     "srn_debug_serve_stamps": (_i, [_vp, _vp]),
     "srn_debug_shard_nb_positions_stride": (C.c_uint32, [_sz, _sz]),
     "srn_debug_last_big_count": (_i, [_vp, C.POINTER(C.c_uint32)]),
+    "srn_debug_prep_records": (_i, [_vp, _vp, _vp, _sz, _sz, _sz, _vp, _sz, C.POINTER(_sz)]),
     "srn_debug_sback_launches": (_i, [_vp, C.POINTER(_u64)]),
     "srn_last_path_counts": (_i, [_vp, C.POINTER(C.c_uint32), C.POINTER(C.c_uint32), C.POINTER(C.c_uint32)]),
     "srn_eval_set_create": (_i, [_vp, _vp, _vp, _sz, _vp, _vp, _sz, C.POINTER(_vp)]),
diff --git a/serenade_amd/csrc/srn_capi.cpp b/serenade_amd/csrc/srn_capi.cpp
--- a/serenade_amd/csrc/srn_capi.cpp
+++ b/serenade_amd/csrc/srn_capi.cpp
@@ -661,6 +661,10 @@
 int srn_debug_last_mid_count(const srn_index_t* idx, uint32_t* out_listed) {
     if (!idx || !idx->dev) return fail(SRN_ENODEV, "index has no device attached");
     return guarded([&]() -> int { return device_last_mid_count(idx->dev, out_listed); });
+}
+int srn_debug_prep_records(const srn_index_t* idx, const uint64_t* items_flat, const uint32_t* q_off, size_t nq, size_t m, size_t max_len, void* out_records, size_t cap_bytes, size_t* out_stride) {
+    if (!idx || !idx->dev) return fail(SRN_ENODEV, "index has no device attached");
+    return guarded([&]() -> int { return device_debug_prep_records(idx->dev, idx->flat, items_flat, q_off, nq, m, max_len, out_records, cap_bytes, out_stride); });
 }
 int srn_debug_last_dedup_count(const srn_index_t* idx, uint32_t* out_merged) {
     if (!idx || !idx->dev || !out_merged) return fail(SRN_EINVAL, "null argument");
diff --git a/serenade_amd/csrc/srn_fast.hip b/serenade_amd/csrc/srn_fast.hip
--- a/serenade_amd/csrc/srn_fast.hip
+++ b/serenade_amd/csrc/srn_fast.hip
@@ -308,6 +308,7 @@
     static_assert(!BIG || MID, "BIG is a form of MID"); static_assert(!LONG || BIG, "LONG is a form of BIG");
     constexpr uint32_t SIDF = BIG ? F_BIG_TOTAL - (F_TOTAL - F_SIDF) : F_SIDF, SATTR = SIDF + 512 * 8;
     constexpr uint32_t MW = (SIDF - F_WORK) / 4;
+    static_assert(BIG || MW == F_LEAN_MW, "the prep record's lean_ok (ready_words, srn_prep.h) is evaluated for the 53 KB layout's merge room");
     __shared__ __attribute__((aligned(16))) char smem[BIG ? F_BIG_TOTAL : F_TOTAL];
 #else
     extern __shared__ __attribute__((aligned(16))) char smem[];
@@ -331,8 +332,8 @@
         const uint32_t alen = f.tiny_len;
         if (f.serve == nullptr) {
         if (alen) { if (tid < 8u) a_items[tid] = f.tiny_items[tid]; if (tid == 0u) { a_off[0] = 0u; a_off[1] = alen; } __syncthreads(); }
-        if (tid < PREP_LANES) prep_group(ix_arg, alen ? (const uint64_t*)a_items : p.items_flat, alen ? (const uint32_t*)a_off : p.q_off, alen ? 0u : blockIdx.x, tid, p.m, p.max_len,
-                                         const_cast<char*>(p.prep) + (size_t)blockIdx.x * p.prep_stride, nullptr, 0u, nullptr);
+        if (tid < PREP_LANES) prep_group<false>(ix_arg, alen ? (const uint64_t*)a_items : p.items_flat, alen ? (const uint32_t*)a_off : p.q_off, alen ? 0u : blockIdx.x, tid, p.m, p.max_len,
+                                         const_cast<char*>(p.prep) + (size_t)blockIdx.x * p.prep_stride, nullptr, 0u, nullptr, WIDE);
         __syncthreads();
         }
     }
@@ -368,7 +369,8 @@
     const uint32_t n_kept = ix.n_kept;
     auto qpos = [&](uint32_t pq) -> uint32_t { return ((wave + NW * (pq >> 6)) << 6) + (pq & 63u); };
 
-    uint32_t* const pre = (uint32_t*)(smem + F_W10 + 64);
+    constexpr uint32_t F_PRE = F_W10 + 32u;
+    uint32_t* const pre = (uint32_t*)(smem + F_PRE);
     bool have_pre = false;
     { const ItemMeta m0 = f.meta_sample[tid];
       ((double*)(smem + SIDF))[tid] = m0.idf > 0.0 ? m0.idf : 1.0; ((uint8_t*)(smem + SATTR))[tid] = (uint8_t)m0.attr;
@@ -425,7 +427,7 @@
                 }
                 __syncthreads();
                 if (sv_flag[0] != 0u) break;
-                if (tid < PREP_LANES) prep_group(ix_arg, (const uint64_t*)sv_items, (const uint32_t*)sv_off, 0u, tid, p.m, p.max_len, const_cast<char*>(p.prep) + (size_t)blockIdx.x * p.prep_stride, nullptr, 0u, nullptr);
+                if (tid < PREP_LANES) prep_group<false>(ix_arg, (const uint64_t*)sv_items, (const uint32_t*)sv_off, 0u, tid, p.m, p.max_len, const_cast<char*>(p.prep) + (size_t)blockIdx.x * p.prep_stride, nullptr, 0u, nullptr, WIDE);
                 __syncthreads();
                 if (tid == 0u) c->stamp[1] = (uint32_t)(wall_clock64() - serve_t0);
             }
@@ -442,26 +444,52 @@
         const char* const rec = p.prep + (size_t)q * p.prep_stride;
         struct { uint32_t U, rmax, xlo, sumw, L, n_staged, cur_attr, unsafe; } hd;
         constexpr uint32_t HW = (uint32_t)sizeof(PrepHead) / 4u;
+        constexpr uint32_t RW0 = (uint32_t)offsetof(PrepHead, ready) / 4u;
+        constexpr bool READY = !MID && MODE != FM_BACK && !TINY;
+        static_assert(!READY || sizeof(PrepHead) + 8u * sizeof(PrepItem) <= 128u * 4u, "a lean record lies inside the 128 words wave 1 parks");
         struct { uint32_t idx, kept; unsigned long long base; } x0{kNone, 0u, 0ull};
-        if (have_pre) {
-            auto uni = [&](uint32_t w) -> uint32_t { return (uint32_t)__builtin_amdgcn_readfirstlane((int)pre[w]); };
-            hd.U = uni(0); hd.rmax = uni(1); hd.xlo = uni(2); hd.sumw = uni(3); hd.L = uni(6); hd.n_staged = uni(7); hd.cur_attr = uni(16); hd.unsafe = uni(17);
-            if (lane < (LONG ? 32u : MID ? 16u : 8u) && lane < hd.L) { const uint32_t* it = pre + HW + 6u * lane; x0.idx = it[0]; x0.kept = it[3]; x0.base = ((unsigned long long)it[5] << 32) | it[4]; }
+        const bool from_pre = have_pre;
+        have_pre = false;
+        auto uni = [&](uint32_t w) -> uint32_t { return (uint32_t)__builtin_amdgcn_readfirstlane((int)pre[w]); };
+        auto load_x0 = [&]() {
+            if (from_pre) { if (lane < (LONG ? 32u : MID ? 16u : 8u) && lane < hd.L) { const uint32_t* it = pre + HW + 6u * lane; x0.idx = it[0]; x0.kept = it[3]; x0.base = ((unsigned long long)it[5] << 32) | it[4]; } }
+            else if ((MID ? lane < (LONG ? 32u : 16u) && lane < p.max_len : lane < 8u) && lane < hd.L) { const PrepItem pi = ((const PrepItem*)(rec + sizeof(PrepHead)))[lane]; x0.idx = pi.idx; x0.kept = pi.kept; x0.base = pi.base; } };
+        uint32_t rw = 0u;
+        uint32_t l15 = lane; asm volatile("" : "+v"(l15)); l15 &= 15u;
+        if (from_pre) {
+            hd.U = uni(0); hd.xlo = uni(2); hd.L = uni(6); hd.n_staged = uni(7); hd.cur_attr = uni(16);
+            if constexpr (READY) { rw = pre[RW0 + l15]; asm volatile("" : "+v"(rw)); }
+            else { hd.rmax = uni(1); hd.sumw = uni(3); hd.unsafe = uni(17); }
         } else {
-            const PrepHead h0 = *(const PrepHead*)rec;
-            hd.U = h0.U; hd.rmax = h0.rmax; hd.xlo = h0.xlo; hd.sumw = h0.sumw; hd.L = h0.L; hd.n_staged = h0.n_staged; hd.cur_attr = h0.cur_attr; hd.unsafe = h0.unsafe;
-            if ((MID ? lane < (LONG ? 32u : 16u) && lane < p.max_len : lane < 8u) && lane < hd.L) { const PrepItem pi = ((const PrepItem*)(rec + sizeof(PrepHead)))[lane]; x0.idx = pi.idx; x0.kept = pi.kept; x0.base = pi.base; }
-        }
-        have_pre = false;
+            const PrepHead& h0 = *(const PrepHead*)rec;
+            hd.U = h0.U; hd.xlo = h0.xlo; hd.L = h0.L; hd.n_staged = h0.n_staged; hd.cur_attr = h0.cur_attr;
+            if constexpr (READY) rw = ((const uint32_t*)rec)[RW0 + l15];
+            else { hd.rmax = h0.rmax; hd.sumw = h0.sumw; hd.unsafe = h0.unsafe; }
+        }
+        auto rdy = [&](uint32_t w) -> uint32_t { return (uint32_t)__builtin_amdgcn_readlane((int)rw, (int)w); };
         const uint32_t L = hd.L, n = hd.n_staged, U = hd.U;
-        unsigned long long rm = __ballot(x0.kept > 0u);
+        const uint32_t rflags = READY ? rdy(RW_FLAGS) : 0u;
+        const bool ready_ok = READY && (rflags & 1u) != 0u;
+        unsigned long long rm = 0ull;
+        uint32_t nr = (rflags >> 8) & 7u;
+        if (!ready_ok) {
+            if constexpr (READY) {
+                if (from_pre) { hd.rmax = uni(1); hd.sumw = uni(3); hd.unsafe = uni(17); }
+                else { const PrepHead& h0 = *(const PrepHead*)rec; hd.rmax = h0.rmax; hd.sumw = h0.sumw; hd.unsafe = h0.unsafe; }
+            }
+            load_x0();
+            rm = __ballot(x0.kept > 0u);
 #ifdef SRN_FAST_EXP_ONELIST
-        rm &= 0ull - rm;
-#endif
-        const uint32_t nr = (uint32_t)__popcll(rm);
-        const bool rel = MID || (WIDE && nr > 3u);
+            rm &= 0ull - rm;
+#endif
+            nr = (uint32_t)__popcll(rm);
+        }
+#ifdef SRN_FAST_EXP_ONELIST
+        else nr = min(nr, 1u);
+#endif
+        const bool rel = MID || (WIDE && (ready_ok ? (rflags >> 16) & 1u : nr > 3u));
         const uint32_t NB = LONG ? F_LONG_NB : MID ? max(nr, 4u) : WIDE && !rel ? 3u : 4u, NBM = (1u << NB) - 1u, base = rel ? hd.xlo : 0u;
-        const bool fits = hd.unsafe != 0u ? false : LONG ? L >= 1u && L <= F_LONG_LMAX && L <= p.max_len && hd.sumw <= F_LONG_CLASSES && nr <= F_LONG_LISTS && 2u * n + 8u + F_LONG_RES_WORDS <= MW && hd.rmax - hd.xlo < (1u << (32u - F_LONG_NB))
+        const bool fits = READY ? ready_ok : hd.unsafe != 0u ? false : LONG ? L >= 1u && L <= F_LONG_LMAX && L <= p.max_len && hd.sumw <= F_LONG_CLASSES && nr <= F_LONG_LISTS && 2u * n + 8u + F_LONG_RES_WORDS <= MW && hd.rmax - hd.xlo < (1u << (32u - F_LONG_NB))
                         : MID ? L >= 1u && L <= F_MID_LMAX && L <= p.max_len && hd.sumw <= F_MID_CLASSES && nr <= F_MID_LISTS && 2u * n + 8u + 256u <= MW && hd.rmax - hd.xlo < (1u << (32u - NB))
                               : L >= 1u && L <= 8u && L <= p.max_len && hd.sumw <= 15u && nr <= 4u && 2u * n + 8u <= MW && (!rel || hd.rmax - hd.xlo < (1u << 28));
         uint32_t* const xq = MODE == FM_FUSED ? nullptr : f.xchg + (size_t)q * f.xchg_stride;
@@ -481,6 +509,23 @@
         }
         if (n == 0u) { if (tid == 0) { if constexpr (MODE == FM_FRONT) xq[0] = 0u; else p.out_counts[q] = 0u; } continue; }
         uint32_t kp[NL], ps[NL]; const uint32_t* src[NL];
+        uint32_t lmask = 0u, cur_idx;
+        if constexpr (READY) {
+            lmask = rdy(RW_LMASK);
+#ifdef SRN_FAST_EXP_ONELIST
+            lmask &= 31u;
+#endif
+            const uint32_t psw = rdy(RW_PS);
+#pragma unroll
+            for (int r = 0; r < NL; ++r) {
+                kp[r] = rdy(RW_KEPT + r); ps[r] = (psw >> (8 * r)) & 0xFFu;
+#ifdef SRN_FAST_EXP_ONELIST
+                if (r) kp[r] = 0u;
+#endif
+                src[r] = ix.post_rank + (((unsigned long long)rdy(RW_BASE + 2 * r + 1) << 32) | rdy(RW_BASE + 2 * r));
+            }
+            cur_idx = rdy(RW_CUR);
+        } else {
 #pragma unroll
         for (int r = 0; r < NL; ++r) {
             const int l = rm ? __ffsll((long long)rm) - 1 : 0;
@@ -490,7 +535,8 @@
             ps[r] = (uint32_t)l;
             rm &= rm - 1ull;
         }
-        const uint32_t cur_idx = (uint32_t)__builtin_amdgcn_readlane((int)x0.idx, 0);
+        cur_idx = (uint32_t)__builtin_amdgcn_readlane((int)x0.idx, 0);
+        }
         const uint32_t cur_attr = hd.cur_attr;
         const uint32_t s1 = kp[0], s2 = s1 + kp[1], s3 = s2 + kp[2];
 
@@ -507,8 +553,11 @@
 #pragma unroll
         for (int r = 0; r < 4; ++r)
 #pragma unroll
-            for (int j = 0; j < 5; ++j) { v[r][j] = 0u; if ((uint32_t)j * BLOCK < kp[r]) v[r][j] = src[r][min(tid + j * BLOCK, kp[r] - 1u)]; }
-        }
+            for (int j = 0; j < 5; ++j) { v[r][j] = 0u; if (READY ? (lmask >> (5 * r + j)) & 1u : (uint32_t)j * BLOCK < kp[r]) v[r][j] = src[r][min(tid + j * BLOCK, kp[r] - 1u)]; }
+        }
+#ifdef SRN_FAST_SUBTICKS
+        FAST_TICK(15);
+#endif
         __syncthreads();
         FAST_PRIO(FP_FRONT);
         if constexpr (MODE != FM_BACK) {
@@ -856,10 +905,13 @@
         const uint32_t qn = MID ? q_after : ordered || listed ? q_ord_next : q + gridDim.x;
         const bool park = MID ? q_after != 0xFFFFFFFFu : ordered || listed ? q_ord_next != 0xFFFFFFFFu : qn < p.nq;
         if (wave == 1u && park) {
-            const char* const rn = p.prep + (size_t)qn * p.prep_stride + lane * 4u;
+            uint32_t lo4 = lane * 4u; asm volatile("" : "+v"(lo4));
+            const char* const rn = p.prep + (size_t)qn * p.prep_stride + lo4;
             const uint32_t dst = (uint32_t)__builtin_amdgcn_readfirstlane((int)lds_addr(pre));
             if (lane * 4u < p.prep_stride) glds_dword_uncounted(rn, dst);
-            if (256u + lane * 4u < min(p.prep_stride, 320u)) glds_dword_uncounted(rn + 256, dst + 256u);
+            constexpr uint32_t PARK = (uint32_t)(sizeof(PrepHead) + (MID ? 10u : 8u) * sizeof(PrepItem));
+            static_assert((MID && !SRN_MID_PREFETCH) || F_PRE + PARK <= F_SINV, "the parked record ends in front of F_SINV");
+            if (256u + lane * 4u < min(p.prep_stride, PARK)) glds_dword_uncounted(rn + 256, dst + 256u);
         }
 #pragma unroll
         for (int t = 0; t < 3; ++t) {
diff --git a/serenade_amd/csrc/srn_internal.h b/serenade_amd/csrc/srn_internal.h
--- a/serenade_amd/csrc/srn_internal.h
+++ b/serenade_amd/csrc/srn_internal.h
@@ -194,6 +194,7 @@
 int device_kernel_timing(DeviceState* d, int enable);
 int device_reserve(DeviceState* d, const FlatIndex& ix, const LaunchParams& p, void* stream);
 int device_last_path_counts(DeviceState* d, uint32_t* nq, uint32_t* general, uint32_t* global_pass);
+int device_debug_prep_records(DeviceState* d, const FlatIndex& ix, const uint64_t* items_flat, const uint32_t* q_off, size_t nq, size_t m, size_t max_len, void* out, size_t cap_bytes, size_t* out_stride);
 int device_last_mid_count(DeviceState* d, uint32_t* listed, uint32_t* big_listed = nullptr);
 int device_last_dedup_count(DeviceState* d, uint32_t* merged);
 static constexpr unsigned kFlagNoResultCache = 0x80000000u;
diff --git a/serenade_amd/csrc/srn_kernels.h b/serenade_amd/csrc/srn_kernels.h
--- a/serenade_amd/csrc/srn_kernels.h
+++ b/serenade_amd/csrc/srn_kernels.h
@@ -27,7 +27,8 @@
 
 struct LaunchAux { const uint32_t* qlist; const uint32_t* qlist_n; uint32_t* retry_list; uint32_t* retry_cnt; char* gscratch; unsigned long long gscratch_stride; char* nb_spill; };
 
-struct PrepHead { uint32_t U, rmax, xlo, sumw, P, nruns, L, n_staged, run_start[8], cur_attr, unsafe; };
+enum ReadyWord : uint32_t { RW_FLAGS = 0, RW_LMASK = 1, RW_CUR = 2, RW_PS = 3, RW_KEPT = 4, RW_BASE = 8, RW_WORDS = 16 };
+struct PrepHead { uint32_t U, rmax, xlo, sumw, P, nruns, L, n_staged, run_start[8], cur_attr, unsafe, ready[RW_WORDS]; };
 struct PrepItem { uint32_t idx, len, pre, kept; unsigned long long base; };
 
 struct ShardPos { uint32_t idx, len; unsigned long long base; };
@@ -55,7 +56,9 @@
 static constexpr uint32_t F_SURV = F_TABLE + F_TABLE_WORDS * 8;
 static constexpr uint32_t F_LDS_BYTES = F_SURV + F_SURV_WORDS * 4;
 static constexpr uint32_t F_WORK = F_NBL, F_WORK_WORDS = (F_LDS_BYTES - F_WORK) / 4;
+static constexpr uint32_t F_LEAN_MW = F_WORK_WORDS;
 static constexpr uint32_t F_M_MAX = 2560;
+static_assert(F_M_MAX <= 5 * 512, "a list is staged in <= 5 loads of 512 entries: ReadyWord RW_LMASK has 5 bits per run");
 static constexpr uint32_t F_FIN_BYTES = 1024, F_FIN_ENTRIES = F_FIN_BYTES / 16 - 1;
 static_assert(F_CAND + F_CAND_CAP * 12 <= F_HOT, "candidate buffer overlaps the accumulators");
 static constexpr uint32_t F_BIG_TOTAL = 80 * 1024;
@@ -142,7 +145,7 @@
 };
 hipError_t launch_predict(const PredictLaunch& a, dim3 grid, size_t lds, hipStream_t st, const DeviceIndex& di, const LaunchParams& p, const KernelCfg& c);
 hipError_t launch_prep(hipStream_t st, const DeviceIndex& di, const uint64_t* items_flat, const uint32_t* q_off, uint32_t nq, uint32_t m,
-                       uint32_t max_len, char* out, uint32_t stride, uint32_t* zero_a = nullptr, uint32_t* zero_b = nullptr,
+                       uint32_t max_len, char* out, uint32_t stride, bool wide, uint32_t* zero_a = nullptr, uint32_t* zero_b = nullptr,
                        const IdSlot* loc_table = nullptr, uint32_t loc_mask = 0, unsigned long long* okeys = nullptr);
 hipError_t launch_finish_big(hipStream_t st, const DeviceIndex& di, const FastParams& f, uint64_t* out_ids, double* out_scores, uint32_t* out_counts, uint32_t how_many, uint32_t grid, const uint32_t* cnt_retry = nullptr, const uint32_t* cnt_slow = nullptr, uint32_t* host_words = nullptr);
 hipError_t launch_finish(hipStream_t st, const DeviceIndex& di, const FastParams& f, uint64_t* out_ids, double* out_scores, uint32_t* out_counts, uint32_t nq, uint32_t how_many);
@@ -153,7 +156,7 @@
 hipError_t launch_shard_lists_copy(hipStream_t st, const DeviceIndex& di, uint32_t nq, uint32_t max_len, const ShardPos* pos_in, const uint32_t* kept, const long long* off,
                                    uint32_t* out);
 hipError_t launch_shard_prep(hipStream_t st, const uint64_t* items_flat, const uint32_t* q_off, uint32_t nq, uint32_t max_len, uint32_t n_shards, const uint32_t* kept_g,
-                             const long long* off_g, unsigned long long shard_stride, const int* head, const ShardPos* pos_local, char* out, uint32_t stride,
+                             const long long* off_g, unsigned long long shard_stride, const int* head, const ShardPos* pos_local, char* out, uint32_t stride, bool wide,
                              const unsigned long long* shard_base = nullptr, bool direct = false);
 hipError_t launch_shard_max(hipStream_t st, int* dst, const int* src, size_t n);
 hipError_t launch_shard_offsets(hipStream_t st, const uint32_t* kept_g, uint32_t nq, uint32_t max_len, uint32_t n_shards, long long* off_g, unsigned long long* tot_dev,
diff --git a/serenade_amd/csrc/srn_kernels.hip b/serenade_amd/csrc/srn_kernels.hip
--- a/serenade_amd/csrc/srn_kernels.hip
+++ b/serenade_amd/csrc/srn_kernels.hip
@@ -282,14 +282,14 @@
 }
 
 __global__ __launch_bounds__(256) void vmis_prep_kernel(DeviceIndex ix, const uint64_t* __restrict__ items_flat, const uint32_t* __restrict__ q_off,
-                                                        uint32_t nq, uint32_t m, uint32_t max_len, char* out, uint32_t stride, uint32_t* zero_a, uint32_t* zero_b,
+                                                        uint32_t nq, uint32_t m, uint32_t max_len, char* out, uint32_t stride, bool wide, uint32_t* zero_a, uint32_t* zero_b,
                                                         const IdSlot* __restrict__ loc_table, uint32_t loc_mask, unsigned long long* __restrict__ okeys) {
     const uint32_t t = blockIdx.x * blockDim.x + threadIdx.x;
     if (t < 8 && zero_a) zero_a[t] = 0u;
     if (t == 8 && zero_b) *zero_b = 0u;
     const uint32_t q = t / PREP_LANES, sub = t % PREP_LANES;
     if (q >= nq) return;
-    prep_group(ix, items_flat, q_off, q, sub, m, max_len, out + (size_t)q * stride, loc_table, loc_mask, okeys);
+    prep_group(ix, items_flat, q_off, q, sub, m, max_len, out + (size_t)q * stride, loc_table, loc_mask, okeys, wide);
 }
 
 #ifndef SRN_GEN_PRIO_LEVELS
@@ -1310,10 +1310,10 @@
 }
 
 hipError_t launch_prep(hipStream_t st, const DeviceIndex& di, const uint64_t* items_flat, const uint32_t* q_off, uint32_t nq, uint32_t m,
-                       uint32_t max_len, char* out, uint32_t stride, uint32_t* zero_a, uint32_t* zero_b, const IdSlot* loc_table, uint32_t loc_mask, unsigned long long* okeys) {
-    static_assert(sizeof(PrepHead) == 72 && sizeof(PrepItem) == 24, "vmis_prep_kernel writes the record word by word");
+                       uint32_t max_len, char* out, uint32_t stride, bool wide, uint32_t* zero_a, uint32_t* zero_b, const IdSlot* loc_table, uint32_t loc_mask, unsigned long long* okeys) {
+    static_assert(sizeof(PrepHead) == 136 && offsetof(PrepHead, ready) == 72 && sizeof(PrepItem) == 24, "vmis_prep_kernel writes the record word by word");
     const uint32_t per_block = 256 / PREP_LANES;
-    hipLaunchKernelGGL(vmis_prep_kernel, dim3((nq + per_block - 1) / per_block), dim3(256), 0, st, di, items_flat, q_off, nq, m, max_len, out, stride, zero_a, zero_b, loc_table, loc_mask, okeys);
+    hipLaunchKernelGGL(vmis_prep_kernel, dim3((nq + per_block - 1) / per_block), dim3(256), 0, st, di, items_flat, q_off, nq, m, max_len, out, stride, wide, zero_a, zero_b, loc_table, loc_mask, okeys);
     return hipGetLastError();
 }
 
diff --git a/serenade_amd/csrc/srn_latency.hip b/serenade_amd/csrc/srn_latency.hip
--- a/serenade_amd/csrc/srn_latency.hip
+++ b/serenade_amd/csrc/srn_latency.hip
@@ -140,7 +140,7 @@
     const bool tiny_fast = plan.fast && (kn.tiny_fast == 3 || (kn.tiny_fast >= 1 && p.max_len > 8) || (kn.tiny_fast == 2 && p.nq <= (kn.no_tiny_fused ? 32u : (uint32_t)kn.tiny_fused_max)));
     if (tiny_fast) { int rc = reserve_fast(w, cap_q); if (rc) return rc; }
     const bool fused = tiny_fast && p.nq <= (uint32_t)kn.tiny_fused_max && !kn.no_tiny_fused;
-    if (!fused) { w->cnt_dirty = true; HIP_TRY(launch_prep(st, d->di, p.items_flat, p.q_off, p.nq, p.m, p.max_len, w->prep, prep_stride, tiny_fast ? w->slow_cnt : nullptr)); }
+    if (!fused) { w->cnt_dirty = true; HIP_TRY(launch_prep(st, d->di, p.items_flat, p.q_off, p.nq, p.m, p.max_len, w->prep, prep_stride, plan.nb_fast == 3u, tiny_fast ? w->slow_cnt : nullptr)); }
     p.prep = w->prep; p.prep_stride = prep_stride;
     TinyCall c{d, w, geo, p, plan, kn, pin, st, blocking_wait};
     int rc = SRN_OK;
diff --git a/serenade_amd/csrc/srn_prep.h b/serenade_amd/csrc/srn_prep.h
--- a/serenade_amd/csrc/srn_prep.h
+++ b/serenade_amd/csrc/srn_prep.h
@@ -6,9 +6,31 @@
 
 namespace srn {
 
+struct ReadyRuns { uint32_t nr = 0, lmask = 0, ps = 0, kept[4] = {0u, 0u, 0u, 0u}; unsigned long long base[4] = {0ull, 0ull, 0ull, 0ull}; };
+__device__ __forceinline__ void ready_add(ReadyRuns& rr, uint32_t pos, uint32_t kept, unsigned long long base) {
+    if (kept == 0u) return;
+#pragma unroll
+    for (uint32_t r = 0; r < 4u; ++r) if (rr.nr == r) { rr.kept[r] = kept; rr.base[r] = base; }
+    if (rr.nr < 4u) { rr.lmask |= ((1u << min((kept + 511u) >> 9, 5u)) - 1u) << (5u * rr.nr); rr.ps |= (pos & 0xFFu) << (8u * rr.nr); }
+    rr.nr = min(rr.nr + 1u, 7u);
+}
+__device__ __forceinline__ void ready_words(const ReadyRuns& rr, uint32_t (&w)[RW_WORDS], uint32_t L, uint32_t max_len, uint32_t sumw, uint32_t n_staged, uint32_t rmax, uint32_t xlo,
+                                            uint32_t unsafe, bool wide, uint32_t cur_idx) {
+#pragma unroll
+    for (uint32_t i = 0; i < RW_WORDS; ++i) w[i] = 0u;
+    if (!(L >= 1u && L <= 8u && L <= max_len && rr.nr <= 4u)) return;
+    const bool rel = wide && rr.nr > 3u;
+    const bool lean_ok = unsafe == 0u && sumw <= 15u && 2u * n_staged + 8u <= F_LEAN_MW && (!rel || rmax - xlo < (1u << 28));
+    w[RW_FLAGS] = (lean_ok ? 1u : 0u) | (rr.nr << 8) | (rel ? 1u << 16 : 0u);
+    w[RW_LMASK] = rr.lmask; w[RW_CUR] = cur_idx; w[RW_PS] = rr.ps;
+#pragma unroll
+    for (uint32_t r = 0; r < 4u; ++r) { w[RW_KEPT + r] = rr.kept[r]; w[RW_BASE + 2u * r] = (uint32_t)rr.base[r]; w[RW_BASE + 2u * r + 1u] = (uint32_t)(rr.base[r] >> 32); }
+}
+
 static constexpr uint32_t PREP_LANES = 8;
+template <bool BLOCK = true>
 __device__ __forceinline__ void prep_group(const DeviceIndex& ix, const uint64_t* __restrict__ items_flat, const uint32_t* __restrict__ q_off, uint32_t q, uint32_t sub, uint32_t m, uint32_t max_len,
-                                           char* rec, const IdSlot* __restrict__ loc_table, uint32_t loc_mask, unsigned long long* __restrict__ okeys) {
+                                           char* rec, const IdSlot* __restrict__ loc_table, uint32_t loc_mask, unsigned long long* __restrict__ okeys, bool wide) {
     const uint32_t qb = q_off[q], L = q_off[q + 1] - qb;
     PrepItem* items = (PrepItem*)(rec + sizeof(PrepHead));
     uint32_t U = 0, rmax = 0, xlo = 0, sumw = 0, P = 0, nruns = 0, n_staged = 0, cur_attr = SRN_ATTR_NONE, my_run_start = 0;
@@ -67,6 +89,7 @@
         P += __shfl(sc_len, PREP_LANES - 1, PREP_LANES); nruns += __shfl(sc_run, PREP_LANES - 1, PREP_LANES);
         if (have && rounds > 1) items[pos] = PrepItem{idx, len, pre, 0u, base};
     }
+    uint32_t kept_last = 0;
     for (uint32_t r = 0; r < rounds; ++r) {
         const uint32_t pos = r * PREP_LANES + sub;
         const bool have = pos < L;
@@ -102,6 +125,7 @@
             }
             if (rounds > 1) items[pos].kept = kept; else items[pos] = PrepItem{idx, len, pre, kept, base};
         }
+        kept_last = kept;
         uint32_t ks = kept;
         #pragma unroll
         for (uint32_t d = 1; d < PREP_LANES; d <<= 1) ks += __shfl_xor(ks, d, PREP_LANES);
@@ -127,6 +151,23 @@
         *(uint2*)(hw + 16) = make_uint2(cur_attr, unsafe);
     }
     hw[8 + sub] = sub < nruns ? my_run_start : 0u;
+    static_assert(offsetof(PrepHead, ready) == 72 && RW_WORDS == 2 * PREP_LANES, "lane s writes words 2 s, 2 s + 1 of the block");
+    if constexpr (!BLOCK) *(uint2*)(hw + 18 + 2u * sub) = make_uint2(0u, 0u);
+    else {
+        ReadyRuns rr;
+        const uint32_t k1 = rounds == 1u ? kept_last : 0u;
+#pragma unroll
+        for (uint32_t s = 0; s < PREP_LANES; ++s) {
+            const uint32_t ks = __shfl(k1, s, PREP_LANES), blo = __shfl((uint32_t)base, s, PREP_LANES), bhi = __shfl((uint32_t)(base >> 32), s, PREP_LANES);
+            ready_add(rr, s, ks, ((unsigned long long)bhi << 32) | blo);
+        }
+        uint32_t w[RW_WORDS];
+        ready_words(rr, w, L, max_len, sumw, n_staged, rmax, xlo, unsafe, wide, __shfl(idx, 0, PREP_LANES));
+        uint2 o = make_uint2(0u, 0u);
+#pragma unroll
+        for (uint32_t s = 0; s < PREP_LANES; ++s) if (sub == s) o = make_uint2(w[2u * s], w[2u * s + 1u]);
+        *(uint2*)(hw + 18 + 2u * sub) = o;
+    }
 }
 
 }
diff --git a/serenade_amd/csrc/srn_runtime.hip b/serenade_amd/csrc/srn_runtime.hip
--- a/serenade_amd/csrc/srn_runtime.hip
+++ b/serenade_amd/csrc/srn_runtime.hip
@@ -379,10 +379,11 @@
     return SRN_OK;
 }
 
-static uint32_t fast_nb(const FlatIndex& ix, const Knobs& kn) {
-    const int rank_bits_f = std::max(1, bits_host(ix.n_kept ? ix.n_kept - 1 : 0));
+static uint32_t fast_nb_of(uint64_t n_kept, const Knobs& kn) {
+    const int rank_bits_f = std::max(1, bits_host(n_kept ? n_kept - 1 : 0));
     return kn.fast_runs == 3 && rank_bits_f <= 29 ? 3u : rank_bits_f <= 28 ? 4u : rank_bits_f <= 29 ? 3u : 0u;
 }
+static uint32_t fast_nb(const FlatIndex& ix, const Knobs& kn) { return fast_nb_of(ix.n_kept, kn); }
 FastPlan fast_plan(const DeviceState* d, const FlatIndex& ix, const LaunchParams& p, const Geometry& geo, const Knobs& kn, bool has_ext) {
     FastPlan f;
     f.nb_fast = fast_nb(ix, kn);
@@ -541,7 +542,7 @@
 
 static int enqueue_front(BatchCall& c, hipStream_t s, char* rec) {
     const LaunchParams& p = c.p; const LaunchPlan& pl = c.pl; OrderBufs& ob = c.ob; Workspace* w = c.w;
-    HIP_TRY(launch_prep(s, c.di, p.items_flat, p.q_off, p.nq, p.m, p.max_len, rec, pl.prep_stride, pl.prep_clears && pl.fast.fast ? w->slow_cnt : nullptr,
+    HIP_TRY(launch_prep(s, c.di, p.items_flat, p.q_off, p.nq, p.m, p.max_len, rec, pl.prep_stride, pl.fast.nb_fast == 3u, pl.prep_clears && pl.fast.fast ? w->slow_cnt : nullptr,
                         pl.prep_clears && pl.retry ? w->retry_cnt : nullptr, nullptr, 0, ob.keys_in));
     if (pl.dedup) {
         HIP_TRY(hipMemsetAsync(ob.dd.slots, 0xFF, (size_t)ob.dd.n_slots * 8, s));
@@ -835,7 +836,7 @@
     if (n_shards != ix.n_shards) return fail(SRN_EINVAL, "n_shards differs from the number of shards this index was cut into");
     if (!device_shard_lists_supported(d, ix, p)) return fail(SRN_EINVAL, "lists mode needs position-set slots (sessions of <= 8 items, m <= m_index, complete lists): use the three-stage pipeline");
     const uint32_t stride = device_prep_stride(p.max_len);
-    HIP_TRY(launch_shard_prep((hipStream_t)stream, p.items_flat, p.q_off, p.nq, p.max_len, n_shards, kept_g, off_g, shard_stride, head, (const ShardPos*)pos_local, records, stride, shard_base, direct));
+    HIP_TRY(launch_shard_prep((hipStream_t)stream, p.items_flat, p.q_off, p.nq, p.max_len, n_shards, kept_g, off_g, shard_stride, head, (const ShardPos*)pos_local, records, stride, fast_nb(ix, knobs()) == 3u, shard_base, direct));
     ExtLists ext{records, stride, direct ? d->di.post_rank : lists_g};
     return predict_ext(d, ix, p, stream, ext);
 }
@@ -848,7 +849,7 @@
     const bool ordered = order_buf && kn.order_min > 0 && p.nq >= (uint32_t)kn.order_min;
     OrderBufs ob;
     if (ordered) { int rc = order_room(order_buf, order_bytes, p.nq, &ob); if (rc) return rc; }
-    HIP_TRY(launch_prep((hipStream_t)stream, post->di, p.items_flat, p.q_off, p.nq, p.m, p.max_len, records, device_prep_stride(p.max_len), nullptr, nullptr, d->di.id_table, d->di.id_mask, ob.keys_in));
+    HIP_TRY(launch_prep((hipStream_t)stream, post->di, p.items_flat, p.q_off, p.nq, p.m, p.max_len, records, device_prep_stride(p.max_len), fast_nb_of(d->di.n_kept, kn) == 3u , nullptr, nullptr, d->di.id_table, d->di.id_mask, ob.keys_in));
     if (ordered) { HIP_TRY(sort_order_keys((hipStream_t)stream, ob.keys_in, ob.keys_out, p.nq, ob.temp, &ob.temp_bytes)); *order_out = ob.keys_out; }
     return SRN_OK;
 }
@@ -917,6 +918,30 @@
     if (nq) *nq = w->last_nq;
     if (general) *general = w->last_fast ? w->h_retry[HW_GENERAL] : w->last_nq;
     if (global_pass) *global_pass = w->last_retry ? w->h_retry[HW_GLOBAL] : 0;
+    return SRN_OK;
+}
+int device_debug_prep_records(DeviceState* d, const FlatIndex& ix, const uint64_t* items_flat, const uint32_t* q_off, size_t nq, size_t m, size_t max_len, void* out, size_t cap_bytes, size_t* out_stride) {
+    if (!q_off || !out_stride || (nq && !out)) return fail(SRN_EINVAL, "null buffer");
+    if (nq > (1u << 24) || m == 0 || m > 0xFFFFFFFFull || max_len == 0 || max_len > SRN_MAX_SESSION_LEN) return fail(SRN_ERANGE, "srn_debug_prep_records: sizes out of range");
+    for (size_t q = 0; q < nq; ++q) if (q_off[q + 1] < q_off[q]) return fail(SRN_EINVAL, "srn_debug_prep_records: q_off must not decrease");
+    const uint32_t stride = prep_stride_of((uint32_t)max_len);
+    *out_stride = stride;
+    if (nq == 0) return SRN_OK;
+    const size_t n_items = q_off[nq], rec_bytes = nq * (size_t)stride;
+    if (n_items && !items_flat) return fail(SRN_EINVAL, "null buffer");
+    if (cap_bytes < rec_bytes) return fail(SRN_ERANGE, "srn_debug_prep_records: the output buffer is too small");
+    HIP_TRY(hipSetDevice(d->device));
+    const size_t items_bytes = (n_items + 1) * 8, off_bytes = ((nq + 1) * 4 + 7) & ~(size_t)7;
+    void* mem = nullptr;
+    if (hipMalloc(&mem, items_bytes + off_bytes + rec_bytes) != hipSuccess) { (void)hipGetLastError(); return fail(SRN_ENOMEM, "srn_debug_prep_records: hipMalloc failed"); }
+    uint64_t* d_items = (uint64_t*)mem; uint32_t* d_off = (uint32_t*)((char*)mem + items_bytes); char* d_rec = (char*)mem + items_bytes + off_bytes;
+    hipError_t e = hipMemset(d_rec, 0, rec_bytes);
+    if (e == hipSuccess && n_items) e = hipMemcpy(d_items, items_flat, n_items * 8, hipMemcpyHostToDevice);
+    if (e == hipSuccess) e = hipMemcpy(d_off, q_off, (nq + 1) * 4, hipMemcpyHostToDevice);
+    if (e == hipSuccess) e = launch_prep(0, d->di, d_items, d_off, (uint32_t)nq, (uint32_t)m, (uint32_t)max_len, d_rec, stride, fast_nb(ix, knobs()) == 3u);
+    if (e == hipSuccess) e = hipMemcpy(out, d_rec, rec_bytes, hipMemcpyDeviceToHost);
+    (void)hipFree(mem);
+    if (e != hipSuccess) return fail(SRN_EHIP, std::string("srn_debug_prep_records: ") + hipGetErrorString(e));
     return SRN_OK;
 }
 int device_last_mid_count(DeviceState* d, uint32_t* listed, uint32_t* big_listed) {
diff --git a/serenade_amd/csrc/srn_shard.hip b/serenade_amd/csrc/srn_shard.hip
--- a/serenade_amd/csrc/srn_shard.hip
+++ b/serenade_amd/csrc/srn_shard.hip
@@ -4,6 +4,7 @@
 
 #include "srn_device.h"
 #include "srn_kernels.h"
+#include "srn_prep.h"
 
 namespace srn {
 
@@ -74,11 +75,12 @@
 __global__ __launch_bounds__(256) void shard_prep_kernel(const uint64_t* __restrict__ items_flat, const uint32_t* __restrict__ q_off, uint32_t nq, uint32_t max_len,
                                                          uint32_t n_shards, const uint32_t* __restrict__ kept_g, const long long* __restrict__ off_g,
                                                          unsigned long long shard_stride, const unsigned long long* __restrict__ shard_base, const int* __restrict__ head,
-                                                         const ShardPos* __restrict__ pos_local, char* __restrict__ out, uint32_t stride, bool direct) {
+                                                         const ShardPos* __restrict__ pos_local, char* __restrict__ out, uint32_t stride, bool direct, bool wide) {
     const uint32_t q = blockIdx.x * blockDim.x + threadIdx.x;
     if (q >= nq) return;
     const uint32_t qb = q_off[q], L = q_off[q + 1] - qb;
-    PrepHead h{0u, 0u, 0u, 0u, 0u, 0u, L, 0u, {0u, 0u, 0u, 0u, 0u, 0u, 0u, 0u}, SRN_ATTR_NONE, 0u};
+    PrepHead h{0u, 0u, 0u, 0u, 0u, 0u, L, 0u, {0u, 0u, 0u, 0u, 0u, 0u, 0u, 0u}, SRN_ATTR_NONE, 0u, {}};
+    ReadyRuns rr; uint32_t cur_idx = kNone;
     PrepItem* items = (PrepItem*)(out + (size_t)q * stride + sizeof(PrepHead));
     if (L != 0 && L <= max_len) {
         h.xlo = (uint32_t)head[3 * (size_t)q]; h.rmax = (uint32_t)head[3 * (size_t)q + 1];
@@ -101,10 +103,12 @@
             }
             if (kp) { h.sumw += L - pos; if (h.nruns < 8) h.run_start[h.nruns] = h.P; ++h.nruns; }
             items[pos] = PrepItem{pos_local[(size_t)q * max_len + pos].idx, kp, h.P, kp, base};
+            ready_add(rr, pos, kp, base); if (pos == 0) cur_idx = items[0].idx;
             h.P += kp;
         }
         h.n_staged = h.P;
     }
+    ready_words(rr, h.ready, L, max_len, h.sumw, h.n_staged, h.rmax, h.xlo, h.unsafe, wide, cur_idx);
     *(PrepHead*)(out + (size_t)q * stride) = h;
 }
 
@@ -124,10 +128,10 @@
     return hipGetLastError();
 }
 hipError_t launch_shard_prep(hipStream_t st, const uint64_t* items_flat, const uint32_t* q_off, uint32_t nq, uint32_t max_len, uint32_t n_shards, const uint32_t* kept_g,
-                             const long long* off_g, unsigned long long shard_stride, const int* head, const ShardPos* pos_local, char* out, uint32_t stride,
+                             const long long* off_g, unsigned long long shard_stride, const int* head, const ShardPos* pos_local, char* out, uint32_t stride, bool wide,
                              const unsigned long long* shard_base, bool direct) {
     hipLaunchKernelGGL(shard_prep_kernel, dim3((nq + 255) / 256), dim3(256), 0, st, items_flat, q_off, nq, max_len, n_shards, kept_g, off_g, shard_stride, shard_base, head, pos_local,
-                       out, stride, direct);
+                       out, stride, direct, wide);
     return hipGetLastError();
 }
 
```

Result: faster. 57.62 million queries/s (median of 6 runs) (+2.5%).
